# MonsieurETM/QPSK

Measured on AMD Instinct MI355X. Metric: complex Msamples/s demodulated + % HBM roofline, 2400-baud RRC+Costas path, higher is better.
Workload: dtype f32

## Files before the change

include/qpsk_hip.h:

```cpp
#ifndef QPSK_HIP_H
#define QPSK_HIP_H

#include <stddef.h>
#include <stdint.h>

#ifdef __cplusplus
extern "C" {
#endif

#define QPSK_NTAPS 127

typedef enum {
    QPSK_OK = 0,
    QPSK_ERR_NO_DEVICE = -1,
    QPSK_ERR_ARG = -2,
    QPSK_ERR_HIP = -3,
    QPSK_ERR_ALLOC = -4,
    QPSK_ERR_STATE = -5,
    QPSK_ERR_RANGE = -6
} qpsk_status;

typedef enum {
    QPSK_TIMING_HIST = 0,
    QPSK_TIMING_FIXED = 1,
// ... 134 lines not shown
int qpsk_outer_push(qpsk_ctx *ctx, const uint8_t *d_bits, long long bits_pitch, int nbits, int max_words, int32_t *d_count, uint8_t *d_words,
                    long long word_pitch, long long *d_pos, uint8_t *d_flags, int32_t *d_info);
int qpsk_outer_interleave_batch(qpsk_ctx *ctx, const uint8_t *d_words, int nrows, int nwords, int n, int branches, const uint8_t *d_hist_in,
                                uint8_t *d_hist_out, uint8_t *d_out);

enum { QPSK_DISPERSAL_MSB_FIRST = 1 };
int qpsk_dispersal_batch(qpsk_ctx *ctx, const uint8_t *d_in, long long in_pitch, int nrows, int len, int group, int flags, const uint8_t *d_flags,
                         int first, uint8_t *d_out, long long out_pitch);
int qpsk_dispersal_sequence(int len, int group, int flags, uint8_t *out);

int qpsk_nodesync_reset(qpsk_ctx *ctx, int nlinks, int nrot, int nshift, int span, int settle, int thr_num, int thr_den, int drop);
int qpsk_nodesync_shifts(int period, uint32_t keep0, uint32_t keep1);
int qpsk_nodesync_push(qpsk_ctx *ctx, const int8_t *d_soft_in, long long in_pitch, int ntx, const int32_t *d_vinfo, int8_t *d_soft_out,
                       long long out_pitch, int32_t *d_info);
int qpsk_nodesync_set(qpsk_ctx *ctx, const int32_t *d_cand);


int qpsk_rrc_fir_batch(qpsk_ctx *ctx, float *d_memory, const float *d_in, float *d_out, int nframes, int length);

int qpsk_rrc_fir_batch_fast(qpsk_ctx *ctx, float *d_memory, const float *d_in, float *d_out, int nframes, int length);

int qpsk_timing_hist_batch(qpsk_ctx *ctx, const float *d_filtered, int nframes, int32_t *d_index, int32_t *d_hist);

int qpsk_timing_scan_batch(qpsk_ctx *ctx, const float *d_in, int nframes, int32_t *d_index, int32_t *d_hist);

int qpsk_timing_fft_batch(qpsk_ctx *ctx, const float *d_in, int nframes, int32_t *d_index, float *d_filtered,
                          double *d_spectrum);

int qpsk_timing_fft_bin_batch(qpsk_ctx *ctx, const float *d_in, int nframes, int32_t *d_index, float *d_filtered,
                              double *d_bin);

int qpsk_costas_batch(qpsk_ctx *ctx, const float *d_symbols_in, int nframes, int nsym, float *d_state,
                      uint8_t *d_sym, float *d_costas);

int qpsk_fft_batch(qpsk_ctx *ctx, const double *d_in, double *d_out, int nbatch, int n, int inverse);

int qpsk_streams_reset(qpsk_ctx *ctx, int nstreams, double mixer_hz);
int qpsk_streams_set_loop_state(qpsk_ctx *ctx, const float *h_state);
int qpsk_streams_get_loop_state(qpsk_ctx *ctx, float *h_state);
int qpsk_streams_rx_cplx(qpsk_ctx *ctx, const float *d_in, uint8_t *d_sym, float *d_freq, float *d_phase,
                         float *d_costas, int32_t *d_index);
int qpsk_streams_rx_pcm(qpsk_ctx *ctx, const int16_t *d_pcm, uint8_t *d_sym, float *d_freq, float *d_phase,
                        float *d_costas, int32_t *d_index);
int qpsk_streams_rx_pcm_host(qpsk_ctx *ctx, const int16_t *h_pcm, float *h_loop_io, uint8_t *h_sym, float *h_costas,
                             int32_t *h_index);

int qpsk_tx_reset(qpsk_ctx *ctx, int nstreams, double tx_hz);
int qpsk_tx_symbols(qpsk_ctx *ctx, const uint8_t *d_symbols, int nsym, int16_t *d_pcm, float *d_baseband);


int qpsk_crc16_batch(qpsk_ctx *ctx, const uint8_t *d_data, int npackets, int nbytes, uint16_t *d_crc);

int qpsk_interleave_batch(qpsk_ctx *ctx, uint8_t *d_data, int npackets, int nbytes, int dir);

int qpsk_scramble_batch(qpsk_ctx *ctx, uint8_t *d_sym, int npackets, int nsym);

typedef struct qpsk_multi qpsk_multi;
int qpsk_multi_create(qpsk_multi **out, const int *devices, int ndev, const qpsk_params *p);
void qpsk_multi_destroy(qpsk_multi *mj);
int qpsk_multi_shards(const qpsk_multi *mj);
int qpsk_multi_load(qpsk_multi *mj, long long total_frames, const float *h_in);
int qpsk_multi_shard(qpsk_multi *mj, int r, int *device, long long *first, long long *count, qpsk_ctx **ctx, float **d_in);
int qpsk_multi_use_device_input(qpsk_multi *mj, int r, const float *d_in);
int qpsk_multi_set_direct_output(qpsk_multi *mj, int slot, uint8_t *h_sym, float *h_freq, float *h_phase);
int qpsk_multi_set_packed(qpsk_multi *mj, int on);
int qpsk_pack_symbols(qpsk_ctx *ctx, const uint8_t *d_sym, long long nrows, int nsym, uint8_t *d_packed);
int qpsk_unpack_symbols_host(const uint8_t *h_packed, long long nrows, int nsym, uint8_t *h_sym);
int qpsk_host_alloc(void **h_ptr, size_t bytes);
int qpsk_host_free(void *h_ptr);
int qpsk_multi_set_acquisition(qpsk_multi *mj, const int32_t *h_index, const float *h_seed);
int qpsk_multi_set_data(qpsk_multi *mj, int on);
int qpsk_multi_rx_begin(qpsk_multi *mj, int slot);
int qpsk_multi_rx_end(qpsk_multi *mj, int slot, uint8_t *h_sym, float *h_freq, float *h_phase);

int qpsk_dev_alloc(qpsk_ctx *ctx, void **d_ptr, size_t bytes);
int qpsk_dev_free(qpsk_ctx *ctx, void *d_ptr);
int qpsk_dev_upload(qpsk_ctx *ctx, void *d_dst, const void *h_src, size_t bytes);
int qpsk_dev_download(qpsk_ctx *ctx, void *h_dst, const void *d_src, size_t bytes);

int qpsk_selftest_sincos_hash(qpsk_ctx *ctx, uint32_t first, uint32_t count, unsigned long long *h_out);

int qpsk_test_inject_status(qpsk_ctx *ctx, int code);
int qpsk_test_hist_state(qpsk_ctx *ctx, int32_t *out);
int qpsk_test_fir_runs(qpsk_ctx *ctx, int nframes, int length, int32_t out[3]);
int qpsk_test_viterbi_launches(qpsk_ctx *ctx, int *out);
int qpsk_test_deframer_advance(qpsk_ctx *ctx, long long delta);
int qpsk_test_viterbi_stream_advance(qpsk_ctx *ctx, long long delta);
int qpsk_test_outer_advance(qpsk_ctx *ctx, long long delta);

#ifdef __cplusplus
}
#endif
#endif
```

qpsk_amd/csrc/api_ctx.cpp:

```cpp
#include "api_ctx.h"

using namespace qpsk;

static thread_local char g_err[512] = "";

int qpsk::fail(int code, const char *fmt, ...)
{
    va_list ap;
    va_start(ap, fmt);
    vsnprintf(g_err, sizeof g_err, fmt, ap);
    va_end(ap);
    return code;
}

static const struct { const char *name; int Tuning::*field; } TUNING_KEYS[] = {
    {"QPSK_FUSED_G", &Tuning::fused_g},       {"QPSK_FUSED_S", &Tuning::fused_s},     {"QPSK_FUSED_LDS", &Tuning::fused_lds},
    {"QPSK_FUSED_GENERIC", &Tuning::generic}, {"QPSK_PIPE_NF", &Tuning::pipe_nf},
    {"QPSK_PIPE_DBG", &Tuning::pipe_variant}, {"QPSK_HIST_GENERIC", &Tuning::hist_generic},
    {"QPSK_PIPE_V", &Tuning::pipe_v},         {"QPSK_PIPE_G", &Tuning::pipe_g},
    {"QPSK_PIPE_LAYOUT_LO", &Tuning::layout_lo}, {"QPSK_PIPE_LAYOUT_HI", &Tuning::layout_hi},
    {"QPSK_FIR_GENERIC", &Tuning::fir_generic}, {"QPSK_FFT_FUSED", &Tuning::fft_fused},
    {"QPSK_STREAM_BLOCK", &Tuning::stream_block}, {"QPSK_STREAM_POLL", &Tuning::stream_poll},
    {"QPSK_STREAM_SCAN", &Tuning::stream_scan}, {"QPSK_STREAM_CARRIER", &Tuning::stream_carrier},
    {"QPSK_LEAN_DMA", &Tuning::lean_dma},     {"QPSK_LEAN_PAIR", &Tuning::lean_pair},
    {"QPSK_EST_WAVES", &Tuning::est_waves},   {"QPSK_HIST_ONEPASS", &Tuning::hist_onepass},
    {"QPSK_VITERBI_LDS", &Tuning::viterbi_lds},   {"QPSK_VITERBI_CHUNK_ROWS", &Tuning::viterbi_chunk_rows},
};

int qpsk::ensure(qpsk_ctx *c, DevBuf &b, size_t bytes)
{
    if (b.cap >= bytes) return QPSK_OK;
    if (b.p) {
        HIP_TRY(hipStreamSynchronize(c->stream));
        HIP_TRY(hipFree(b.p));
        b.p = nullptr;
        b.cap = 0;
    }
    hipError_t e = hipMalloc(&b.p, bytes);
    if (e != hipSuccess) {
        b.p = nullptr;
        return fail(QPSK_ERR_ALLOC, "hipMalloc(%zu bytes): %s", bytes, hipGetErrorString(e));
    }
    b.cap = bytes;
    return QPSK_OK;
}

int qpsk::check_status(qpsk_ctx *c)
{
    const int st = __atomic_exchange_n(c->status.h_status, 0, __ATOMIC_ACQ_REL);
    if (st != STATUS_PIPE_TIMEOUT) c->streams.stream_work_unchecked = false;
    if (st == STATUS_PIPE_TIMEOUT) {
        if (c->streams.nstreams > 0 && c->streams.stream_work_unchecked) c->streams.poison();
        c->streams.stream_work_unchecked = false;
        return fail(QPSK_ERR_HIP, "pipeline kernel: producer/consumer wait timed out; results of the calls since the last synchronisation are invalid");
    }
    if (st == STATUS_PHASE_RANGE)
        return fail(QPSK_ERR_RANGE, "Costas loop phase beyond the bounded 2 pi wrap (input amplitude far outside the modem's range; "
                                    "the reference's phase_wrap() would spin or hang, costas_loop.c:61-67); results of the calls since the last synchronisation are invalid");
    if (st == STATUS_BAD_INDEX)
        return fail(QPSK_ERR_ARG, "an external timing offset (qpsk_rx_batch_ext d_index_in) lies outside 0..%d: the kernel demodulated that frame "
                                  "at offset 0; results of the calls since the last synchronisation are invalid", MAX_INDEX);
    if (st == STATUS_EST_NONFINITE)
        return fail(QPSK_ERR_RANGE, "qpsk_carrier_est_batch: a NaN / Inf sample inside the window the estimate reads; results of the calls since "
                                    "the last synchronisation are invalid");
    if (st == STATUS_SOFT_NONFINITE)
        return fail(QPSK_ERR_RANGE, "qpsk_soft_batch / qpsk_deframer_push_coded: a NaN / Inf sample among those a row's sums or soft output use, or a NaN / Inf gain; "
                                    "results of the calls since the last synchronisation are invalid");
    if (st == STATUS_SOFT_BAD_LAG)
        return fail(QPSK_ERR_ARG, "qpsk_soft_batch: a lag in d_lag is negative or puts the payload beyond the row (that row's soft output is zeros); "
                                  "results of the calls since the last synchronisation are invalid");
    if (st == STATUS_NONFINITE)
        return fail(QPSK_ERR_RANGE, "a Costas loop ended on a NaN / Inf state: the input held a non-finite sample (the reference hangs in phase_wrap() "
                                    "on an infinite phase, costas_loop.c:61-67); results of the calls since the last synchronisation are invalid");
    if (st != 0) return fail(QPSK_ERR_HIP, "kernel status %d", st);
    return QPSK_OK;
}

int qpsk_test_inject_status(qpsk_ctx *c, int code)
{
    if (!c || !c->status.h_status) return fail(QPSK_ERR_ARG, "null context");
    __atomic_store_n(c->status.h_status, code, __ATOMIC_RELEASE);
    return QPSK_OK;
}

int qpsk::bind(const qpsk_ctx *c)
{
    HIP_TRY(hipSetDevice(c->device));
    return QPSK_OK;
}

int qpsk::use_context_gains(qpsk_ctx *c)
{
    const float g[2] = {c->alpha, c->beta};
    if (c->h_gains.size() != 2 || c->h_gains[0] != g[0] || c->h_gains[1] != g[1]) {
        HIP_TRY(hipStreamSynchronize(c->stream));
        c->h_gains.assign(g, g + 2);
        HIP_TRY(hipMemcpyAsync(c->d_gains, c->h_gains.data(), sizeof g, hipMemcpyHostToDevice, c->stream));
    }
    return QPSK_OK;
}

const char *qpsk_last_error(void) { return g_err; }
const char *qpsk_version(void) { return "qpsk_hip 0.3 (gfx950)"; }

int qpsk_device_count(void)
{
    int n = 0;
    if (hipGetDeviceCount(&n) != hipSuccess) return 0;
// ... 40 lines not shown
        return fail(QPSK_ERR_NO_DEVICE, "no HIP device available (%s); this library has no CPU path",
                    e == hipSuccess ? "device count 0" : hipGetErrorString(e));
    if (device < 0) HIP_TRY(hipGetDevice(&device));
    if (device >= ndev) return fail(QPSK_ERR_NO_DEVICE, "device %d out of range (%d devices)", device, ndev);
    if (!(p->fs > 0.0) || !(p->rs > 0.0) || p->frame_size <= 0)
        return fail(QPSK_ERR_ARG, "fs, rs and frame_size must be positive");
    const int cycles = (int)(p->fs / p->rs);
    if (cycles < 1 || cycles > 64) return fail(QPSK_ERR_ARG, "CYCLES = (int)(fs/rs) = %d out of range 1..64", cycles);
    if (p->frame_size % cycles != 0)
        return fail(QPSK_ERR_ARG, "frame_size %d is not a multiple of CYCLES %d", p->frame_size, cycles);
    if (p->timing_mode < QPSK_TIMING_HIST || p->timing_mode > QPSK_TIMING_FFT)
        return fail(QPSK_ERR_ARG, "unknown timing_mode %d", p->timing_mode);
    if (p->fixed_index < 0 || p->fixed_index > MAX_INDEX)
        return fail(QPSK_ERR_ARG, "fixed_index %d outside 0..%d", p->fixed_index, MAX_INDEX);

    HIP_TRY(hipSetDevice(device));
    KERNEL_TRY(prepare_kernels());
    KERNEL_TRY(prepare_pipe_kernel());
    KERNEL_TRY(prepare_timing_scan());
    KERNEL_TRY(prepare_stream_block());
    KERNEL_TRY(prepare_stream_scan());
    KERNEL_TRY(prepare_carrier_est());
    qpsk_ctx *c = new qpsk_ctx();
    c->device = device;
    for (const auto &k : TUNING_KEYS) {
        const char *v = getenv(k.name);
        if (!v || !*v) continue;
        if (k.field == &Tuning::viterbi_chunk_rows) {
            char *end = nullptr;
            const long n = strtol(v, &end, 10);
            if (end == v || *end) continue;
            c->tune.*(k.field) = n < 0 ? -1 : n > INT_MAX ? INT_MAX : (int)n;
            continue;
        }
        c->tune.*(k.field) = atoi(v);
    }
    if (c->tune.viterbi_chunk_rows == 0) {
        delete c;
        return fail(QPSK_ERR_ARG, "qpsk_ctx_create: QPSK_VITERBI_CHUNK_ROWS = 0 in the environment (>= 1, or negative for the library's own choice)");
    }
    {
        int ncu = 0;
        if (hipDeviceGetAttribute(&ncu, hipDeviceAttributeMultiprocessorCount, device) == hipSuccess && ncu > 0)
            c->ncu = ncu;
    }
    c->prm = *p;
    c->cycles = cycles;
    c->nsym = p->frame_size / cycles;
    c->stream = (hipStream_t)stream;
    qpsk_host_rrc_taps((float)p->fs, (float)p->rs, p->rrc_alpha, c->taps);
    c->damping = sqrtf(2.0f) / 2.0f;
    qpsk_host_loop_gains(c->damping, p->loop_bw, &c->alpha, &c->beta);
    c->min_freq = p->min_freq;
    c->max_freq = p->max_freq;
    if (hipMalloc((void **)&c->d_taps, 128 * sizeof(float)) != hipSuccess ||
        hipMalloc((void **)&c->d_gains, MAX_BW * 2 * sizeof(float)) != hipSuccess ||
        hipHostMalloc((void **)&c->status.h_status, sizeof(int), hipHostMallocMapped) != hipSuccess ||
        hipHostGetDevicePointer((void **)&c->status.d_status, c->status.h_status, 0) != hipSuccess) {
        qpsk_ctx_destroy(c);
        return fail(QPSK_ERR_ALLOC, "hipMalloc of configuration buffers failed");
    }
    *c->status.h_status = 0;
    if (hipHostMalloc((void **)&c->streams.h_done, sizeof(unsigned), hipHostMallocMapped) != hipSuccess ||
        hipHostGetDevicePointer((void **)&c->streams.d_done, c->streams.h_done, 0) != hipSuccess) {
        qpsk_ctx_destroy(c);
        return fail(QPSK_ERR_ALLOC, "pinned counter");
    }
    *c->streams.h_done = 0;
    int rc = upload_config(c);
    if (rc != QPSK_OK) { qpsk_ctx_destroy(c); return rc; }
    *out = c;
    return QPSK_OK;
}

void qpsk_ctx_destroy(qpsk_ctx *c)
{
    if (!c) return;
    hipSetDevice(c->device);
    hipStreamSynchronize(c->stream);
    hipFree(c->d_taps);
    hipFree(c->d_gains);
    if (c->status.h_status) hipHostFree(c->status.h_status);
    if (c->streams.h_done) hipHostFree(c->streams.h_done);
    for (DevBuf *b : {&c->index, &c->filtered, &c->mixed, &c->keystream, &c->sympad, &c->mislist, &c->datacostas, &c->vitdec, &c->softgain, &c->dfstage})
        b->release();
    for (auto &kv : c->twiddles) hipFree(kv.second);
    hipFree(c->d_fast);
    c->hist.release();
    c->streams.release();
    c->tx.release();
    c->df.release();
    c->framer.release();
    c->vs.release();
    c->outer.release();
    c->nodesync.release();
    c->dispersal.release();
    delete c;
}

int qpsk_ctx_sync(qpsk_ctx *c)
{
    if (!c) return fail(QPSK_ERR_ARG, "null context");
    HIP_TRY(hipSetDevice(c->device));
    HIP_TRY(hipStreamSynchronize(c->stream));
    return check_status(c);
}

int qpsk_pack_symbols(qpsk_ctx *c, const uint8_t *d_sym, long long nrows, int nsym, uint8_t *d_packed)
{
    if (!c || !d_sym || !d_packed || nrows < 0 || nsym <= 0) return fail(QPSK_ERR_ARG, "qpsk_pack_symbols: bad argument");
    if (bind(c)) return QPSK_ERR_HIP;
    if ((nsym & 15) == 0 && (((uintptr_t)d_sym & 15) || ((uintptr_t)d_packed & 3)))
        return fail(QPSK_ERR_ARG, "qpsk_pack_symbols: d_sym must be 16-byte and d_packed 4-byte aligned");
    KERNEL_TRY(launch_pack_dibits(d_sym, d_packed, (size_t)nrows, nsym, c->stream));
    return QPSK_OK;
}

int qpsk_unpack_symbols_host(const uint8_t *h_packed, long long nrows, int nsym, uint8_t *h_sym)
{
    if (!h_packed || !h_sym || nrows < 0 || nsym <= 0) return fail(QPSK_ERR_ARG, "qpsk_unpack_symbols_host: bad argument");
    const size_t pb = (size_t)(nsym + 3) / 4;
    for (long long r = 0; r < nrows; r++) {
        const uint8_t *p = h_packed + (size_t)r * pb;
        uint8_t *o = h_sym + (size_t)r * (size_t)nsym;
        for (int i = 0; i < nsym; i++) o[i] = (uint8_t)((p[i >> 2] >> (2 * (i & 3))) & 3u);
    }
    return QPSK_OK;
}

int qpsk_ctx_check(qpsk_ctx *c)
{
    if (!c) return fail(QPSK_ERR_ARG, "null context");
    return check_status(c);
}

extern "C" int qpsk_set_error(int code, const char *msg)
{
    return fail(code, "%s", msg ? msg : "");
}

int qpsk_ctx_set_stream(qpsk_ctx *c, void *stream)
{
    if (!c) return fail(QPSK_ERR_ARG, "null context");
    HIP_TRY(hipSetDevice(c->device));
    HIP_TRY(hipStreamSynchronize(c->stream));
    c->stream = (hipStream_t)stream;
    return QPSK_OK;
}

int qpsk_ctx_set_tuning(qpsk_ctx *c, const char *name, int value)
{
    if (!c || !name) return fail(QPSK_ERR_ARG, "null argument");
    for (const auto &k : TUNING_KEYS)
        if (!strcmp(k.name, name)) {
            if (value == 0 && k.field == &Tuning::viterbi_chunk_rows)
                return fail(QPSK_ERR_ARG, "qpsk_ctx_set_tuning: QPSK_VITERBI_CHUNK_ROWS = 0 (>= 1, or negative for the library's own choice)");
            c->tune.*(k.field) = value < 0 ? -1 : value;
            return QPSK_OK;
        }
    return fail(QPSK_ERR_ARG, "qpsk_ctx_set_tuning: unknown name '%s'", name);
}

int qpsk_ctx_cycles(const qpsk_ctx *c) { return c ? c->cycles : 0; }
int qpsk_ctx_nsym(const qpsk_ctx *c) { return c ? c->nsym : 0; }
const char *qpsk_ctx_last_kernel(const qpsk_ctx *c) { return c ? c->last_kernel : ""; }

int qpsk_ctx_get_taps(const qpsk_ctx *c, float *h)
// ... 83 lines not shown
```

qpsk_amd/csrc/api_ctx.h:

```cpp
#ifndef QPSK_API_CTX_H
#define QPSK_API_CTX_H

#include "../../include/qpsk_hip.h"
#include "host_math.h"
#include "kernels.h"

#include <hip/hip_runtime.h>
#include <limits.h>
#include <math.h>
#include <stdarg.h>
#include <stdio.h>
#include <stdlib.h>
#include <string.h>
#include <time.h>
#include <algorithm>
#include <initializer_list>
#include <map>
#include <vector>

struct qpsk_ctx;

namespace qpsk {

QPSK_UNIT_LOCAL int fail(int code, const char *fmt, ...);

#define HIP_TRY(expr)                                                                         \
    do {                                                                                      \
        hipError_t e_ = (expr);                                                               \
        if (e_ != hipSuccess)                                                                 \
            return fail(QPSK_ERR_HIP, "%s: %s (%s:%d)", #expr, hipGetErrorString(e_), __FILE__, __LINE__); \
    } while (0)

#define KERNEL_TRY(expr)                                                                      \
    do {                                                                                      \
        (void)hipGetLastError();  \
        int e_ = (expr);                                                                      \
        if (e_ != 0)                                                                          \
            return fail(QPSK_ERR_HIP, "%s: %s (%s:%d)", #expr, hipGetErrorString((hipError_t)e_), __FILE__, __LINE__); \
    } while (0)

struct QPSK_UNIT_LOCAL DevBuf {
    void *p = nullptr;
    size_t cap = 0;
    void release() { hipFree(p); *this = DevBuf(); }
};

struct Tuning {
    int fused_g = -1, fused_s = -1, fused_lds = -1;
    int generic = -1;
    int pipe_nf = -1;
    int pipe_v = -1, pipe_g = -1;
    int layout_lo = -1, layout_hi = -1;
    int pipe_variant = -1;
    int hist_generic = -1;
    int fir_generic = -1;
    int stream_scan = -1;
    int stream_poll = -1;
    int stream_block = -1;
    int stream_carrier = -1;
    int lean_dma = -1;
    int hist_onepass = -1;
    int est_waves = -1;
    int lean_pair = -1;
    int viterbi_lds = -1;
    int fft_fused = -1;
    int viterbi_chunk_rows = -1;
};

static inline int tuned(int v, int dflt) { return v >= 0 ? v : dflt; }


struct StatusWord {
    int *h_status = nullptr;
    int *d_status = nullptr;
};

struct QPSK_UNIT_LOCAL HistGuess {
    int32_t *d_hint = nullptr;
    int32_t *h_hist_stats = nullptr, *d_hist_stats = nullptr;
    bool hint_valid = false;
    void release();
};

struct QPSK_UNIT_LOCAL Streams {
    int nstreams = 0;
    float *s_memory = nullptr, *s_dec = nullptr, *s_loop = nullptr, *s_mixer = nullptr;
    float *s_ctab = nullptr, *s_cstate = nullptr;
    bool carrier_shared = false;
    unsigned carrier_blocks = 0;
    unsigned carrier_scans = 0;
    float *carrier_pending = nullptr;
    bool stream_work_unchecked = false;
    bool streams_poisoned = false;
    unsigned char *h_stage = nullptr, *d_stage = nullptr;
    size_t stage_cap = 0;
    unsigned *h_done = nullptr, *d_done = nullptr;
    unsigned done_expect = 0;
    void poison()
    {
        streams_poisoned = true;
        carrier_shared = false;
        carrier_pending = nullptr;
    }
    void release();
};

struct QPSK_UNIT_LOCAL Transmitters {
    int ntx = 0;
    uint8_t *t_hist = nullptr;
    float *t_mixer = nullptr;
    DevBuf tx_b;
    void release();
};

struct QPSK_UNIT_LOCAL Deframer {
    uint8_t *state = nullptr, *tables = nullptr;
    size_t stride = 0;
    int nstreams = 0, nsync = 0, min_score = 0, nbytes = 0, max_packets = 0;
    unsigned long long sync_lo[2] = {0, 0}, sync_hi[2] = {0, 0};
    bool ready = false;
    bool coded = false;
    int mode = 0, nsteps = 0;
    int nbody = 0;
    CodedLayout layout;
    float scale = 0.f;
    unsigned crc_init = 0;
    void release();
};

struct QPSK_UNIT_LOCAL Framer {
    uint8_t *ks = nullptr;
    int ks_len = 0;
    void release();
};

struct QPSK_UNIT_LOCAL ViterbiStream {
    uint8_t *state = nullptr;
    size_t stride = 0;
    int nstreams = 0, depth = 0, window = 0;
    Puncture punct = {1, 1u, 1u, 2};
    bool punctured = false;
    long long total = 0;
    long long advanced = 0;
    void release();
};

struct QPSK_UNIT_LOCAL OuterLink {
    uint8_t *state = nullptr;
    size_t stride = 0;
    int nstreams = 0, n = 0, branches = 0, sync = 0, lock = 0, drop = 0, flags = 0;
    int group = 0;
    long long total = 0;
    void release();
};

struct QPSK_UNIT_LOCAL NodeSync {
    uint8_t *state = nullptr;
    int nlinks = 0, nrot = 0, nshift = 0, span = 0, settle = 0, thr_num = 0, thr_den = 0, drop = 0;
    int have = 0;
    void release();
};

struct QPSK_UNIT_LOCAL Dispersal {
    uint8_t *table = nullptr;
    int len = 0, group = 0, flags = 0;
    void release();
};

}

struct qpsk_ctx {
    int device = 0;
    qpsk::Tuning tune;
    int ncu = 256;
    const char *last_kernel = "";
    int viterbi_launches = 0;
    bool taps_symmetric = false;
    hipStream_t stream = nullptr;
    qpsk_params prm{};
    int cycles = 0, nsym = 0;
    float taps[QPSK_NTAPS];
    float damping = 0.f, alpha = 0.f, beta = 0.f;
    float min_freq = 0.f, max_freq = 0.f;
    float *d_taps = nullptr;
    float *d_gains = nullptr;
    std::vector<float> h_gains;
    qpsk::DevBuf index, filtered, mixed, keystream, sympad, mislist;
    qpsk::DevBuf datacostas;
    qpsk::DevBuf vitdec;
    qpsk::DevBuf softgain;
    qpsk::DevBuf dfstage;
    int keystream_len = 0;
    std::map<int, double *> twiddles;
    float *d_fast = nullptr;
    bool fast_valid = false;
    qpsk::StatusWord status;
    qpsk::HistGuess hist;
    qpsk::Streams streams;
    qpsk::Transmitters tx;
    qpsk::Deframer df;
    qpsk::Framer framer;
    qpsk::ViterbiStream vs;
    qpsk::OuterLink outer;
    qpsk::NodeSync nodesync;
    qpsk::Dispersal dispersal;
};

namespace qpsk {

static const int MAX_BW = 64;

QPSK_UNIT_LOCAL int ensure(qpsk_ctx *c, DevBuf &b, size_t bytes);
QPSK_UNIT_LOCAL int check_status(qpsk_ctx *c);
QPSK_UNIT_LOCAL int bind(const qpsk_ctx *c);
QPSK_UNIT_LOCAL int use_context_gains(qpsk_ctx *c);

QPSK_UNIT_LOCAL int fir_full_rate(qpsk_ctx *c, const float *x, const float *memory, float *y, int nframes, int length, size_t in_pitch = 0);
QPSK_UNIT_LOCAL int fft_timing_indices(qpsk_ctx *c, const float *d_in, int nframes, int32_t *d_index, float *d_y = nullptr,
                                       double *d_X = nullptr, size_t pitch = 0, double *d_bin = nullptr);
QPSK_UNIT_LOCAL int costas_over_symbols(qpsk_ctx *c, float *d_symbols, int nframes, int nsym, int dstride, float *d_state,
                                        uint8_t *d_sym, float *d_costas, const float *refill = nullptr,
                                        const int32_t *refill_index = nullptr, bool refill_planar = false);

struct Pattern {
    int period;
    uint32_t keep0, keep1;
};
QPSK_UNIT_LOCAL int layout_add_pattern(const char *who, const Pattern *pattern, CodedLayout *l);
QPSK_UNIT_LOCAL int layout_add_stride(const char *who, int nsteps, const int *stride, CodedLayout *l);
struct ViterbiRoute {
    size_t per_row;
    bool lds;
    size_t chunk_rows;
};
QPSK_UNIT_LOCAL ViterbiRoute viterbi_route(const qpsk_ctx *c, size_t rows, int nsteps);

}

#endif
```

qpsk_amd/csrc/api_rx.cpp:

```cpp
#include "api_ctx.h"

using namespace qpsk;

#ifdef QPSK_PIPE_PROFILE
static const int PIPE_VARIANT_MASK = ~0;
#else
static const int PIPE_VARIANT_MASK = 4 | 8 | 16 | 64 | 128 | 256 | 512 | 1024 | 8192;
#endif

int qpsk_test_hist_state(qpsk_ctx *c, int32_t *out)
{
    if (!c || !out) return fail(QPSK_ERR_ARG, "null argument");
    out[0] = out[1] = out[2] = out[3] = out[4] = -1;
    if (!c->hist.d_hint) return QPSK_OK;
    HIP_TRY(hipSetDevice(c->device));
    HIP_TRY(hipStreamSynchronize(c->stream));
    int32_t h[2];
    HIP_TRY(hipMemcpy(h, c->hist.d_hint, sizeof h, hipMemcpyDeviceToHost));
    out[0] = c->hist.hint_valid ? h[0] : -1;
    out[1] = h[1];
    out[2] = c->hist.h_hist_stats[0]; out[3] = c->hist.h_hist_stats[1]; out[4] = c->hist.h_hist_stats[2];
    return QPSK_OK;
}

int qpsk_test_fir_runs(qpsk_ctx *c, int nframes, int length, int32_t out[3])
{
    if (!c || !out) return fail(QPSK_ERR_ARG, "qpsk_test_fir_runs: null argument");
    if (nframes < 1 || length < 1) return fail(QPSK_ERR_ARG, "qpsk_test_fir_runs: nframes %d length %d", nframes, length);
    const FirRuns r = rrc_fir_stream_runs(nframes, length, c->ncu);
    out[0] = r.ntiles; out[1] = r.parts; out[2] = r.tpp;
    return QPSK_OK;
}

void HistGuess::release()
{
    if (d_hint) hipFree(d_hint);
    if (h_hist_stats) hipHostFree(h_hist_stats);
    *this = HistGuess();
}

static bool fir_takes_stream(const qpsk_ctx *c) { return c->taps_symmetric && tuned(c->tune.fir_generic, 0) == 0; }

int qpsk::fir_full_rate(qpsk_ctx *c, const float *x, const float *memory, float *y, int nframes, int length, size_t in_pitch)
{
    if (fir_takes_stream(c))
        return launch_rrc_fir_stream(x, memory, y, c->d_taps, nframes, length, c->stream, in_pitch, c->ncu);
    return launch_rrc_fir(x, memory, y, c->d_taps, nframes, length, c->stream, in_pitch);
}

static void pick_tiling(const qpsk_ctx *c, int nframes, int nbw, int *G, int *S)
{
    int g = nframes / 256;
    if (g < 1) g = 1;
    if (g > 64 / nbw) g = 64 / nbw;
    if (g < 1) g = 1;
    g = tuned(c->tune.fused_g, g);
    if (g < 1) g = 1;
    if (g * nbw > 64) g = 64 / nbw;
    int s = tuned(c->tune.fused_s, 64);
    s &= ~7;
    if (s < 8) s = 8;
    const size_t budget = (size_t)tuned(c->tune.fused_lds, 64 * 1024);
    while (s > 8 && fused_lds_bytes(g, s, c->cycles, nbw) > budget) s -= 8;
    while (g > 1 && fused_lds_bytes(g, s, c->cycles, nbw) > (size_t)MAX_LDS_BYTES) g--;
    *G = g;
    *S = s;
}

static int get_twiddles(qpsk_ctx *c, int n, double **out)
{
    auto it = c->twiddles.find(n);
    if (it != c->twiddles.end()) { *out = it->second; return QPSK_OK; }
    const size_t cnt = n >= 2 ? (size_t)n / 2 : 1;
    std::vector<double> h(2 * cnt, 0.0);
    qpsk_host_twiddles(n, h.data());
    double *tw = nullptr;
    HIP_TRY(hipMalloc((void **)&tw, sizeof(double) * 2 * cnt));
    HIP_TRY(hipMemcpy(tw, h.data(), sizeof(double) * 2 * cnt, hipMemcpyHostToDevice));
    c->twiddles[n] = tw;
    *out = tw;
    return QPSK_OK;
}

static int fft_timing_tables(qpsk_ctx *c, double **tw_out, double **cs_out)
{
    const int C = c->cycles, nfft = timing_fft_nfft();
    if (C < 2 || C > 8 || (C & (C - 1)))
        return fail(QPSK_ERR_ARG, "QPSK_TIMING_FFT needs CYCLES in {2,4,8} (the symbol-rate bin NFFT/CYCLES must be exact and the offset < 8); CYCLES = %d", C);
    if (c->prm.frame_size < timing_fft_first() + nfft)
        return fail(QPSK_ERR_ARG, "QPSK_TIMING_FFT needs frame_size >= %d", timing_fft_first() + nfft);
    double *tw = nullptr;
    int rc = get_twiddles(c, nfft, &tw);
    if (rc) return rc;
    double *cs = nullptr;
    auto it = c->twiddles.find(-C);
    if (it == c->twiddles.end()) {
        std::vector<double> full(2 * (size_t)C);
        qpsk_host_phases(C, full.data());
        HIP_TRY(hipMalloc((void **)&cs, sizeof(double) * 2 * C));
        HIP_TRY(hipMemcpy(cs, full.data(), sizeof(double) * 2 * C, hipMemcpyHostToDevice));
        c->twiddles[-C] = cs;
    } else {
        cs = it->second;
    }
    *tw_out = tw;
    *cs_out = cs;
    return QPSK_OK;
}

int qpsk::fft_timing_indices(qpsk_ctx *c, const float *d_in, int nframes, int32_t *d_index, float *d_y, double *d_X, size_t pitch, double *d_bin)
{
    double *tw = nullptr, *cs = nullptr;
    int rc = fft_timing_tables(c, &tw, &cs);
// ... 152 lines not shown
            if (hint) hipFree(hint);
            return fail(QPSK_ERR_ALLOC, "one-pass histogram route: %s", hipGetErrorString(e));
        }
        h_stats[0] = h_stats[1] = h_stats[2] = -1;
        c->hist.d_hint = hint;
        c->hist.h_hist_stats = h_stats;
        c->hist.d_hist_stats = d_stats;
        c->hist.hint_valid = false;
    }
    const int op = tuned(c->tune.hist_onepass, -1);
    const int seen = __atomic_load_n(&c->hist.h_hist_stats[1], __ATOMIC_ACQUIRE), off_majority = __atomic_load_n(&c->hist.h_hist_stats[2], __ATOMIC_ACQUIRE);
    const bool guess_is_good = seen > 0 && off_majority == 0;
    if (op == 0 || !c->hist.hint_valid || !(op == 1 || guess_is_good) || !rx_hist_shape_ok(a)) return QPSK_OK;
    if (int rc = ensure(c, c->index, sizeof(int32_t) * (size_t)a.nframes)) return rc;
    if (int rc = ensure(c, c->mislist, sizeof(int32_t) * (size_t)a.nframes)) return rc;
    int32_t *mis_count = c->hist.d_hint + 1;
    HIP_TRY(hipMemsetAsync(mis_count, 0, sizeof(int32_t), c->stream));
    KERNEL_TRY(launch_rx_hist(a, (int32_t *)c->index.p, c->hist.d_hint, (int32_t *)c->mislist.p, mis_count, c->status.d_status, c->stream));
    FusedArgs af = a;
    af.index = (const int32_t *)c->index.p;
    af.frame_list = (const int32_t *)c->mislist.p;
    af.frame_list_count = mis_count;
    af.G = 4;
    af.S = 64;
    KERNEL_TRY(launch_rx_fused(af, c->stream));
    KERNEL_TRY(launch_index_majority((const int32_t *)c->index.p, a.nframes, c->hist.d_hint, mis_count, c->hist.d_hist_stats, c->stream));
    c->last_kernel = "rx_hist_kernel (one pass on the guessed index) + rx_fused_kernel (fall-back list)";
    if (d_index)
        HIP_TRY(hipMemcpyAsync(d_index, c->index.p, sizeof(int32_t) * (size_t)a.nframes, hipMemcpyDeviceToDevice, c->stream));
    *taken = true;
    return QPSK_OK;
}

static int rx_launch(qpsk_ctx *c, const FusedArgs &a, const RxRoute &rt)
{
    if (a.est_tw && !(rt.kind == K_FUSED_PIPE && rt.nf == pipe_max_nf()) && rt.kind != K_LEAN)
        return fail(QPSK_ERR_STATE, "internal: in-launch FFT timing estimate planned for a kernel that has none");
    if (a.data_rule && rt.kind != K_LEAN)
        return fail(QPSK_ERR_STATE, "internal: data rule planned for a kernel that has none");
    switch (rt.kind) {
    case K_LEAN:
        KERNEL_TRY(launch_rx_lean(a, rt.G, rt.layout, c->status.d_status, c->stream));
        c->last_kernel = a.est_tw ? "rx_lean_kernel (FFT timing estimate inside the launch)" : "rx_lean_kernel";
        break;
    case K_PIPE2:
        KERNEL_TRY(launch_rx_pipe2(a, rt.G, rt.layout, c->status.d_status, c->stream));
        c->last_kernel = "rx_pipe2_kernel";
        break;
    case K_FUSED_PIPE:
        KERNEL_TRY(launch_rx_fused_pipe(a, rt.nf, c->status.d_status, c->stream));
        c->last_kernel = a.est_tw ? "rx_fused_pipe_kernel (FFT timing estimate inside the launch)" : "rx_fused_pipe_kernel";
        break;
    default:
        KERNEL_TRY(launch_rx_fused(a, c->stream));
        c->last_kernel = "rx_fused_kernel";
    }
    return QPSK_OK;
}

static int rx_batch_common(qpsk_ctx *c, const float *d_in, long long frame_pitch, int nframes, int nbw, uint8_t *d_sym,
                           float *d_freq, float *d_phase, float *d_costas, int32_t *d_index, float *d_hz,
                           const ExtAcq *ext = nullptr, uint8_t *d_data = nullptr)
{
    if (!c || !d_in || !(d_sym || d_data)) return fail(QPSK_ERR_ARG, "qpsk_rx_batch: null context, input or symbol buffer");
    if (nframes <= 0) return fail(QPSK_ERR_ARG, "qpsk_rx_batch: nframes = %d", nframes);
    if (frame_pitch == 0) frame_pitch = c->prm.frame_size;
    if (frame_pitch < c->prm.frame_size)
        return fail(QPSK_ERR_ARG, "qpsk_rx_batch_pitched: frame_pitch %lld below frame_size %d", frame_pitch, c->prm.frame_size);
    if (bind(c)) return QPSK_ERR_HIP;
    FusedArgs a{};
    a.x = reinterpret_cast<const float2 *>(d_in);
    a.frame_pitch = (size_t)frame_pitch;
    a.nframes = nframes;
    a.frame_size = c->prm.frame_size;
    a.cycles = c->cycles;
    a.nsym = c->nsym;
    pick_tiling(c, nframes, nbw, &a.G, &a.S);
    a.fixed_index = c->prm.fixed_index;
    a.dbg = tuned(c->tune.pipe_variant, 0) & PIPE_VARIANT_MASK;
    a.lean_dma = tuned(c->tune.lean_dma, 1) != 0;
    a.lean_twowin = tuned(c->tune.lean_dma, 1) != 2 ? 1 : 0;
    a.est_waves = tuned(c->tune.est_waves, 0);
    a.lean_pair = tuned(c->tune.lean_pair, 3);
    a.taps = c->d_taps;
    a.gains = c->d_gains;
    a.nbw = nbw;
    a.min_freq = c->min_freq;
    a.max_freq = c->max_freq;
    a.rs = c->prm.rs;
    a.sym = d_sym ? d_sym : d_data;
    a.data_rule = d_data && !d_sym;
    a.freq = d_freq;
    a.phase = d_phase;
    a.costas = reinterpret_cast<float2 *>(d_costas);
    a.hz = d_hz;
    a.status = c->status.d_status;
    if (ext) a.index = ext->index;
    if (ext && ext->seed) {
        a.state_in = ext->seed;
        a.seed_setters = 1;
    }

    RxRoute rt;
    if (int rc = rx_route(c, a, d_data != nullptr, &rt)) return rc;

    a.data_rule = rt.data_rule;
    if (rt.need_pad) {
        if (int rc = ensure(c, c->sympad, (size_t)rt.G * (size_t)c->nsym)) return rc;
        a.sym_pad = (uint8_t *)c->sympad.p;
    }
    if (rt.need_dump) {
        if (int rc = ensure(c, c->datacostas, sizeof(float2) * (size_t)nframes * (size_t)c->nsym)) return rc;
        a.costas = (float2 *)c->datacostas.p;
    }

    const bool hist_guess = c->prm.timing_mode == QPSK_TIMING_HIST && !ext;
    if (hist_guess) {
        bool taken = false;
        const int rc = rx_hist_onepass(c, a, rt, d_index, &taken);
        if (rc || taken) return rc;
    }

    const int32_t *idx = a.index;
    if (!idx) {
        if (int rc = timing_indices(c, d_in, (size_t)frame_pitch, nframes, &idx, rt.fused_fft)) return rc;
        a.index = idx;
    }
    if (rt.fused_fft) {
        double *est_tw = nullptr, *est_cs = nullptr;
        if (int rc = fft_timing_tables(c, &est_tw, &est_cs)) return rc;
        a.est_tw = reinterpret_cast<const double2 *>(est_tw);
        a.est_cs = reinterpret_cast<const double2 *>(est_cs);
        a.index_out = d_index ? (int32_t *)c->index.p : nullptr;
        if (d_index) idx = (const int32_t *)c->index.p;
    }

    if (int rc = rx_launch(c, a, rt)) return rc;

    if (hist_guess && c->hist.d_hint && idx && tuned(c->tune.hist_onepass, -1) != 0) {
        KERNEL_TRY(launch_index_majority(idx, nframes, c->hist.d_hint, c->hist.d_hint + 1, c->hist.d_hist_stats, c->stream));
        c->hist.hint_valid = true;
    }
    if (rt.kind == K_LEAN && (nframes & 1)) {
        const size_t last0 = (size_t)((nframes - 1) / rt.G) * (size_t)rt.G;
        HIP_TRY(hipMemcpyAsync(a.sym + (size_t)(nframes - 1) * (size_t)c->nsym, a.sym_pad + ((size_t)(nframes - 1) - last0) * (size_t)c->nsym,
                               (size_t)c->nsym, hipMemcpyDeviceToDevice, c->stream));
    }
    if (d_data && !a.data_rule)
        KERNEL_TRY(launch_data_from_costas(a.costas, d_data, (size_t)nframes * (size_t)c->nsym, c->stream));
    if (d_index) {
        if (idx == d_index) {
        } else if (idx)
            HIP_TRY(hipMemcpyAsync(d_index, idx, sizeof(int32_t) * (size_t)nframes, hipMemcpyDeviceToDevice, c->stream));
        else
            KERNEL_TRY(launch_fill_i32(d_index, nframes, c->prm.fixed_index, c->stream));
    }
    return QPSK_OK;
}

static int rx_prologue(qpsk_ctx *c)
{
    if (!c) return QPSK_OK;
    if (bind(c)) return QPSK_ERR_HIP;
    return use_context_gains(c);
}

// ... 46 lines not shown

int qpsk_rx_batch_data(qpsk_ctx *c, const float *d_in, long long frame_pitch, int nframes, const int32_t *d_index_in, const float *d_seed,
                       uint8_t *d_data, uint8_t *d_sym, float *d_freq, float *d_phase, int32_t *d_index, float *d_hz)
{
    if (int rp = rx_prologue(c)) return rp;
    if (frame_pitch < 0) return fail(QPSK_ERR_ARG, "qpsk_rx_batch_data: frame_pitch = %lld", frame_pitch);
    if (!d_data) return fail(QPSK_ERR_ARG, "qpsk_rx_batch_data: d_data is NULL");
    const ExtAcq ext = {d_index_in, d_seed};
    return rx_batch_common(c, d_in, frame_pitch, nframes, 1, d_sym, d_freq, d_phase, nullptr, d_index, d_hz, &ext, d_data);
}

int qpsk_sync_batch(qpsk_ctx *c, const uint8_t *d_data, int nframes, int nsym, const uint8_t *h_sync, int nsync, int lag_min, int lag_max,
                    int nout, uint8_t *d_out, int32_t *d_lag, int32_t *d_rot, int32_t *d_score)
{
    if (!c || !d_data || !h_sync) return fail(QPSK_ERR_ARG, "qpsk_sync_batch: null context, data or sync word");
    if (nframes <= 0 || nsym <= 0) return fail(QPSK_ERR_ARG, "qpsk_sync_batch: nframes = %d, nsym = %d", nframes, nsym);
    if (nsync < 1 || nsync > SYNC_MAX_WORD) return fail(QPSK_ERR_ARG, "qpsk_sync_batch: nsync = %d outside 1..%d", nsync, SYNC_MAX_WORD);
    if (nout < 0 || lag_min < 0 || lag_max < lag_min || (long long)lag_max + nsync + nout > nsym)
        return fail(QPSK_ERR_ARG, "qpsk_sync_batch: lags %d..%d, nsync %d, nout %d do not fit a row of %d", lag_min, lag_max, nsync, nout, nsym);
    if (!d_out && !d_lag && !d_rot && !d_score) return fail(QPSK_ERR_ARG, "qpsk_sync_batch: every output is NULL");
    for (int i = 0; i < nsync; i++)
        if (h_sync[i] > 3) return fail(QPSK_ERR_ARG, "qpsk_sync_batch: sync[%d] = %d is not a dibit", i, (int)h_sync[i]);
    if (d_out && nout > 0) {
        const uintptr_t o0 = (uintptr_t)d_out, o1 = o0 + (size_t)nframes * (size_t)nout;
        const uintptr_t d0 = (uintptr_t)d_data, d1 = d0 + (size_t)nframes * (size_t)nsym;
        if (o0 < d1 && d0 < o1) return fail(QPSK_ERR_ARG, "qpsk_sync_batch: d_out overlaps d_data");
    }
    if (bind(c)) return QPSK_ERR_HIP;
    KERNEL_TRY(launch_sync_search(d_data, nframes, nsym, h_sync, nsync, lag_min, lag_max, nout, nout > 0 ? d_out : nullptr, d_lag, d_rot,
                                  d_score, c->stream));
    c->last_kernel = "sync_search_kernel";
    return QPSK_OK;
}

int qpsk_rx_batch_bw_ext(qpsk_ctx *c, const float *d_in, int nframes, const float *h_loop_bw, int nbw, const int32_t *d_index_in,
                         const float *d_seed, uint8_t *d_sym, float *d_freq, float *d_phase, int32_t *d_index)
{
    const ExtAcq ext = {d_index_in, d_seed};
    return rx_batch_bw_impl(c, d_in, nframes, h_loop_bw, nbw, d_sym, d_freq, d_phase, d_index, &ext);
}

int qpsk::costas_over_symbols(qpsk_ctx *c, float *d_symbols, int nframes, int nsym, int dstride, float *d_state,
                              uint8_t *d_sym, float *d_costas, const float *refill, const int32_t *refill_index, bool refill_planar)
{
    float *carrier_tab = c->streams.carrier_pending;
    c->streams.carrier_pending = nullptr;
    if (tuned(c->tune.generic, 0)) {
        if (carrier_tab) KERNEL_TRY(launch_carrier_table(c->streams.s_cstate, carrier_tab, c->prm.frame_size, true, c->stream));
        KERNEL_TRY(launch_costas(d_symbols, nframes, nsym, dstride, 1, c->d_gains, c->min_freq, c->max_freq, d_state, d_state,
                                 d_sym, d_costas, c->status.d_status, c->stream));
        if (refill) {
            if (dstride != nsym) return fail(QPSK_ERR_ARG, "internal: refill needs packed rows");
            KERNEL_TRY(launch_decimate(refill, refill_index, d_symbols, nframes, nsym * c->cycles, c->cycles, nsym, c->stream));
        }
        return QPSK_OK;
    }
    FusedArgs a{};
    a.nframes = nframes;
    a.nsym = nsym;
    a.frame_size = nsym * c->cycles;
    a.cycles = c->cycles;
    a.refill = reinterpret_cast<const float2 *>(refill);
    a.refill_dst = reinterpret_cast<float2 *>(d_symbols);
    a.refill_planar = refill_planar ? 1 : 0;
    a.index = refill_index;
    a.gains = c->d_gains;
    a.nbw = 1;
    a.min_freq = c->min_freq;
    a.max_freq = c->max_freq;
    a.rs = c->prm.rs;
    a.state_in = d_state;
    a.state_out = d_state;
    a.sym = d_sym;
    a.costas = reinterpret_cast<float2 *>(d_costas);
    a.dsrc = reinterpret_cast<const float2 *>(d_symbols);
    a.dstride = dstride;
    a.status = c->status.d_status;
    if (carrier_tab) {
        a.carrier_state = c->streams.s_cstate;
        a.carrier_tab = reinterpret_cast<float2 *>(carrier_tab);
        a.carrier_frame = c->prm.frame_size;
    }
    a.dbg = tuned(c->tune.pipe_variant, 0) & PIPE_VARIANT_MASK;
    int nf = (nframes + c->ncu * pipe_frames(1) - 1) / (c->ncu * pipe_frames(1));
    if (nf < 1) nf = 1;
    if (nf > pipe_max_nf()) nf = pipe_max_nf();
    KERNEL_TRY(launch_costas_pipe(a, nf, c->status.d_status, c->stream));
    return QPSK_OK;
}

int qpsk_rrc_fir_batch(qpsk_ctx *c, float *d_memory, const float *d_in, float *d_out, int nframes, int length)
{
    if (!c || !d_in || !d_out) return fail(QPSK_ERR_ARG, "qpsk_rrc_fir_batch: null argument");
    if (nframes <= 0 || length <= 0) return fail(QPSK_ERR_ARG, "qpsk_rrc_fir_batch: nframes %d length %d", nframes, length);
    if (bind(c)) return QPSK_ERR_HIP;
    const float *src = d_in;
    if (d_in == d_out) {
        const size_t bytes = sizeof(float) * 2 * (size_t)nframes * length;
        int rc = ensure(c, c->mixed, bytes);
        if (rc) return rc;
        HIP_TRY(hipMemcpyAsync(c->mixed.p, d_in, bytes, hipMemcpyDeviceToDevice, c->stream));
        src = (const float *)c->mixed.p;
    }
    KERNEL_TRY(fir_full_rate(c, src, d_memory, d_out, nframes, length));
    c->last_kernel = fir_takes_stream(c) ? "rrc_fir_stream_kernel" : "rrc_fir_kernel";
    if (d_memory) KERNEL_TRY(launch_delay_line(src, d_memory, nframes, length, c->stream));
    return QPSK_OK;
}

int qpsk_rrc_fir_batch_fast(qpsk_ctx *c, float *d_memory, const float *d_in, float *d_out, int nframes, int length)
{
    if (!c || !d_in || !d_out) return fail(QPSK_ERR_ARG, "qpsk_rrc_fir_batch_fast: null argument");
    if (nframes <= 0 || length <= 0) return fail(QPSK_ERR_ARG, "qpsk_rrc_fir_batch_fast: nframes %d length %d", nframes, length);
    if (d_in == d_out) return fail(QPSK_ERR_ARG, "qpsk_rrc_fir_batch_fast: every block reads 126 samples in front of it: separate buffers");
    if (bind(c)) return QPSK_ERR_HIP;
    if (!c->fast_valid) {
        const int n = rrc_fir_fast_nfft();
        std::vector<float> t(4 * (size_t)n);
        qpsk_host_fir_fast_tables(c->taps, t.data(), t.data() + 2 * n);
        if (!c->d_fast) HIP_TRY(hipMalloc((void **)&c->d_fast, sizeof(float) * t.size()));
        HIP_TRY(hipStreamSynchronize(c->stream));
        HIP_TRY(hipMemcpy(c->d_fast, t.data(), sizeof(float) * t.size(), hipMemcpyHostToDevice));
        c->fast_valid = true;
    }
    KERNEL_TRY(launch_rrc_fir_fast(d_in, d_memory, d_out, c->d_fast, c->d_fast + 2 * rrc_fir_fast_nfft(), nframes, length, c->stream));
    if (d_memory) KERNEL_TRY(launch_delay_line(d_in, d_memory, nframes, length, c->stream));
    return QPSK_OK;
}

int qpsk_timing_hist_batch(qpsk_ctx *c, const float *d_filtered, int nframes, int32_t *d_index, int32_t *d_hist)
{
    if (!c || !d_filtered || !d_index) return fail(QPSK_ERR_ARG, "qpsk_timing_hist_batch: null argument");
    if (nframes <= 0) return fail(QPSK_ERR_ARG, "nframes = %d", nframes);
    if (bind(c)) return QPSK_ERR_HIP;
    KERNEL_TRY(launch_timing_hist(d_filtered, nframes, c->prm.frame_size, c->cycles, d_index, d_hist,
                                  tuned(c->tune.hist_generic, 0) == 2, c->stream));
    return QPSK_OK;
}

int qpsk_timing_scan_batch(qpsk_ctx *c, const float *d_in, int nframes, int32_t *d_index, int32_t *d_hist)
{
    if (!c || !d_in || !d_index) return fail(QPSK_ERR_ARG, "qpsk_timing_scan_batch: null argument");
    if (nframes <= 0) return fail(QPSK_ERR_ARG, "nframes = %d", nframes);
    if (bind(c)) return QPSK_ERR_HIP;
    if (!(c->cycles == 8 && c->prm.frame_size % timing_scan_tile() == 0 && ((uintptr_t)d_in % 16) == 0))
        return fail(QPSK_ERR_ARG, "qpsk_timing_scan_batch needs CYCLES = 8, frame_size %% %d == 0 and 16-byte aligned input "
                                  "(use qpsk_rrc_fir_batch + qpsk_timing_hist_batch otherwise)", timing_scan_tile());
    KERNEL_TRY(launch_timing_scan(d_in, nframes, c->prm.frame_size, c->d_taps, d_index, d_hist, c->status.d_status, c->stream, 0,
                                  c->taps_symmetric && tuned(c->tune.fir_generic, 0) == 0));
    return QPSK_OK;
}

int qpsk_timing_fft_batch(qpsk_ctx *c, const float *d_in, int nframes, int32_t *d_index, float *d_filtered, double *d_spectrum)
{
    if (!c || !d_in || !d_index) return fail(QPSK_ERR_ARG, "qpsk_timing_fft_batch: null argument");
    if (nframes <= 0) return fail(QPSK_ERR_ARG, "nframes = %d", nframes);
    if (bind(c)) return QPSK_ERR_HIP;
    return fft_timing_indices(c, d_in, nframes, d_index, d_filtered, d_spectrum);
}

int qpsk_timing_fft_bin_batch(qpsk_ctx *c, const float *d_in, int nframes, int32_t *d_index, float *d_filtered, double *d_bin)
{
    if (!c || !d_in || !d_index) return fail(QPSK_ERR_ARG, "qpsk_timing_fft_bin_batch: null argument");
    if (nframes <= 0) return fail(QPSK_ERR_ARG, "nframes = %d", nframes);
    if (bind(c)) return QPSK_ERR_HIP;
    return fft_timing_indices(c, d_in, nframes, d_index, d_filtered, nullptr, 0, d_bin);
// ... 83 lines not shown
```

qpsk_amd/csrc/costas_asm.h:

```cpp
#ifndef QPSK_COSTAS_ASM_H
#define QPSK_COSTAS_ASM_H

#include "qpsk_device.h"

namespace qpsk {

constexpr int COSTAS_ASM_GROUP = 16;
#ifndef COSTAS_RING_STEPS
#define COSTAS_RING_STEPS 64
#endif
constexpr int COSTAS_RING_GROUP = COSTAS_RING_STEPS;
static_assert(COSTAS_RING_GROUP == 16 || COSTAS_RING_GROUP == 32 || COSTAS_RING_GROUP == 64, "ring groups of 16, 32 or 64 steps");
#ifndef COSTAS_RING_STEPS_LO
#define COSTAS_RING_STEPS_LO 16
#endif
constexpr int COSTAS_RING_GROUP_LO = COSTAS_RING_STEPS_LO;
static_assert(COSTAS_RING_GROUP_LO == 16 || COSTAS_RING_GROUP_LO == 32 || COSTAS_RING_GROUP_LO == 64, "ring groups of 16, 32 or 64 steps");

__device__ __forceinline__ unsigned lds_addr(const void *p)
{
    return (unsigned)(__UINTPTR_TYPE__)(const __attribute__((address_space(3))) void *)p;
}

__device__ __forceinline__ unsigned long long uniform64(unsigned long long v)
// ... 30 lines not shown
    QPSK_STEP_1_PRE(QPSK_CMP_P(PIN), PIN)                                                                     \
    "s_cbranch_vccnz " LW "f\n"                                                                               \
    LR ":\n\t"

#define QPSK_STEP_P_PRE(CMP, PIN)                                                                             \
    CMP                                                                                                       \
    "v_cvt_f64_f32 v[106:107], " PIN "\n\t"                                                                   \
    "v_mul_f64 v[104:105], v[106:107], %[k2pi]\n\t"                                                           \
    "v_rndne_f64_e32 v[104:105], v[104:105]\n\t"                                                              \
    "v_fmac_f64_e32 v[106:107], %[nhpi], v[104:105]\n\t"                                                      \
    "v_mul_f64 v[108:109], v[106:107], v[106:107]\n\t"                                                        \
    "v_fma_f64 v[100:101], v[106:107], %[km], %[kj]\n\t"                                                      \
    "v_fma_f64 v[110:111], v[108:109], %[ka], %[kb]\n\t"                                                      \
    "v_mul_f64 v[104:105], v[108:109], v[100:101]\n\t"                                                        \
    "v_fma_f64 v[110:111], v[108:109], v[110:111], %[kc]\n\t"
#define QPSK_HEAD_CHAIN_P(PIN) QPSK_STEP_P_PRE("", PIN)
#define QPSK_HEAD_DEFERRED_P(PIN, LW, LR)                                                                    \
    QPSK_STEP_P_PRE(QPSK_CMP_P(PIN), PIN)                                                                     \
    "s_cbranch_vccnz " LW "f\n"                                                                               \
    LR ":\n\t"

#define QPSK_BODY_F32(PIN, POUT, DREG, WAIT, READ, QW)                                                        \
    WAIT                                                                                                      \
    "v_pk_mul_f32 v[100:101], " DREG ", v[110:111] op_sel_hi:[1,0]\n\t"                                       \
    "v_pk_mul_f32 v[104:105], " DREG ", v[112:113] op_sel:[1,0] op_sel_hi:[0,0]\n\t"                          \
    READ                                                                                                      \
    "v_pk_add_f32 v[114:115], v[100:101], v[104:105] neg_hi:[0,1]\n\t"                                        \
    QW                                                                                                        \
    "v_sub_f32_e64 v106, |v115|, |v114|\n\t"                                    \
    "v_xor_b32_e32 v108, v114, v115\n\t"                                  \
    "v_pk_mul_f32 v[102:103], %[beal], v[106:107] op_sel_hi:[1,0]\n\t"                   \
    "v_bfi_b32 v108, %[absm], 1.0, v108\n\t"                                                    \
    "v_fmac_f32_e32 v118, v108, v102\n\t"                           \
    "v_add_f32_e32 " POUT ", " PIN ", v118\n\t"                                                               \
    "v_fmac_f32_e32 " POUT ", v108, v103\n\t"

#define QPSK_BODY(PIN, POUT, DREG, WAIT, READ, QW)                                                            \
    "v_fma_f64 v[110:111], v[108:109], v[110:111], %[c2]\n\t"                                                 \
    "v_mul_f64 v[104:105], v[106:107], v[108:109]\n\t"                                                        \
    "v_fma_f64 v[110:111], v[108:109], v[110:111], %[c1]\n\t"                                                 \
    "v_fma_f64 v[112:113], v[108:109], v[112:113], %[s1]\n\t"                                                 \
    "v_fma_f64 v[110:111], v[108:109], v[110:111], 1.0\n\t"                                                   \
    "v_fmac_f64_e32 v[106:107], v[104:105], v[112:113]\n\t"                   \
    "v_cvt_f32_f64 v110, v[110:111]\n\t"                                                                      \
    "v_cvt_f32_f64 v112, v[106:107]\n\t"                                                                      \
    QPSK_BODY_F32(PIN, POUT, DREG, WAIT, READ, QW)

#define QPSK_BODY_P(PIN, POUT, DREG, WAIT, READ, QW)                                                          \
    "v_fma_f64 v[110:111], v[108:109], v[110:111], %[kd]\n\t"                                                 \
    "v_fmac_f64_e32 v[100:101], v[104:105], v[110:111]\n\t"                                                   \
    "v_cvt_f32_f64 v110, v[100:101]\n\t"                                                                      \
    "v_med3_f32 v118, v118, %[fmin], %[fmax]\n\t"                                                             \
    "v_min3_f32 v126, v126, |v114|, |v115|\n\t"                                                               \
    "v_mul_f32_dpp v112, v110, %[sg] quad_perm:[1,0,3,2] row_mask:0xf bank_mask:0xf\n\t"                      \
    QPSK_BODY_F32(PIN, POUT, DREG, WAIT, READ, QW)

#define QPSK_TAIL(POUT, FOUT, LW, LR)                                                                         \
    "v_cmp_ge_f32_e64 vcc, |" POUT "|, %[tau]\n\t"                                                            \
    "v_med3_f32 " FOUT ", v118, %[fmin], %[fmax]\n\t"                                                         \
    "v_min3_f32 v126, v126, |v114|, |v115|\n\t"                                                               \
    "s_cbranch_vccnz " LW "f\n"                                                                               \
    LR ":\n\t"

#define QPSK_WRAP_ONCE(P)                                                                                     \
    "v_cvt_f64_f32 v[100:101], " P "\n\t"                                                                     \
    "v_bfi_b32 v129, %[absm], v127, " P "\n\t"                                                                \
    "v_add_f64 v[100:101], v[100:101], -v[128:129]\n\t"                                                       \
    "v_cvt_f32_f64 v104, v[100:101]\n\t"                                                                      \
    "v_cndmask_b32_e32 " P ", " P ", v104, vcc\n\t"                                                           \
    "v_cmp_ge_f32_e64 vcc, |" P "|, %[tau]\n\t"                                                               \
    "s_or_b64 %[fl], %[fl], vcc\n\t"

#define QPSK_WRAP_HEAD(PIN, LW, LR)                                                                           \
    LW ":\n\t"                                                                                                \
    QPSK_WRAP_ONCE(PIN)                                                                                       \
    QPSK_STEP_1_PRE("", PIN)                                                                                  \
    "s_branch " LR "b\n"
#define QPSK_WRAP_HEAD_P(PIN, LW, LR)                                                                         \
    LW ":\n\t"                                                                                                \
    QPSK_WRAP_ONCE(PIN)                                                                                       \
    QPSK_STEP_P_PRE("", PIN)                                                                                  \
    "s_branch " LR "b\n"

#define QPSK_WRAP_TAIL(POUT, LW, LR)                                                                          \
    LW ":\n\t"                                                                                                \
    QPSK_WRAP_ONCE(POUT)                                                                                      \
    "s_branch " LR "b\n"

#define QPSK_WAIT0 "s_waitcnt lgkmcnt(0)\n\t"
#define QPSK_WAIT1 "s_waitcnt lgkmcnt(1)\n\t"
#define QPSK_RDA(OFF) "ds_read_b128 v[120:123], " QPSK_DA " offset:" QPSK_STR(OFF) "\n\t"
#define QPSK_RDB(OFF) "ds_read_b128 v[136:139], " QPSK_DA " offset:" QPSK_STR(OFF) "\n\t"
#define QPSK_QW(OFF) "ds_write_b128 " QPSK_ZA ", v[140:143] offset:" QPSK_STR(OFF) "\n\t"

#define QPSK_STEP_QUAD_(HD, BD, SA_LO, SA_HI, SB_LO, SB_HI, RD1, RD2, QOFF, P4, L1, L2, L3, L4)                \
    HD("v140", "1" L1, "2" L1)                                                                        \
    BD("v140", "v141", SA_LO, QPSK_WAIT1, RD1, "")                                                    \
    HD("v141", "1" L2, "2" L2)                                                                        \
    BD("v141", "v142", SA_HI, "", "", "")                                                             \
    HD("v142", "1" L3, "2" L3)                                                                        \
    BD("v142", "v143", SB_LO, QPSK_WAIT0, RD2, "")                                                    \
    HD("v143", "1" L4, "2" L4)                                                                        \
    BD("v143", P4, SB_HI, "", "", QPSK_QW(QOFF))
#define QPSK_STEP_QUAD(...) QPSK_STEP_QUAD_(QPSK_HEAD_DEFERRED, QPSK_BODY, __VA_ARGS__)

#define QPSK_DA "%[da]"
#define QPSK_ZA "%[za]"
__device__ __forceinline__ unsigned costas_asm_run(float &phase, float &freq, unsigned &d_addr, unsigned &z_addr,
                                                   unsigned groups, float alpha, float beta, float min_freq,
                                                   float max_freq, unsigned long long &flags_out, unsigned long long ign = 0ull)
{
    unsigned long long flags, tmp;
    ign = uniform64(ign);
    const double c3 = -0x1.6c087e89a359dp-10, s2 = 0x1.1107605230bc4p-7;
    double beal;
    {
        const float2 ba = make_float2(beta, alpha);
        __builtin_memcpy(&beal, &ba, 8);
    }
    asm volatile(
        "v_mov_b32 v128, 0x54442d18\n\t"
        "v_mov_b32 v127, 0x401921fb\n\t"
        "ds_read_b128 v[120:123], %[da]\n\t"
        "s_mov_b64 %[fl], 0\n\t"
        "s_waitcnt lgkmcnt(0)\n"
        "2:\n\t"
        "v_mov_b32 v130, %[p]\n\t"
        "v_mov_b32 v131, %[f]\n\t"
        "v_mov_b32 v118, %[f]\n\t"
        "v_mov_b32 v126, 0x7f800000\n\t"
        "v_mov_b32 v140, %[p]\n\t"
        QPSK_HEAD_CHAIN("v140")
        QPSK_BODY("v140", "v141", "v[120:121]", QPSK_WAIT1, QPSK_RDB(16), "")
        QPSK_HEAD_DEFERRED("v141", "101", "201")
        QPSK_BODY("v141", "v142", "v[122:123]", "", "", "")
        QPSK_HEAD_DEFERRED("v142", "102", "202")
        QPSK_BODY("v142", "v143", "v[136:137]", QPSK_WAIT0, QPSK_RDA(32), "")
        QPSK_HEAD_DEFERRED("v143", "103", "203")
        QPSK_BODY("v143", "v140", "v[138:139]", "", "", QPSK_QW(0))
        QPSK_STEP_QUAD("v[120:121]", "v[122:123]", "v[136:137]", "v[138:139]", QPSK_RDB(48), QPSK_RDA(64), 16, "v140", "04", "05", "06", "07")
        QPSK_STEP_QUAD("v[120:121]", "v[122:123]", "v[136:137]", "v[138:139]", QPSK_RDB(80), QPSK_RDA(96), 32, "v140", "08", "09", "10", "11")
        QPSK_STEP_QUAD("v[120:121]", "v[122:123]", "v[136:137]", "v[138:139]", QPSK_RDB(112), QPSK_RDA(128), 48, "%[p]", "12", "13", "14", "15")
        QPSK_TAIL("%[p]", "%[f]", "116", "216")
        "v_cmp_eq_f32_e64 %[tm], 0, v126\n\t"
        "s_andn2_b64 %[tm], %[tm], %[ign]\n\t"
        "s_or_b64 %[fl], %[fl], %[tm]\n\t"
        "s_cmp_lg_u64 %[fl], 0\n\t"
        "s_cbranch_scc1 3f\n\t"
        "v_add_u32_e32 %[da], 0x80, %[da]\n\t"
        "v_add_u32_e32 %[za], 0x40, %[za]\n\t"
        "s_sub_u32 %[ng], %[ng], 1\n\t"
        "s_cmp_lg_u32 %[ng], 0\n\t"
        "s_cbranch_scc1 2b\n\t"
        "s_branch 4f\n"
        "3:\n\t"
        "v_mov_b32 %[p], v130\n\t"
        "v_mov_b32 %[f], v131\n\t"
        "s_branch 4f\n"
        QPSK_WRAP_HEAD("v141", "101", "201")
        QPSK_WRAP_HEAD("v142", "102", "202")
        QPSK_WRAP_HEAD("v143", "103", "203")
        QPSK_WRAP_HEAD("v140", "104", "204")
        QPSK_WRAP_HEAD("v141", "105", "205")
        QPSK_WRAP_HEAD("v142", "106", "206")
        QPSK_WRAP_HEAD("v143", "107", "207")
        QPSK_WRAP_HEAD("v140", "108", "208")
        QPSK_WRAP_HEAD("v141", "109", "209")
        QPSK_WRAP_HEAD("v142", "110", "210")
        QPSK_WRAP_HEAD("v143", "111", "211")
        QPSK_WRAP_HEAD("v140", "112", "212")
        QPSK_WRAP_HEAD("v141", "113", "213")
        QPSK_WRAP_HEAD("v142", "114", "214")
        QPSK_WRAP_HEAD("v143", "115", "215")
        QPSK_WRAP_TAIL("%[p]", "116", "216")
        "4:\n\t"
        "s_waitcnt lgkmcnt(0)"
        : [p] "+v"(phase), [f] "+v"(freq), [da] "+v"(d_addr), [za] "+v"(z_addr), [ng] "+s"(groups),
          [fl] "=&s"(flags), [tm] "=&s"(tmp)
        : [c3] "v"(c3), [s2] "v"(s2), [fmax] "v"(max_freq), [beal] "v"(beal),
          [k2pi] "s"(0x1.45F306DC9C883p-1), [nhpi] "s"(-0x1.921FB54442D18p0), [c4] "s"(0x1.99343027bf8c3p-16),
          [s3] "s"(-0x1.994eb3774cf24p-13), [c2] "s"(0x1.55553e1068f19p-5), [s1] "s"(-0x1.555545995a603p-3),
          [c1] "s"(-0x1.ffffffd0c621cp-2), [fmin] "s"(min_freq), [tau] "s"(TAU_F), [absm] "s"(0x7fffffffu), [ign] "s"(ign)
        : "vcc", "scc", "memory", "v100", "v101", "v102", "v103", "v104", "v105", "v106", "v107", "v108", "v109",
          "v110", "v111", "v112", "v113", "v114", "v115", "v116", "v117", "v118", "v119", "v120", "v121", "v122",
          "v123", "v124", "v125", "v126", "v127", "v128", "v129", "v130", "v131", "v132", "v133", "v134", "v135",
          "v136", "v137", "v138", "v139", "v140", "v141", "v142", "v143");
    flags_out = flags;
    return groups;
}

#undef QPSK_DA
#undef QPSK_ZA

#define QPSK_DA "v132"
#define QPSK_ZA "v134"
#define QPSK_RDN "ds_read_b128 v[120:123], v124\n\t"
#define QPSK_RING_CR "ds_read_b32 v125, %[ra]\n\t"
#define QPSK_CAT_(a, b) a##b
#define QPSK_CAT(a, b) QPSK_CAT_(a, b)
#define QPSK_RING_ALIGN_1 ".p2align 6\n"
#define QPSK_RING_ALIGN_P ".p2align 6\n\ts_nop 0\n\ts_nop 0\n\ts_nop 0\n\ts_nop 0\n"
#define QPSK_RQ(HD, BD, ...) QPSK_STEP_QUAD_(HD, BD, "v[120:121]", "v[122:123]", "v[136:137]", "v[138:139]", __VA_ARGS__)
#define QPSK_RING_Q0(HC, HD, BD, CR)                                                                                          \
    HC("v140")                                                                                                         \
    BD("v140", "v141", "v[120:121]", QPSK_WAIT1, QPSK_RDB(16) CR, "")                                                  \
    HD("v141", "1001", "2001")                                                                                         \
    BD("v141", "v142", "v[122:123]", "", "", "")                                                                       \
    HD("v142", "1002", "2002")                                                                                         \
    BD("v142", "v143", "v[136:137]", QPSK_WAIT0, QPSK_RDA(32), "")                                                     \
    HD("v143", "1003", "2003")                                                                                         \
    BD("v143", "v140", "v[138:139]", "", "", QPSK_QW(0))
#define QPSK_RING_QN(HD, BD, B8, B4, B, CR)                                                                                   \
    QPSK_RQ(HD, BD, QPSK_RDB(B8+16) CR, QPSK_RDA(B8+32), B4+0, "v140", B "00", B "01", B "02", B "03")
#define QPSK_RING_Q4_15(HD, BD, B8, B4, B, RDLAST, PLAST)                                                                     \
    QPSK_RQ(HD, BD, QPSK_RDB(B8+48), QPSK_RDA(B8+64), B4+16, "v140", B "04", B "05", B "06", B "07")                \
    QPSK_RQ(HD, BD, QPSK_RDB(B8+80), QPSK_RDA(B8+96), B4+32, "v140", B "08", B "09", B "10", B "11")                \
    QPSK_RQ(HD, BD, QPSK_RDB(B8+112), RDLAST, B4+48, PLAST, B "12", B "13", B "14", B "15")
#define QPSK_RING_W1_15(WH, B)                                                                                                \
    WH("v141", "1" B "01", "2" B "01") WH("v142", "1" B "02", "2" B "02") WH("v143", "1" B "03", "2" B "03")            \
    WH("v140", "1" B "04", "2" B "04") WH("v141", "1" B "05", "2" B "05") WH("v142", "1" B "06", "2" B "06")            \
    WH("v143", "1" B "07", "2" B "07") WH("v140", "1" B "08", "2" B "08") WH("v141", "1" B "09", "2" B "09")            \
    WH("v142", "1" B "10", "2" B "10") WH("v143", "1" B "11", "2" B "11") WH("v140", "1" B "12", "2" B "12")            \
    WH("v141", "1" B "13", "2" B "13") WH("v142", "1" B "14", "2" B "14") WH("v143", "1" B "15", "2" B "15")
#define QPSK_RING_W0(WH, B) WH("v140", "1" B "00", "2" B "00")
#define QPSK_RING_POS_16 "7"
#define QPSK_RING_DSH_16 "7"
#define QPSK_RING_ZSH_16 "6"
#define QPSK_RING_CSH_16 "2"
#define QPSK_RING_INCHUNK_16 "s_and_b32 %[t0], %[k], 3\n\ts_cmp_lg_u32 %[t0], 0\n\ts_cbranch_scc1 2b\n\t"
#define QPSK_RING_STEPS_16(HC, HD, BD)                                                                                        \
    QPSK_RING_Q0(HC, HD, BD, QPSK_RING_CR) QPSK_RING_Q4_15(HD, BD, 0, 0, "0", QPSK_RDN, "%[p]")
#define QPSK_RING_WRAPS_16(WH) QPSK_RING_W1_15(WH, "0")
#define QPSK_RING_POS_32 "3"
#define QPSK_RING_DSH_32 "8"
#define QPSK_RING_ZSH_32 "7"
#define QPSK_RING_CSH_32 "1"
#define QPSK_RING_INCHUNK_32 "s_and_b32 %[t0], %[k], 1\n\ts_cmp_lg_u32 %[t0], 0\n\ts_cbranch_scc1 2b\n\t"
#define QPSK_RING_STEPS_32(HC, HD, BD)                                                                                        \
    QPSK_RING_Q0(HC, HD, BD, "") QPSK_RING_Q4_15(HD, BD, 0, 0, "0", QPSK_RDA(128), "v140")                                    \
    QPSK_RING_QN(HD, BD, 128, 64, "1", QPSK_RING_CR) QPSK_RING_Q4_15(HD, BD, 128, 64, "1", QPSK_RDN, "%[p]")
#define QPSK_RING_WRAPS_32(WH) QPSK_RING_W1_15(WH, "0") QPSK_RING_W0(WH, "1") QPSK_RING_W1_15(WH, "1")
#define QPSK_RING_POS_64 "1"
#define QPSK_RING_DSH_64 "9"
#define QPSK_RING_ZSH_64 "8"
#define QPSK_RING_CSH_64 "0"
#define QPSK_RING_INCHUNK_64 ""
#define QPSK_RING_STEPS_64(HC, HD, BD)                                                                                        \
    QPSK_RING_Q0(HC, HD, BD, "") QPSK_RING_Q4_15(HD, BD, 0, 0, "0", QPSK_RDA(128), "v140")                                    \
    QPSK_RING_QN(HD, BD, 128, 64, "1", "") QPSK_RING_Q4_15(HD, BD, 128, 64, "1", QPSK_RDA(256), "v140")                       \
    QPSK_RING_QN(HD, BD, 256, 128, "2", "") QPSK_RING_Q4_15(HD, BD, 256, 128, "2", QPSK_RDA(384), "v140")                     \
    QPSK_RING_QN(HD, BD, 384, 192, "3", QPSK_RING_CR) QPSK_RING_Q4_15(HD, BD, 384, 192, "3", QPSK_RDN, "%[p]")
#define QPSK_RING_WRAPS_64(WH)                                                                                                \
    QPSK_RING_W1_15(WH, "0") QPSK_RING_W0(WH, "1") QPSK_RING_W1_15(WH, "1") QPSK_RING_W0(WH, "2") QPSK_RING_W1_15(WH, "2")      \
    QPSK_RING_W0(WH, "3") QPSK_RING_W1_15(WH, "3")
#define QPSK_RING_TEXT(HC, HD, BD, WH, INIT, ALIGN, G)                                                                        \
    "v_mov_b32 v128, 0x54442d18\n\t"                                                    \
    "v_mov_b32 v127, 0x401921fb\n\t" INIT                                                                                   \
    "s_and_b32 %[t0], %[k], " QPSK_CAT(QPSK_RING_POS_, G) "\n\t"                                                       \
    "s_lshl_b32 %[t0], %[t0], " QPSK_CAT(QPSK_RING_DSH_, G) "\n\t"                                                     \
    "v_add_u32_e32 v132, %[t0], %[db]\n\t"                                                                             \
    "ds_read_b128 v[120:123], v132\n\t"                                                                                \
    "s_mov_b64 %[fl], 0\n\t"                                                                                           \
    "s_waitcnt lgkmcnt(0)\n"                                                                                           \
                                                                                              \
    ALIGN                                                                                                              \
    "2:\n\t"                                                                                                           \
                                                        \
    "s_and_b32 %[t0], %[k], " QPSK_CAT(QPSK_RING_POS_, G) "\n\t"                                                       \
    "s_lshl_b32 %[t1], %[t0], " QPSK_CAT(QPSK_RING_DSH_, G) "\n\t"                                                     \
    "v_add_u32_e32 v132, %[t1], %[db]\n\t"                                                                             \
    "s_lshl_b32 %[t1], %[t0], " QPSK_CAT(QPSK_RING_ZSH_, G) "\n\t"                                                     \
    "v_add_u32_e32 v134, %[t1], %[zb]\n\t"                                                                             \
    "s_add_u32 %[t0], %[k], 1\n\t"                                                                                     \
    "s_and_b32 %[t0], %[t0], " QPSK_CAT(QPSK_RING_POS_, G) "\n\t"                                                      \
    "s_lshl_b32 %[t0], %[t0], " QPSK_CAT(QPSK_RING_DSH_, G) "\n\t"                                                     \
    "v_add_u32_e32 v124, %[t0], %[db]\n\t"                                                                             \
    "v_mov_b32 v130, %[p]\n\t"                                                                                         \
    "v_mov_b32 v131, %[f]\n\t"                                                                                         \
    "v_mov_b32 v118, %[f]\n\t"                                        \
    "v_mov_b32 v126, 0x7f800000\n\t"                                                                                   \
    "v_mov_b32 v140, %[p]\n\t"                                                                                         \
                      \
    QPSK_CAT(QPSK_RING_STEPS_, G)(HC, HD, BD)                                                                          \
    QPSK_TAIL("%[p]", "%[f]", "1900", "2900")                                                                          \
    "v_cmp_eq_f32_e64 %[tm], 0, v126\n\t"                                                                              \
    "s_andn2_b64 %[tm], %[tm], %[ign]\n\t"    \
    "s_or_b64 %[fl], %[fl], %[tm]\n\t"                                                                                 \
    "s_cmp_lg_u64 %[fl], 0\n\t"                                                                                        \
    "s_cbranch_scc1 3f\n\t"                                                                                            \
    "s_add_u32 %[k], %[k], 1\n\t"                                                                                      \
    QPSK_CAT(QPSK_RING_INCHUNK_, G)                             \
                         \
    "s_lshr_b32 %[t0], %[k], " QPSK_CAT(QPSK_RING_CSH_, G) "\n\t"                                                      \
    "v_mov_b32 v104, %[t0]\n\t"                                                                                        \
    "s_mov_b64 %[ex], exec\n\t"                                                                                        \
    "s_mov_b64 exec, 1\n\t"                                                                                            \
    "ds_write_b32 %[ca], v104\n\t"                                                                                     \
    "s_mov_b64 exec, %[ex]\n\t"                                                                                        \
    "s_cmp_ge_u32 %[k], %[ke]\n\t"                                                                                     \
    "s_cbranch_scc1 4f\n\t"                                                                                            \
       \
    "v_cmp_le_i32_e64 %[tm], v125, %[t0]\n\t"                                                                          \
    "s_cmp_lg_u64 %[tm], 0\n\t"                                                                                        \
    "s_cbranch_scc0 2b\n\t"                                                                                            \
    "s_branch 4f\n"                                                                                                    \
    "3:\n\t"                                                                                                           \
    "v_mov_b32 %[p], v130\n\t"                                                                                         \
    "v_mov_b32 %[f], v131\n\t"                                                                                         \
    "s_branch 4f\n"                                                                                                    \
    QPSK_CAT(QPSK_RING_WRAPS_, G)(WH)                                                                                  \
    QPSK_WRAP_TAIL("%[p]", "1900", "2900")                                                                             \
    "4:\n\t"                                                                                                           \
    "s_waitcnt lgkmcnt(0)"

__device__ __forceinline__ void costas_asm_run_ring(float &phase, float &freq, unsigned d_base, unsigned z_base,
                                                    unsigned ready_addr, unsigned consumed_addr, unsigned &k, unsigned kend,
                                                    float alpha, float beta, float min_freq, float max_freq,
                                                    unsigned long long &flags_out, unsigned long long ign = 0ull)
{
    unsigned long long flags, tmp, ex;
    ign = uniform64(ign);
    kend = __builtin_amdgcn_readfirstlane(kend);
    unsigned t0, t1;
    const double c3 = -0x1.6c087e89a359dp-10, s2 = 0x1.1107605230bc4p-7;
    double beal;
    {
        const float2 ba = make_float2(beta, alpha);
        __builtin_memcpy(&beal, &ba, 8);
    }
    asm volatile(
        QPSK_RING_TEXT(QPSK_HEAD_CHAIN, QPSK_HEAD_DEFERRED, QPSK_BODY, QPSK_WRAP_HEAD, "", QPSK_RING_ALIGN_1, COSTAS_RING_STEPS)
        : [p] "+v"(phase), [f] "+v"(freq), [k] "+s"(k), [fl] "=&s"(flags), [tm] "=&s"(tmp), [ex] "=&s"(ex),
          [t0] "=&s"(t0), [t1] "=&s"(t1)
        : [db] "v"(d_base), [zb] "v"(z_base), [ra] "v"(ready_addr), [ca] "v"(consumed_addr), [ke] "s"(kend),
          [c3] "v"(c3), [s2] "v"(s2), [fmax] "v"(max_freq), [beal] "v"(beal),
          [k2pi] "s"(0x1.45F306DC9C883p-1), [nhpi] "s"(-0x1.921FB54442D18p0), [c4] "s"(0x1.99343027bf8c3p-16),
          [s3] "s"(-0x1.994eb3774cf24p-13), [c2] "s"(0x1.55553e1068f19p-5), [s1] "s"(-0x1.555545995a603p-3),
          [c1] "s"(-0x1.ffffffd0c621cp-2), [fmin] "s"(min_freq), [tau] "s"(TAU_F), [absm] "s"(0x7fffffffu), [ign] "s"(ign)
        : "vcc", "scc", "memory", "v100", "v101", "v102", "v103", "v104", "v105", "v106", "v107", "v108", "v109",
          "v110", "v111", "v112", "v113", "v114", "v115", "v116", "v117", "v118", "v119", "v120", "v121", "v122",
          "v123", "v124", "v125", "v126", "v127", "v128", "v129", "v130", "v131", "v132", "v133", "v134", "v135",
          "v136", "v137", "v138", "v139", "v140", "v141", "v142", "v143");
    flags_out = flags;
}

__device__ __forceinline__ void costas_asm_run_ring_pair(float &phase, float &freq, unsigned d_base, unsigned z_base,
                                                         unsigned ready_addr, unsigned consumed_addr, unsigned &k, unsigned kend,
                                                         float alpha, float beta, float min_freq, float max_freq, bool odd,
                                                         unsigned long long &flags_out, unsigned long long ign = 0ull)
{
    unsigned long long flags, tmp, ex;
    ign = uniform64(ign);
    kend = __builtin_amdgcn_readfirstlane(kend);
    unsigned t0, t1;
    const double ka = odd ? 0.0 : 0x1.99343027bf8c3p-16, kb = odd ? -0x1.994eb3774cf24p-13 : -0x1.6c087e89a359dp-10;
    const double kc = odd ? 0x1.1107605230bc4p-7 : 0x1.55553e1068f19p-5, kd = odd ? -0x1.555545995a603p-3 : -0x1.ffffffd0c621cp-2;
    const double km = odd ? 1.0 : 0.0, kj = odd ? -0.0 : 1.0;
    const float sg = odd ? -1.0f : 1.0f;
    double beal;
    {
        const float2 ba = make_float2(beta, alpha);
        __builtin_memcpy(&beal, &ba, 8);
    }
    asm volatile(
        QPSK_RING_TEXT(QPSK_HEAD_CHAIN_P, QPSK_HEAD_DEFERRED_P, QPSK_BODY_P, QPSK_WRAP_HEAD_P, "v_mov_b32 v114, 1.0\n\tv_mov_b32 v115, 1.0\n\t", QPSK_RING_ALIGN_P, COSTAS_RING_STEPS)
        : [p] "+v"(phase), [f] "+v"(freq), [k] "+s"(k), [fl] "=&s"(flags), [tm] "=&s"(tmp), [ex] "=&s"(ex),
          [t0] "=&s"(t0), [t1] "=&s"(t1)
        : [db] "v"(d_base), [zb] "v"(z_base), [ra] "v"(ready_addr), [ca] "v"(consumed_addr), [ke] "s"(kend),
          [ka] "v"(ka), [kb] "v"(kb), [kc] "v"(kc), [kd] "v"(kd), [km] "v"(km), [kj] "v"(kj), [sg] "v"(sg),
          [fmax] "v"(max_freq), [beal] "v"(beal),
          [k2pi] "s"(0x1.45F306DC9C883p-1), [nhpi] "s"(-0x1.921FB54442D18p0),
          [fmin] "s"(min_freq), [tau] "s"(TAU_F), [absm] "s"(0x7fffffffu), [ign] "s"(ign)
        : "vcc", "scc", "memory", "v100", "v101", "v102", "v103", "v104", "v105", "v106", "v107", "v108", "v109",
          "v110", "v111", "v112", "v113", "v114", "v115", "v116", "v117", "v118", "v119", "v120", "v121", "v122",
          "v123", "v124", "v125", "v126", "v127", "v128", "v129", "v130", "v131", "v132", "v133", "v134", "v135",
          "v136", "v137", "v138", "v139", "v140", "v141", "v142", "v143");
    flags_out = flags;
}
#undef QPSK_DA
#undef QPSK_ZA

}
#endif
```

qpsk_amd/csrc/costas_asm_lo.h:

```cpp
#ifndef QPSK_COSTAS_ASM_LO_H
#define QPSK_COSTAS_ASM_LO_H

#include "costas_asm.h"

namespace qpsk {

constexpr int COSTAS_ASM_LO_END_VGPR = 128;

#define QPSKLO_HEAD_CHAIN(PIN)                                                                                  \
    "v_cvt_f64_f32 v[90:91], " PIN "\n\t"                                                                   \
    "v_mul_f64 v[88:89], v[90:91], %[k2pi]\n\t"                                                           \
    "v_rndne_f64_e32 v[88:89], v[88:89]\n\t"                                                              \
    "v_fmac_f64_e32 v[90:91], %[nhpi], v[88:89]\n\t"                                                      \
    "v_mul_f64 v[92:93], v[90:91], v[90:91]\n\t"                                                        \
    "v_fma_f64 v[94:95], v[92:93], %[c4], %[c3]\n\t"                                                      \
    "v_fma_f64 v[96:97], v[92:93], %[s3], %[s2]\n\t"

#define QPSKLO_CMP_P(PIN) "v_cmp_ge_f32_e64 vcc, |" PIN "|, %[tau]\n\t"
#define QPSKLO_STEP_1_PRE(CMP, PIN)                                                                             \
    CMP                                                                                                       \
    "v_cvt_f64_f32 v[90:91], " PIN "\n\t"                                                                   \
    "v_mul_f64 v[88:89], v[90:91], %[k2pi]\n\t"                                                           \
    "v_med3_f32 v102, v102, %[fmin], %[fmax]\n\t"                                                             \
    "v_rndne_f64_e32 v[88:89], v[88:89]\n\t"                                                              \
// ... 5 lines not shown
#define QPSKLO_HEAD_DEFERRED(PIN, LW, LR)                                                                      \
    QPSKLO_STEP_1_PRE(QPSKLO_CMP_P(PIN), PIN)                                                                     \
    "s_cbranch_vccnz " LW "f\n"                                                                               \
    LR ":\n\t"

#define QPSKLO_STEP_P_PRE(CMP, PIN)                                                                             \
    CMP                                                                                                       \
    "v_cvt_f64_f32 v[90:91], " PIN "\n\t"                                                                   \
    "v_mul_f64 v[88:89], v[90:91], %[k2pi]\n\t"                                                           \
    "v_rndne_f64_e32 v[88:89], v[88:89]\n\t"                                                              \
    "v_fmac_f64_e32 v[90:91], %[nhpi], v[88:89]\n\t"                                                      \
    "v_mul_f64 v[92:93], v[90:91], v[90:91]\n\t"                                                        \
    "v_fma_f64 v[84:85], v[90:91], %[km], %[kj]\n\t"                                                      \
    "v_fma_f64 v[94:95], v[92:93], %[ka], %[kb]\n\t"                                                      \
    "v_mul_f64 v[88:89], v[92:93], v[84:85]\n\t"                                                        \
    "v_fma_f64 v[94:95], v[92:93], v[94:95], %[kc]\n\t"
#define QPSKLO_HEAD_CHAIN_P(PIN) QPSKLO_STEP_P_PRE("", PIN)
#define QPSKLO_HEAD_DEFERRED_P(PIN, LW, LR)                                                                    \
    QPSKLO_STEP_P_PRE(QPSKLO_CMP_P(PIN), PIN)                                                                     \
    "s_cbranch_vccnz " LW "f\n"                                                                               \
    LR ":\n\t"

#define QPSKLO_BODY_F32(PIN, POUT, DREG, WAIT, READ, QW)                                                        \
    WAIT                                                                                                      \
    "v_pk_mul_f32 v[84:85], " DREG ", v[94:95] op_sel_hi:[1,0]\n\t"                                       \
    "v_pk_mul_f32 v[88:89], " DREG ", v[96:97] op_sel:[1,0] op_sel_hi:[0,0]\n\t"                          \
    READ                                                                                                      \
    "v_pk_add_f32 v[98:99], v[84:85], v[88:89] neg_hi:[0,1]\n\t"                                        \
    QW                                                                                                        \
    "v_sub_f32_e64 v90, |v99|, |v98|\n\t"                                    \
    "v_xor_b32_e32 v92, v98, v99\n\t"                                  \
    "v_pk_mul_f32 v[86:87], %[beal], v[90:91] op_sel_hi:[1,0]\n\t"                   \
    "v_bfi_b32 v92, %[absm], 1.0, v92\n\t"                                                    \
    "v_fmac_f32_e32 v102, v92, v86\n\t"                           \
    "v_add_f32_e32 " POUT ", " PIN ", v102\n\t"                                                               \
    "v_fmac_f32_e32 " POUT ", v92, v87\n\t"                 
#define QPSKLO_BODY(PIN, POUT, DREG, WAIT, READ, QW)                                                            \
    "v_fma_f64 v[94:95], v[92:93], v[94:95], %[c2]\n\t"                                                 \
    "v_mul_f64 v[88:89], v[90:91], v[92:93]\n\t"                                                        \
    "v_fma_f64 v[94:95], v[92:93], v[94:95], %[c1]\n\t"                                                 \
    "v_fma_f64 v[96:97], v[92:93], v[96:97], %[s1]\n\t"                                                 \
    "v_fma_f64 v[94:95], v[92:93], v[94:95], 1.0\n\t"                                                   \
    "v_fmac_f64_e32 v[90:91], v[88:89], v[96:97]\n\t"                   \
    "v_cvt_f32_f64 v94, v[94:95]\n\t"                                                                      \
    "v_cvt_f32_f64 v96, v[90:91]\n\t"                                                                      \
    QPSKLO_BODY_F32(PIN, POUT, DREG, WAIT, READ, QW)

#define QPSKLO_BODY_P(PIN, POUT, DREG, WAIT, READ, QW)                                                          \
    "v_fma_f64 v[94:95], v[92:93], v[94:95], %[kd]\n\t"                                                 \
    "v_fmac_f64_e32 v[84:85], v[88:89], v[94:95]\n\t"                                                   \
    "v_cvt_f32_f64 v94, v[84:85]\n\t"                                                                      \
    "v_med3_f32 v102, v102, %[fmin], %[fmax]\n\t"                                                             \
    "v_min3_f32 v110, v110, |v98|, |v99|\n\t"                                                               \
    "v_mul_f32_dpp v96, v94, %[sg] quad_perm:[1,0,3,2] row_mask:0xf bank_mask:0xf\n\t"                      \
    QPSKLO_BODY_F32(PIN, POUT, DREG, WAIT, READ, QW)

#define QPSKLO_TAIL(POUT, FOUT, LW, LR)                                                                         \
    "v_cmp_ge_f32_e64 vcc, |" POUT "|, %[tau]\n\t"                                                            \
    "v_med3_f32 " FOUT ", v102, %[fmin], %[fmax]\n\t"                                                         \
    "v_min3_f32 v110, v110, |v98|, |v99|\n\t"                                                               \
    "s_cbranch_vccnz " LW "f\n"                                                                               \
    LR ":\n\t"

#define QPSKLO_WRAP_ONCE(P)                                                                                     \
    "v_cvt_f64_f32 v[84:85], " P "\n\t"                                                                     \
    "v_bfi_b32 v113, %[absm], v111, " P "\n\t"                                                                \
    "v_add_f64 v[84:85], v[84:85], -v[112:113]\n\t"                                                       \
    "v_cvt_f32_f64 v88, v[84:85]\n\t"                                                                      \
    "v_cndmask_b32_e32 " P ", " P ", v88, vcc\n\t"                                                           \
    "v_cmp_ge_f32_e64 vcc, |" P "|, %[tau]\n\t"                                                               \
    "s_or_b64 %[fl], %[fl], vcc\n\t"

#define QPSKLO_WRAP_HEAD(PIN, LW, LR)                                                                           \
    LW ":\n\t"                                                                                                \
    QPSKLO_WRAP_ONCE(PIN)                                                                                       \
    QPSKLO_STEP_1_PRE("", PIN)                                                                                  \
    "s_branch " LR "b\n"
#define QPSKLO_WRAP_HEAD_P(PIN, LW, LR)                                                                         \
    LW ":\n\t"                                                                                                \
    QPSKLO_WRAP_ONCE(PIN)                                                                                       \
    QPSKLO_STEP_P_PRE("", PIN)                                                                                  \
    "s_branch " LR "b\n"

#define QPSKLO_WRAP_TAIL(POUT, LW, LR)                                                                          \
    LW ":\n\t"                                                                                                \
    QPSKLO_WRAP_ONCE(POUT)                                                                                      \
    "s_branch " LR "b\n"

#define QPSKLO_WAIT0 "s_waitcnt lgkmcnt(0)\n\t"
#define QPSKLO_WAIT1 "s_waitcnt lgkmcnt(1)\n\t"
#define QPSKLO_RDA(OFF) "ds_read_b128 v[104:107], " QPSKLO_DA " offset:" QPSK_STR(OFF) "\n\t"
#define QPSKLO_RDB(OFF) "ds_read_b128 v[120:123], " QPSKLO_DA " offset:" QPSK_STR(OFF) "\n\t"
#define QPSKLO_QW(OFF) "ds_write_b128 " QPSKLO_ZA ", v[124:127] offset:" QPSK_STR(OFF) "\n\t"

#define QPSKLO_STEP_QUAD_(HD, BD, SA_LO, SA_HI, SB_LO, SB_HI, RD1, RD2, QOFF, P4, L1, L2, L3, L4)                \
    HD("v124", "1" L1, "2" L1)                                                                        \
    BD("v124", "v125", SA_LO, QPSKLO_WAIT1, RD1, "")                                                    \
    HD("v125", "1" L2, "2" L2)                                                                        \
    BD("v125", "v126", SA_HI, "", "", "")                                                             \
    HD("v126", "1" L3, "2" L3)                                                                        \
    BD("v126", "v127", SB_LO, QPSKLO_WAIT0, RD2, "")                                                    \
    HD("v127", "1" L4, "2" L4)                                                                        \
    BD("v127", P4, SB_HI, "", "", QPSKLO_QW(QOFF))
#define QPSKLO_STEP_QUAD(...) QPSKLO_STEP_QUAD_(QPSKLO_HEAD_DEFERRED, QPSKLO_BODY, __VA_ARGS__)

#define QPSKLO_DA "%[da]"
#define QPSKLO_ZA "%[za]"
__device__ __forceinline__ unsigned costas_asm_run_lo(float &phase, float &freq, unsigned &d_addr, unsigned &z_addr,
                                                   unsigned groups, float alpha, float beta, float min_freq,
                                                   float max_freq, unsigned long long &flags_out, unsigned long long ign = 0ull)
{
    unsigned long long flags, tmp;
    ign = uniform64(ign);
    const double c3 = -0x1.6c087e89a359dp-10, s2 = 0x1.1107605230bc4p-7;
    double beal;                     {
        const float2 ba = make_float2(beta, alpha);
        __builtin_memcpy(&beal, &ba, 8);
    }
    asm volatile(
        "v_mov_b32 v112, 0x54442d18\n\t"                "v_mov_b32 v111, 0x401921fb\n\t"
        "ds_read_b128 v[104:107], %[da]\n\t"
        "s_mov_b64 %[fl], 0\n\t"
        "s_waitcnt lgkmcnt(0)\n"
        "2:\n\t"
        "v_mov_b32 v114, %[p]\n\t"
        "v_mov_b32 v115, %[f]\n\t"
        "v_mov_b32 v102, %[f]\n\t"                    "v_mov_b32 v110, 0x7f800000\n\t"                "v_mov_b32 v124, %[p]\n\t"
                QPSKLO_HEAD_CHAIN("v124")
        QPSKLO_BODY("v124", "v125", "v[104:105]", QPSKLO_WAIT1, QPSKLO_RDB(16), "")
        QPSKLO_HEAD_DEFERRED("v125", "101", "201")
        QPSKLO_BODY("v125", "v126", "v[106:107]", "", "", "")
        QPSKLO_HEAD_DEFERRED("v126", "102", "202")
        QPSKLO_BODY("v126", "v127", "v[120:121]", QPSKLO_WAIT0, QPSKLO_RDA(32), "")
        QPSKLO_HEAD_DEFERRED("v127", "103", "203")
        QPSKLO_BODY("v127", "v124", "v[122:123]", "", "", QPSKLO_QW(0))
                QPSKLO_STEP_QUAD("v[104:105]", "v[106:107]", "v[120:121]", "v[122:123]", QPSKLO_RDB(48), QPSKLO_RDA(64), 16, "v124", "04", "05", "06", "07")
        QPSKLO_STEP_QUAD("v[104:105]", "v[106:107]", "v[120:121]", "v[122:123]", QPSKLO_RDB(80), QPSKLO_RDA(96), 32, "v124", "08", "09", "10", "11")
        QPSKLO_STEP_QUAD("v[104:105]", "v[106:107]", "v[120:121]", "v[122:123]", QPSKLO_RDB(112), QPSKLO_RDA(128), 48, "%[p]", "12", "13", "14", "15")
        QPSKLO_TAIL("%[p]", "%[f]", "116", "216")
        "v_cmp_eq_f32_e64 %[tm], 0, v110\n\t"
        "s_andn2_b64 %[tm], %[tm], %[ign]\n\t"           "s_or_b64 %[fl], %[fl], %[tm]\n\t"
        "s_cmp_lg_u64 %[fl], 0\n\t"
        "s_cbranch_scc1 3f\n\t"
        "v_add_u32_e32 %[da], 0x80, %[da]\n\t"
        "v_add_u32_e32 %[za], 0x40, %[za]\n\t"
        "s_sub_u32 %[ng], %[ng], 1\n\t"
        "s_cmp_lg_u32 %[ng], 0\n\t"
        "s_cbranch_scc1 2b\n\t"
        "s_branch 4f\n"
        "3:\n\t"
        "v_mov_b32 %[p], v114\n\t"
        "v_mov_b32 %[f], v115\n\t"
        "s_branch 4f\n"
        QPSKLO_WRAP_HEAD("v125", "101", "201")
        QPSKLO_WRAP_HEAD("v126", "102", "202")
        QPSKLO_WRAP_HEAD("v127", "103", "203")
        QPSKLO_WRAP_HEAD("v124", "104", "204")
        QPSKLO_WRAP_HEAD("v125", "105", "205")
        QPSKLO_WRAP_HEAD("v126", "106", "206")
        QPSKLO_WRAP_HEAD("v127", "107", "207")
        QPSKLO_WRAP_HEAD("v124", "108", "208")
        QPSKLO_WRAP_HEAD("v125", "109", "209")
        QPSKLO_WRAP_HEAD("v126", "110", "210")
        QPSKLO_WRAP_HEAD("v127", "111", "211")
        QPSKLO_WRAP_HEAD("v124", "112", "212")
        QPSKLO_WRAP_HEAD("v125", "113", "213")
        QPSKLO_WRAP_HEAD("v126", "114", "214")
        QPSKLO_WRAP_HEAD("v127", "115", "215")
        QPSKLO_WRAP_TAIL("%[p]", "116", "216")
        "4:\n\t"
        "s_waitcnt lgkmcnt(0)"
        : [p] "+v"(phase), [f] "+v"(freq), [da] "+v"(d_addr), [za] "+v"(z_addr), [ng] "+s"(groups),
          [fl] "=&s"(flags), [tm] "=&s"(tmp)
        : [c3] "v"(c3), [s2] "v"(s2), [fmax] "v"(max_freq), [beal] "v"(beal),
          [k2pi] "s"(0x1.45F306DC9C883p-1), [nhpi] "s"(-0x1.921FB54442D18p0), [c4] "s"(0x1.99343027bf8c3p-16),
          [s3] "s"(-0x1.994eb3774cf24p-13), [c2] "s"(0x1.55553e1068f19p-5), [s1] "s"(-0x1.555545995a603p-3),
          [c1] "s"(-0x1.ffffffd0c621cp-2), [fmin] "s"(min_freq), [tau] "s"(TAU_F), [absm] "s"(0x7fffffffu), [ign] "s"(ign)
        : "vcc", "scc", "memory", "v84", "v85", "v86", "v87", "v88", "v89", "v90", "v91", "v92", "v93",
          "v94", "v95", "v96", "v97", "v98", "v99", "v100", "v101", "v102", "v103", "v104", "v105", "v106",
          "v107", "v108", "v109", "v110", "v111", "v112", "v113", "v114", "v115", "v116", "v117", "v118", "v119",
          "v120", "v121", "v122", "v123", "v124", "v125", "v126", "v127");
    flags_out = flags;
    return groups;
}

#undef QPSKLO_DA
#undef QPSKLO_ZA

#define QPSKLO_DA "v116"
#define QPSKLO_ZA "v118"
#define QPSKLO_RDN "ds_read_b128 v[104:107], v108\n\t"
#define QPSKLO_RING_CR "ds_read_b32 v109, %[ra]\n\t"
#define QPSKLO_CAT_(a, b) a##b
#define QPSKLO_CAT(a, b) QPSKLO_CAT_(a, b)
#define QPSKLO_RING_ALIGN_1 ".p2align 6\n"
#define QPSKLO_RING_ALIGN_P ".p2align 6\n\ts_nop 0\n\ts_nop 0\n\ts_nop 0\n\ts_nop 0\n"
#define QPSKLO_RQ(HD, BD, ...) QPSKLO_STEP_QUAD_(HD, BD, "v[104:105]", "v[106:107]", "v[120:121]", "v[122:123]", __VA_ARGS__)
#define QPSKLO_RING_Q0(HC, HD, BD, CR)                                                                                          \
    HC("v124")                                                                                                         \
    BD("v124", "v125", "v[104:105]", QPSKLO_WAIT1, QPSKLO_RDB(16) CR, "")                                                  \
    HD("v125", "1001", "2001")                                                                                         \
    BD("v125", "v126", "v[106:107]", "", "", "")                                                                       \
    HD("v126", "1002", "2002")                                                                                         \
    BD("v126", "v127", "v[120:121]", QPSKLO_WAIT0, QPSKLO_RDA(32), "")                                                     \
    HD("v127", "1003", "2003")                                                                                         \
    BD("v127", "v124", "v[122:123]", "", "", QPSKLO_QW(0))
#define QPSKLO_RING_QN(HD, BD, B8, B4, B, CR)                                                                                   \
    QPSKLO_RQ(HD, BD, QPSKLO_RDB(B8+16) CR, QPSKLO_RDA(B8+32), B4+0, "v124", B "00", B "01", B "02", B "03")
#define QPSKLO_RING_Q4_15(HD, BD, B8, B4, B, RDLAST, PLAST)                                                                     \
    QPSKLO_RQ(HD, BD, QPSKLO_RDB(B8+48), QPSKLO_RDA(B8+64), B4+16, "v124", B "04", B "05", B "06", B "07")                \
    QPSKLO_RQ(HD, BD, QPSKLO_RDB(B8+80), QPSKLO_RDA(B8+96), B4+32, "v124", B "08", B "09", B "10", B "11")                \
    QPSKLO_RQ(HD, BD, QPSKLO_RDB(B8+112), RDLAST, B4+48, PLAST, B "12", B "13", B "14", B "15")
#define QPSKLO_RING_W1_15(WH, B)                                                                                                \
    WH("v125", "1" B "01", "2" B "01") WH("v126", "1" B "02", "2" B "02") WH("v127", "1" B "03", "2" B "03")            \
    WH("v124", "1" B "04", "2" B "04") WH("v125", "1" B "05", "2" B "05") WH("v126", "1" B "06", "2" B "06")            \
    WH("v127", "1" B "07", "2" B "07") WH("v124", "1" B "08", "2" B "08") WH("v125", "1" B "09", "2" B "09")            \
    WH("v126", "1" B "10", "2" B "10") WH("v127", "1" B "11", "2" B "11") WH("v124", "1" B "12", "2" B "12")            \
    WH("v125", "1" B "13", "2" B "13") WH("v126", "1" B "14", "2" B "14") WH("v127", "1" B "15", "2" B "15")
#define QPSKLO_RING_W0(WH, B) WH("v124", "1" B "00", "2" B "00")
#define QPSKLO_RING_POS_16 "7"
#define QPSKLO_RING_DSH_16 "7"
#define QPSKLO_RING_ZSH_16 "6"
#define QPSKLO_RING_CSH_16 "2"
#define QPSKLO_RING_INCHUNK_16 "s_and_b32 %[t0], %[k], 3\n\ts_cmp_lg_u32 %[t0], 0\n\ts_cbranch_scc1 2b\n\t"
#define QPSKLO_RING_STEPS_16(HC, HD, BD)                                                                                        \
    QPSKLO_RING_Q0(HC, HD, BD, QPSKLO_RING_CR) QPSKLO_RING_Q4_15(HD, BD, 0, 0, "0", QPSKLO_RDN, "%[p]")
#define QPSKLO_RING_WRAPS_16(WH) QPSKLO_RING_W1_15(WH, "0")
#define QPSKLO_RING_POS_32 "3"
#define QPSKLO_RING_DSH_32 "8"
#define QPSKLO_RING_ZSH_32 "7"
#define QPSKLO_RING_CSH_32 "1"
#define QPSKLO_RING_INCHUNK_32 "s_and_b32 %[t0], %[k], 1\n\ts_cmp_lg_u32 %[t0], 0\n\ts_cbranch_scc1 2b\n\t"
#define QPSKLO_RING_STEPS_32(HC, HD, BD)                                                                                        \
    QPSKLO_RING_Q0(HC, HD, BD, "") QPSKLO_RING_Q4_15(HD, BD, 0, 0, "0", QPSKLO_RDA(128), "v124")                                    \
    QPSKLO_RING_QN(HD, BD, 128, 64, "1", QPSKLO_RING_CR) QPSKLO_RING_Q4_15(HD, BD, 128, 64, "1", QPSKLO_RDN, "%[p]")
#define QPSKLO_RING_WRAPS_32(WH) QPSKLO_RING_W1_15(WH, "0") QPSKLO_RING_W0(WH, "1") QPSKLO_RING_W1_15(WH, "1")
#define QPSKLO_RING_POS_64 "1"
#define QPSKLO_RING_DSH_64 "9"
#define QPSKLO_RING_ZSH_64 "8"
#define QPSKLO_RING_CSH_64 "0"
#define QPSKLO_RING_INCHUNK_64 ""
#define QPSKLO_RING_STEPS_64(HC, HD, BD)                                                                                        \
    QPSKLO_RING_Q0(HC, HD, BD, "") QPSKLO_RING_Q4_15(HD, BD, 0, 0, "0", QPSKLO_RDA(128), "v124")                                    \
    QPSKLO_RING_QN(HD, BD, 128, 64, "1", "") QPSKLO_RING_Q4_15(HD, BD, 128, 64, "1", QPSKLO_RDA(256), "v124")                       \
    QPSKLO_RING_QN(HD, BD, 256, 128, "2", "") QPSKLO_RING_Q4_15(HD, BD, 256, 128, "2", QPSKLO_RDA(384), "v124")                     \
    QPSKLO_RING_QN(HD, BD, 384, 192, "3", QPSKLO_RING_CR) QPSKLO_RING_Q4_15(HD, BD, 384, 192, "3", QPSKLO_RDN, "%[p]")
#define QPSKLO_RING_WRAPS_64(WH)                                                                                                \
    QPSKLO_RING_W1_15(WH, "0") QPSKLO_RING_W0(WH, "1") QPSKLO_RING_W1_15(WH, "1") QPSKLO_RING_W0(WH, "2") QPSKLO_RING_W1_15(WH, "2")      \
    QPSKLO_RING_W0(WH, "3") QPSKLO_RING_W1_15(WH, "3")
#define QPSKLO_RING_TEXT(HC, HD, BD, WH, INIT, ALIGN, G)                                                                        \
    "v_mov_b32 v112, 0x54442d18\n\t"                                                    \
    "v_mov_b32 v111, 0x401921fb\n\t" INIT                                                                                   \
    "s_and_b32 %[t0], %[k], " QPSKLO_CAT(QPSKLO_RING_POS_, G) "\n\t"                                                       \
    "s_lshl_b32 %[t0], %[t0], " QPSKLO_CAT(QPSKLO_RING_DSH_, G) "\n\t"                                                     \
    "v_add_u32_e32 v116, %[t0], %[db]\n\t"                                                                             \
    "ds_read_b128 v[104:107], v116\n\t"                                                                                \
    "s_mov_b64 %[fl], 0\n\t"                                                                                           \
    "s_waitcnt lgkmcnt(0)\n"                                                                                           \
                                                                                              \
    ALIGN                                                                                                              \
    "2:\n\t"                                                                                                           \
                                                        \
    "s_and_b32 %[t0], %[k], " QPSKLO_CAT(QPSKLO_RING_POS_, G) "\n\t"                                                       \
    "s_lshl_b32 %[t1], %[t0], " QPSKLO_CAT(QPSKLO_RING_DSH_, G) "\n\t"                                                     \
    "v_add_u32_e32 v116, %[t1], %[db]\n\t"                                                                             \
    "s_lshl_b32 %[t1], %[t0], " QPSKLO_CAT(QPSKLO_RING_ZSH_, G) "\n\t"                                                     \
    "v_add_u32_e32 v118, %[t1], %[zb]\n\t"                                                                             \
    "s_add_u32 %[t0], %[k], 1\n\t"                                                                                     \
    "s_and_b32 %[t0], %[t0], " QPSKLO_CAT(QPSKLO_RING_POS_, G) "\n\t"                                                      \
    "s_lshl_b32 %[t0], %[t0], " QPSKLO_CAT(QPSKLO_RING_DSH_, G) "\n\t"                                                     \
    "v_add_u32_e32 v108, %[t0], %[db]\n\t"                                                                             \
    "v_mov_b32 v114, %[p]\n\t"                                                                                         \
    "v_mov_b32 v115, %[f]\n\t"                                                                                         \
    "v_mov_b32 v102, %[f]\n\t"                                        \
    "v_mov_b32 v110, 0x7f800000\n\t"                                                                                   \
    "v_mov_b32 v124, %[p]\n\t"                                                                                         \
                      \
    QPSKLO_CAT(QPSKLO_RING_STEPS_, G)(HC, HD, BD)                                                                          \
    QPSKLO_TAIL("%[p]", "%[f]", "1900", "2900")                                                                          \
    "v_cmp_eq_f32_e64 %[tm], 0, v110\n\t"                                                                              \
    "s_andn2_b64 %[tm], %[tm], %[ign]\n\t"    \
    "s_or_b64 %[fl], %[fl], %[tm]\n\t"                                                                                 \
    "s_cmp_lg_u64 %[fl], 0\n\t"                                                                                        \
    "s_cbranch_scc1 3f\n\t"                                                                                            \
    "s_add_u32 %[k], %[k], 1\n\t"                                                                                      \
    QPSKLO_CAT(QPSKLO_RING_INCHUNK_, G)                             \
                         \
    "s_lshr_b32 %[t0], %[k], " QPSKLO_CAT(QPSKLO_RING_CSH_, G) "\n\t"                                                      \
    "v_mov_b32 v88, %[t0]\n\t"                                                                                        \
    "s_mov_b64 %[ex], exec\n\t"                                                                                        \
    "s_mov_b64 exec, 1\n\t"                                                                                            \
    "ds_write_b32 %[ca], v88\n\t"                                                                                     \
    "s_mov_b64 exec, %[ex]\n\t"                                                                                        \
    "s_cmp_ge_u32 %[k], %[ke]\n\t"                                                                                     \
    "s_cbranch_scc1 4f\n\t"                                                                                            \
       \
    "v_cmp_le_i32_e64 %[tm], v109, %[t0]\n\t"                                                                          \
    "s_cmp_lg_u64 %[tm], 0\n\t"                                                                                        \
    "s_cbranch_scc0 2b\n\t"                                                                                            \
    "s_branch 4f\n"                                                                                                    \
    "3:\n\t"                                                                                                           \
    "v_mov_b32 %[p], v114\n\t"                                                                                         \
    "v_mov_b32 %[f], v115\n\t"                                                                                         \
    "s_branch 4f\n"                                                                                                    \
    QPSKLO_CAT(QPSKLO_RING_WRAPS_, G)(WH)                                                                                  \
    QPSKLO_WRAP_TAIL("%[p]", "1900", "2900")                                                                             \
    "4:\n\t"                                                                                                           \
    "s_waitcnt lgkmcnt(0)"

__device__ __forceinline__ void costas_asm_run_ring_lo(float &phase, float &freq, unsigned d_base, unsigned z_base,
                                                    unsigned ready_addr, unsigned consumed_addr, unsigned &k, unsigned kend,
                                                    float alpha, float beta, float min_freq, float max_freq,
                                                    unsigned long long &flags_out, unsigned long long ign = 0ull)
{
    unsigned long long flags, tmp, ex;
    ign = uniform64(ign);
    kend = __builtin_amdgcn_readfirstlane(kend);
    unsigned t0, t1;
    const double c3 = -0x1.6c087e89a359dp-10, s2 = 0x1.1107605230bc4p-7;
    double beal;
    {
        const float2 ba = make_float2(beta, alpha);
        __builtin_memcpy(&beal, &ba, 8);
    }
    asm volatile(
        QPSKLO_RING_TEXT(QPSKLO_HEAD_CHAIN, QPSKLO_HEAD_DEFERRED, QPSKLO_BODY, QPSKLO_WRAP_HEAD, "", QPSKLO_RING_ALIGN_1, COSTAS_RING_STEPS_LO)
        : [p] "+v"(phase), [f] "+v"(freq), [k] "+s"(k), [fl] "=&s"(flags), [tm] "=&s"(tmp), [ex] "=&s"(ex),
          [t0] "=&s"(t0), [t1] "=&s"(t1)
        : [db] "v"(d_base), [zb] "v"(z_base), [ra] "v"(ready_addr), [ca] "v"(consumed_addr), [ke] "s"(kend),
          [c3] "v"(c3), [s2] "v"(s2), [fmax] "v"(max_freq), [beal] "v"(beal),
          [k2pi] "s"(0x1.45F306DC9C883p-1), [nhpi] "s"(-0x1.921FB54442D18p0), [c4] "s"(0x1.99343027bf8c3p-16),
          [s3] "s"(-0x1.994eb3774cf24p-13), [c2] "s"(0x1.55553e1068f19p-5), [s1] "s"(-0x1.555545995a603p-3),
          [c1] "s"(-0x1.ffffffd0c621cp-2), [fmin] "s"(min_freq), [tau] "s"(TAU_F), [absm] "s"(0x7fffffffu), [ign] "s"(ign)
        : "vcc", "scc", "memory", "v84", "v85", "v86", "v87", "v88", "v89", "v90", "v91", "v92", "v93",
          "v94", "v95", "v96", "v97", "v98", "v99", "v100", "v101", "v102", "v103", "v104", "v105", "v106",
          "v107", "v108", "v109", "v110", "v111", "v112", "v113", "v114", "v115", "v116", "v117", "v118", "v119",
          "v120", "v121", "v122", "v123", "v124", "v125", "v126", "v127");
    flags_out = flags;
}

__device__ __forceinline__ void costas_asm_run_ring_pair_lo(float &phase, float &freq, unsigned d_base, unsigned z_base,
                                                         unsigned ready_addr, unsigned consumed_addr, unsigned &k, unsigned kend,
                                                         float alpha, float beta, float min_freq, float max_freq, bool odd,
                                                         unsigned long long &flags_out, unsigned long long ign = 0ull)
{
    unsigned long long flags, tmp, ex;
    ign = uniform64(ign);
    kend = __builtin_amdgcn_readfirstlane(kend);
    unsigned t0, t1;
        const double ka = odd ? 0.0 : 0x1.99343027bf8c3p-16, kb = odd ? -0x1.994eb3774cf24p-13 : -0x1.6c087e89a359dp-10;
    const double kc = odd ? 0x1.1107605230bc4p-7 : 0x1.55553e1068f19p-5, kd = odd ? -0x1.555545995a603p-3 : -0x1.ffffffd0c621cp-2;
    const double km = odd ? 1.0 : 0.0, kj = odd ? -0.0 : 1.0;
    const float sg = odd ? -1.0f : 1.0f;
    double beal;
    {
        const float2 ba = make_float2(beta, alpha);
        __builtin_memcpy(&beal, &ba, 8);
    }
    asm volatile(
                QPSKLO_RING_TEXT(QPSKLO_HEAD_CHAIN_P, QPSKLO_HEAD_DEFERRED_P, QPSKLO_BODY_P, QPSKLO_WRAP_HEAD_P, "v_mov_b32 v98, 1.0\n\tv_mov_b32 v99, 1.0\n\t", QPSKLO_RING_ALIGN_P, COSTAS_RING_STEPS_LO)
        : [p] "+v"(phase), [f] "+v"(freq), [k] "+s"(k), [fl] "=&s"(flags), [tm] "=&s"(tmp), [ex] "=&s"(ex),
          [t0] "=&s"(t0), [t1] "=&s"(t1)
        : [db] "v"(d_base), [zb] "v"(z_base), [ra] "v"(ready_addr), [ca] "v"(consumed_addr), [ke] "s"(kend),
          [ka] "v"(ka), [kb] "v"(kb), [kc] "v"(kc), [kd] "v"(kd), [km] "v"(km), [kj] "v"(kj), [sg] "v"(sg),
          [fmax] "v"(max_freq), [beal] "v"(beal),
          [k2pi] "s"(0x1.45F306DC9C883p-1), [nhpi] "s"(-0x1.921FB54442D18p0),
          [fmin] "s"(min_freq), [tau] "s"(TAU_F), [absm] "s"(0x7fffffffu), [ign] "s"(ign)
        : "vcc", "scc", "memory", "v84", "v85", "v86", "v87", "v88", "v89", "v90", "v91", "v92", "v93",
          "v94", "v95", "v96", "v97", "v98", "v99", "v100", "v101", "v102", "v103", "v104", "v105", "v106",
          "v107", "v108", "v109", "v110", "v111", "v112", "v113", "v114", "v115", "v116", "v117", "v118", "v119",
          "v120", "v121", "v122", "v123", "v124", "v125", "v126", "v127");
    flags_out = flags;
}
#undef QPSKLO_DA
#undef QPSKLO_ZA

}
#endif
```

qpsk_amd/csrc/kernels.h:

```cpp
#ifndef QPSK_KERNELS_H
#define QPSK_KERNELS_H

#include <hip/hip_runtime.h>
#include <stddef.h>
#include <stdint.h>

namespace qpsk {

constexpr int LOOKBACK = 128;
constexpr int LOOKAHEAD = 8;
constexpr int MAX_LDS_BYTES = 160 * 1024;
constexpr int MAX_INDEX = 7;
constexpr int STATUS_PIPE_TIMEOUT = 1;
constexpr int STATUS_PHASE_RANGE = 2;
constexpr int STATUS_NONFINITE = 3;
constexpr int STATUS_BAD_INDEX = 4;
constexpr int STATUS_EST_NONFINITE = 5;
constexpr int STATUS_SOFT_NONFINITE = 6;
constexpr int STATUS_SOFT_BAD_LAG = 7;

struct FusedArgs {
    const float2 *x;
    size_t frame_pitch;
    int nframes, frame_size, cycles, nsym;
    int G, S;
    int mixed;
    int share_simd0;
    const int32_t *index;
    int fixed_index;
    const double2 *est_tw, *est_cs;
    int32_t *index_out;
    int lean_twowin;
    int lean_dma;
    int est_waves;
    int lean_pair;
    int dbg;
    const float2 *dsrc;
    int dstride;
    const float2 *refill;
    float2 *refill_dst;
    int refill_planar;
    const int32_t *frame_list, *frame_list_count;
    const float *taps;
    const float *gains;
    int nbw;
    float min_freq, max_freq;
    double rs;
    const float *state_in;
    int seed_setters;
    float *state_out;
    uint8_t *sym;
    uint8_t *sym_pad;
    float *freq, *phase;
    float2 *costas;
    float *hz;
    int *status;
    float *carrier_state;
    float2 *carrier_tab;
    int carrier_frame;
    int data_rule;
};

size_t fused_lds_bytes(int G, int S, int cycles, int nbw);
int prepare_kernels(void);
int launch_rx_fused(const FusedArgs &a, hipStream_t s);
size_t pipe_lds_bytes(int NF, int nbw);
int pipe_frames(int NF);
int pipe_cycles(void);
int pipe_max_nf(void);
int prepare_pipe_kernel(void);
#define QPSK_UNIT_LOCAL __attribute__((visibility("hidden")))
QPSK_UNIT_LOCAL int prepare_costas_pipe(void);
QPSK_UNIT_LOCAL int prepare_rx_fused_pipe(void);
int launch_rx_fused_pipe(const FusedArgs &a, int NF, int *status, hipStream_t s);
int launch_costas_pipe(const FusedArgs &a, int NF, int *status, hipStream_t s);
size_t pipe2_lds_bytes(int G, int nwin, int nbw);
int pipe2_max_fir(void);
int pipe2_max_frames(void);
int pipe2_max_units_per_wave(void);
int pipe2_max_hw_waves(void);
unsigned long long pipe2_default_layout(int NU);
struct LayoutCount {
    int units, nwin, hw;
    bool share_simd0, valid;
};
inline LayoutCount layout_count(unsigned long long layout, int max_per_wave = pipe2_max_units_per_wave())
{
    LayoutCount n = {0, 0, 1, false, (layout & 15) == 0};
    for (int w = 1; w < 16; w++) {
        const int cw = (int)((layout >> (4 * w)) & 15);
        if (cw > max_per_wave || (cw && w >= pipe2_max_hw_waves())) n.valid = false;
        n.units += cw;
        n.nwin += cw != 0;
        if (cw) n.hw = w + 1;
        if (cw && (w == 4 || w == 8)) n.share_simd0 = true;
    }
    return n;
}
int launch_rx_pipe2(const FusedArgs &a, int G, unsigned long long layout, int *status, hipStream_t s);
QPSK_UNIT_LOCAL int prepare_rx_pipe2(void);
size_t lean_lds_bytes(int G, int nwin);
unsigned long long lean_default_layout(int NU);
bool lean_shape_ok(const FusedArgs &a, int G);
int launch_rx_lean(const FusedArgs &a, int G, unsigned long long layout, int *status, hipStream_t s);
QPSK_UNIT_LOCAL int prepare_rx_lean(void);
bool lean_est_ok(const FusedArgs &a, int G, unsigned long long layout);
bool rx_hist_shape_ok(const FusedArgs &a);
int launch_rx_hist(const FusedArgs &a, int32_t *index_true, const int32_t *hint, int32_t *mis_list, int32_t *mis_count, int *status, hipStream_t s);
int launch_index_majority(const int32_t *index, int nframes, int32_t *hint, int32_t *mis_count, int32_t *h_stats, hipStream_t s);
QPSK_UNIT_LOCAL int prepare_rx_hist(void);
int launch_rrc_fir(const float *x, const float *memory, float *y, const float *taps, int nframes, int length,
                   hipStream_t s, size_t in_pitch = 0);
int launch_rrc_fir_stream(const float *x, const float *memory, float *y, const float *taps, int nframes, int length,
                          hipStream_t s, size_t in_pitch = 0, int ncu = 0);
struct FirRuns { int ntiles, parts, tpp; };
FirRuns rrc_fir_stream_runs(int nframes, int length, int ncu);
int launch_delay_line(const float *x, float *memory, int nframes, int length, hipStream_t s);
int launch_rrc_fir_fast(const float *x, const float *memory, float *y, const float *H, const float *tw, int nframes, int length,
// ... 298 lines not shown
```

qpsk_amd/csrc/rx_hist.hip:

```cpp
#include "rx_pipe2_geom.h"
#include "costas_asm_lo.h"
#include "fir_full8s_asm.h"

namespace qpsk {

struct StreamLo {
    static constexpr int RING_GROUP = COSTAS_RING_GROUP_LO;
    template <class... A> static __device__ __forceinline__ void ring(A &&...a) { costas_asm_run_ring_lo(a...); }
    template <class... A> static __device__ __forceinline__ void ring_pair(A &&...a) { costas_asm_run_ring_pair_lo(a...); }
    template <class... A> static __device__ __forceinline__ unsigned run(A &&...a) { return costas_asm_run_lo(a...); }
};

namespace histk {
constexpr int G = 16, NSCAN = 4, NFIR = 8, UF = 2, QL = 32, R = 8;
constexpr int TILE = QL * R;
constexpr int DRO = 2, PADS = 2, WPOS = TILE + HIST, WSF = 480, PITCH = TILE + 4;
constexpr int HW_WAVES = 14;
constexpr int THREADS = 64 * HW_WAVES;
__device__ constexpr int role_of(int hw)
{
    return hw == 0 ? 12 : hw <= 3 ? hw - 1 : hw <= 11 ? hw : hw == 13 ? 3 : -1;
}
__device__ __host__ constexpr int slot_of(int p) { return p + PADS * (p / R); }
static_assert(slot_of(WPOS - 1) < WSF && WSF % 2 == 0, "window geometry (timing_scan.hip)");
static_assert(COSTAS_ASM_LO_END_VGPR <= 128, "rx_hist_kernel: four waves on SIMD 0");
struct Ctl {
    int ready[NFIR];
    int consumed[NSCAN];
    int flushed[NSCAN];
    lean::Ctl loop;
    DeferredVerdict spec;
};
static_assert(sizeof(Ctl) % 16 == 0, "the frame windows behind the control block take 16-byte stores");
}

__global__ void __launch_bounds__(histk::THREADS)
rx_hist_kernel(FusedArgs a, int32_t *index_true, const int32_t *hint, int32_t *mis_list, int32_t *mis_count, int *status)
{
    using namespace histk;
    using GM = lean::GeomLean;
    extern __shared__ __attribute__((aligned(16))) unsigned char smem_raw[];
    Ctl *sm = reinterpret_cast<Ctl *>(smem_raw);
    float2 *win = reinterpret_cast<float2 *>(smem_raw + sizeof(Ctl));
    float *ring = reinterpret_cast<float *>(win + (size_t)G * WSF);
    unsigned char *rows = reinterpret_cast<unsigned char *>(ring + (size_t)G * DRO * 2 * PITCH);
    float2 *dring = reinterpret_cast<float2 *>(rows);
    float *zring = reinterpret_cast<float *>(rows + lean::Z_OFFSET_BYTES);
    const int tid = threadIdx.x, lane = tid & 63;
    const int wave = role_of(__builtin_amdgcn_readfirstlane(tid >> 6));
    const int f0 = blockIdx.x * G;
    const int frame_size = a.frame_size, nframes = a.nframes;
    const int ntiles = frame_size / TILE, nchunks = a.nsym / pipe2::S;
    const int gi = __builtin_amdgcn_readfirstlane(hint[0]) & 7;
    int *abortf = &sm->loop.abort_flag;

    if (tid < NFIR) sm->ready[tid] = 0;
    if (tid < NSCAN) { sm->consumed[tid] = 0; sm->flushed[tid] = 0; }
    if (tid < MAX_WAVES) sm->loop.ready[tid] = 0;
    if (tid == 0) { sm->loop.consumed = 0; sm->loop.abort_flag = 0; sm->spec.done = 0; }
    __syncthreads();

    if (wave < 0) return;
    if (wave == NSCAN + NFIR) {
        costas_wave<GM, StreamLo>(a, &sm->loop, dring, zring, G, f0, lane, nchunks, status, &sm->spec);
        return;
    }
    if (wave < NSCAN) {
        __builtin_amdgcn_s_setprio(3);
        const int fl = lane >> 4, comp = (lane >> 3) & 1, q = lane & 7;
        const int g = 4 * wave + fl;
        const float qf = (float)q;
        float av = 0.0f, mx = 0.0f;
        int cum = 0, done = 0;
        bool ok = true;
        auto serve_flush = [&]() {
            const int cons = __builtin_amdgcn_readfirstlane(ld_acquire(&sm->loop.consumed));
            while (done < cons && done < nchunks) {
                if (f0 + g < nframes) flush_records<GM, 4>(a, zring, dring, g, f0 + g, lane & 15, done);
                done++;
                if (lane == 0) st_release(&sm->flushed[wave], done);
            }
        };
        for (int t = 0; t < ntiles && ok; t++) {
            int spins = 0;
            while (!__all(ld_acquire(&sm->ready[g >> 1]) >= t + 1)) {
                serve_flush();
                __builtin_amdgcn_s_sleep(2);
                if (++spins > SPIN_LIMIT || __hip_atomic_load(abortf, __ATOMIC_RELAXED, __HIP_MEMORY_SCOPE_WORKGROUP)) {
                    __hip_atomic_store(abortf, 1, __ATOMIC_RELAXED, __HIP_MEMORY_SCOPE_WORKGROUP);
                    ok = false;
// ... 208 lines not shown
```

qpsk_amd/csrc/rx_pipe.h:

```cpp
#ifndef QPSK_RX_PIPE_H
#define QPSK_RX_PIPE_H
#include <hip/hip_runtime.h>
#include <stdint.h>
#include "qpsk_device.h"
#include "costas_asm.h"
#include "kernels.h"
#include "rx_profile.h"

namespace qpsk {

namespace pipe {

constexpr int C = 8;
constexpr int DR = 2;
constexpr int MAX_WAVES = 16;
constexpr int SPIN_LIMIT = 1 << 24;

template <int QL_, int R_, int MAX_NF_, int SPARE_, bool PINNED_>
struct Geom {
    static constexpr bool PINNED = PINNED_;
    static constexpr int QL = QL_;
    static constexpr int R = R_;
    static constexpr int MAX_NF = MAX_NF_;
    static constexpr int SPARE = SPARE_;
    static constexpr int FWV = 64 / QL;
    static constexpr int S = R * QL;
    static constexpr int CH = S * C;
    static constexpr int TSTEPS = NTAPS + C * (R - 1);
    static constexpr int PAD = R * C;
    static constexpr int WL = CH + 128;
    static constexpr int WSLOTS = ((WL + 2 * (WL / (2 * C)) + 31) / 32) * 32;
    static constexpr int DSTRIDE = DR * S + 2;
    static constexpr int ZSTRIDE = DR * S + 4;
    static constexpr int MAX_THREADS = SPARE ? 512 : 64 * (MAX_NF + 1);
    static_assert(QL == 16 && 64 % QL == 0 && 128 % PAD == 0, "slot arithmetic assumes 16 lanes per frame");
};
template <int QL_, int R_>
struct WaveMap {
    static constexpr int QL = QL_, R = R_;
};
using GeomNarrow = Geom<16, 4, 4, 1, true>;

#define QPSK_GEOM_CONSTANTS(GM)                                                                          \
    constexpr int QL = GM::QL, R = GM::R, FWV = GM::FWV, S = GM::S, CH = GM::CH, WSLOTS = GM::WSLOTS,    \
                  DSTRIDE = GM::DSTRIDE, ZSTRIDE = GM::ZSTRIDE, TSTEPS = GM::TSTEPS, PAD = GM::PAD,      \
                  MAX_NF = GM::MAX_NF;                                                                   \
    (void)QL; (void)R; (void)FWV; (void)S; (void)CH; (void)WSLOTS; (void)DSTRIDE; (void)ZSTRIDE;         \
    (void)TSTEPS; (void)PAD; (void)MAX_NF

struct Smem {
    float taps[128];
    int ready[MAX_WAVES];
    int consumed;
    int abort_flag;
    int pad_[2];
    int est_index[16];
};

__device__ __forceinline__ int ld_acquire(const int *p)
{
    int v = __hip_atomic_load(p, __ATOMIC_RELAXED, __HIP_MEMORY_SCOPE_WORKGROUP);
    __builtin_amdgcn_fence(__ATOMIC_ACQUIRE, "workgroup");
    return v;
}

__device__ __forceinline__ void st_release(int *p, int v)
{
    __builtin_amdgcn_fence(__ATOMIC_RELEASE, "workgroup");
    __hip_atomic_store(p, v, __ATOMIC_RELAXED, __HIP_MEMORY_SCOPE_WORKGROUP);
}

__device__ __forceinline__ void report_status(int *status, int what)
{
    __hip_atomic_store(status, what, __ATOMIC_RELAXED, __HIP_MEMORY_SCOPE_SYSTEM);
}

__device__ __forceinline__ bool wait_ge(int *p, int target, int *abort_flag)
{
    int spins = 0;
    while (ld_acquire(p) < target) {
        __builtin_amdgcn_s_sleep(2);
        if (++spins > SPIN_LIMIT || __hip_atomic_load(abort_flag, __ATOMIC_RELAXED, __HIP_MEMORY_SCOPE_WORKGROUP)) {
            __hip_atomic_store(abort_flag, 1, __ATOMIC_RELAXED, __HIP_MEMORY_SCOPE_WORKGROUP);
            return false;
        }
    }
    return true;
}

}

using namespace pipe;

struct StreamHi {
    static constexpr int RING_GROUP = COSTAS_RING_GROUP;
    template <class... A> static __device__ __forceinline__ void ring(A &&...a) { costas_asm_run_ring(a...); }
    template <class... A> static __device__ __forceinline__ void ring_pair(A &&...a) { costas_asm_run_ring_pair(a...); }
    template <class... A> static __device__ __forceinline__ unsigned run(A &&...a) { return costas_asm_run(a...); }
};

struct DeferredVerdict {
    unsigned over[2];
    unsigned nonfinite[2];
    int done;
    int pad_[3];
};

template <class GM, class ST = StreamHi, class SM>
__device__ __forceinline__ void costas_wave(const FusedArgs &a, SM *sm, const float2 *dring, float *zring, int G,
                                            int f0, int lane, int nchunks, int *status, DeferredVerdict *defer = nullptr)
{
    QPSK_GEOM_CONSTANTS(GM);
    const int nbw = a.nbw, N = a.nsym;
    if (a.share_simd0 != ((a.dbg & 512) != 0)) __builtin_amdgcn_s_setprio(1);
    else __builtin_amdgcn_s_setprio(3);
    const bool pair = a.lean_pair != 0;
    const bool odd = pair && (lane & 1);
    const int g = pair ? lane >> 1 : lane / nbw, b = pair ? 0 : lane - g * nbw;
    const bool inwg = pair ? lane < 2 * G : lane < G * nbw;
    const bool active = inwg && f0 + g < a.nframes;
    Loop st = {0.0f, 0.0f};
    LoopGains lg = {0.0f, 0.0f, a.min_freq, a.max_freq};
    bool over = false;
    if (active) {
        lg.alpha = a.gains[2 * b];
        lg.beta = a.gains[2 * b + 1];
        if (a.state_in) {
            st.phase = a.state_in[2 * ((size_t)(f0 + g) * nbw + b)];
            st.freq = a.state_in[2 * ((size_t)(f0 + g) * nbw + b) + 1];
            if (a.seed_setters) seed_setters(st.phase, st.freq, a.min_freq, a.max_freq, over);
        }
    }
    const int gl = inwg ? g : 0;
    const int gw = a.mixed == 2 ? gl / 2 : a.mixed == 1 && gl >= 12 ? 3 + (gl - 12) / 2 : gl / FWV;
    const float2 *dl = dring + (size_t)gl * DSTRIDE;
    float *zl = zring + (size_t)(pair ? gl : lane) * ZSTRIDE;
    const bool fast_clamp = a.min_freq < 0.0f && a.max_freq > 0.0f;
    float ph = st.phase, fr = st.freq;
    auto zero_run = [&](int from, int to) {
        const uint4 *p = reinterpret_cast<const uint4 *>(dl + from);
        unsigned acc = 0;
        for (int i = 0; i < (to - from) / 2; i++) {
            const uint4 v = p[i];
            acc |= v.x | v.y | v.z | v.w;
        }
        return acc == 0u;
    };
    auto excusable = [&](unsigned long long lanes, int from, int to) {
        const bool z = ((lanes >> lane) & 1ull) != 0ull && __float_as_uint(ph) != 0x80000000u && __float_as_uint(fr) != 0x80000000u &&
                       zero_run(from, to);
        return (unsigned long long)__ballot(z);
    };
    const float al = lg.alpha, be = lg.beta, fmin_ = a.min_freq, fmax_ = a.max_freq;
    bool ok = true;
    prof::SerialProbe probe(a, lane);
    const bool ring_stream = fast_clamp && !(a.dbg & (8 | 16 | probe.chunkwise_bits())) && S == 4 * COSTAS_ASM_GROUP && DR == 2;
    const int first_ring_chunk = __any(active && __float_as_uint(ph) == 0x80000000u) ? 1 : 0;
    for (int c = 0; c < nchunks && ok; c++) {
        if (ring_stream && c >= first_ring_chunk && (c + 1) * S <= N) {
            const int cfull = N / S;
            if (active) {
                constexpr int AG = ST::RING_GROUP;
                constexpr unsigned GPC = S == 4 * COSTAS_ASM_GROUP ? (unsigned)(S / AG) : 1u, RPOS = 2u * GPC - 1u;
                unsigned k = GPC * (unsigned)c;
                const unsigned kend = GPC * (unsigned)cfull;
                const unsigned d_base = lds_addr(dl), z_base = lds_addr(zl);
                const unsigned ready_addr = lds_addr(&sm->ready[gw]), consumed_addr = lds_addr(&sm->consumed);
                unsigned long long ign = 0ull;
                while (k < kend) {
                    if ((k & (GPC - 1u)) == 0u) {
                        ok = wait_ge(&sm->ready[gw], (int)(k / GPC) + 1, &sm->abort_flag);
                        if (!__all(ok)) { ok = false; break; }
                        if (ign) {
                            const int at = (int)(k & RPOS) * AG;
                            ign = excusable(ign, at, at + S);
                        }
                    }
                    unsigned long long fl = 0ull;
                    bool ran = false;
                    if (!__any(__float_as_uint(fr) == 0x80000000u)) {
                        unsigned ks = __builtin_amdgcn_readfirstlane(k);
                        const unsigned kstop = ign ? min(kend, (ks | (GPC - 1u)) + 1u) : kend;
                        probe.enter_stream();
                        if (pair)
                            ST::ring_pair(ph, fr, d_base, z_base, ready_addr, consumed_addr, ks, kstop, al, be, fmin_, fmax_, odd, fl, ign);
                        else
                            ST::ring(ph, fr, d_base, z_base, ready_addr, consumed_addr, ks, kstop, al, be, fmin_, fmax_, fl, ign);
                        ran = true;
                        probe.leave_stream();
                        k = ks;
                    }
                    if ((!ran || fl != 0ull) && k < kend) {
                        const int at = (int)(k & RPOS) * AG;
                        const unsigned long long fresh = fl & ~ign;
                        if (ran && fresh) {
                            const unsigned long long zm = excusable(fresh, at, ((int)(k & RPOS) | (int)(GPC - 1u)) * AG + AG);
                            if ((fresh & ~zm) == 0ull) { ign |= zm; continue; }
                        }
                        for (int i = 0; i < AG; i++) {
                            float tx, ty; unsigned qq;
                            zl[at + i] = ph;
                            costas_step_t<true>(ph, fr, al, be, fmin_, fmax_, dl[at + i], tx, ty, qq, over);
                        }
                        k++;
                        if ((k & (GPC - 1u)) == 0u && lane == 0) st_release(&sm->consumed, (int)(k / GPC));
                    }
                }
            }
            ok = __all(ok);
            c = cfull - 1;
            continue;
        }
        ok = wait_ge(&sm->ready[gw], c + 1, &sm->abort_flag);
        if (!__all(ok)) { ok = false; break; }
        probe.chunk_waited(c);
        const int slot = (c % DR) * S;
        const int cnt = min(S, N - c * S);
        if (active && !QPSK_ABLATE(a, 2)) {
            int j = 0;
            if (c == 0) {
                Loop s0 = {ph, fr};
                zl[slot] = ph;
                costas_step<true>(s0, lg, dl[slot], over);
                ph = s0.phase; fr = s0.freq;
                j = 1;
                for (; j < min(4, cnt); j++) {
                    float tx, ty; unsigned qq;
                    zl[slot + j] = ph;
                    if (fast_clamp) costas_step_t<true>(ph, fr, al, be, fmin_, fmax_, dl[slot + j], tx, ty, qq, over);
                    else costas_step_t<false>(ph, fr, al, be, fmin_, fmax_, dl[slot + j], tx, ty, qq, over);
                }
            }
            if (fast_clamp && !(a.dbg & 8)) {
                constexpr int AG = COSTAS_ASM_GROUP;
                unsigned long long ign = 0ull;
                while (cnt - j >= AG) {
                    unsigned da = lds_addr(dl + slot + j), za = lds_addr(zl + slot + j);
                    unsigned long long fl = 0ull;
                    bool ran = false;
                    const unsigned want = __builtin_amdgcn_readfirstlane((unsigned)(cnt - j) / AG);
                    unsigned left = want;
                    if (!__any(__float_as_uint(fr) == 0x80000000u)) {
                        left = ST::run(ph, fr, da, za, want, al, be, fmin_, fmax_, fl, ign);
                        ran = true;
                    }
                    j += AG * (int)(want - left);
                    if (left != 0) {
                        const unsigned long long fresh = fl & ~ign;
                        if (ran && fresh) {
                            const unsigned long long zm = excusable(fresh, slot + j, slot + j + AG * (int)left);
                            if ((fresh & ~zm) == 0ull) { ign |= zm; continue; }
                        }
                        for (int i = 0; i < AG; i++, j++) {
                            float tx, ty; unsigned qq;
                            zl[slot + j] = ph;
                            costas_step_t<true>(ph, fr, al, be, fmin_, fmax_, dl[slot + j], tx, ty, qq, over);
                        }
                    }
                }
            }
            float2 dcur = dl[slot + j];
            if (fast_clamp) {
#pragma unroll 1
                for (; j < cnt; j++) {
                    const float2 dnext = dl[slot + j + 1];
                    float tx, ty; unsigned qq;
                    zl[slot + j] = ph;
                    costas_step_t<true>(ph, fr, al, be, fmin_, fmax_, dcur, tx, ty, qq, over);
                    dcur = dnext;
                }
            } else {
#pragma unroll 4
                for (; j < cnt; j++) {
                    const float2 dnext = dl[slot + j + 1];
                    float tx, ty; unsigned qq;
                    zl[slot + j] = ph;
                    costas_step_t<false>(ph, fr, al, be, fmin_, fmax_, dcur, tx, ty, qq, over);
                    dcur = dnext;
                }
            }
        }
        if (lane == 0) st_release(&sm->consumed, c + 1);
        probe.chunk_done();
    }
    probe.finish(nchunks, S);
    st.phase = ph; st.freq = fr;
    if (active && ok && !odd) {
        const size_t o = (size_t)(f0 + g) * nbw + b;
        if (a.freq) a.freq[o] = st.freq;
        if (a.phase) a.phase[o] = st.phase;
// ... 79 lines not shown
```

qpsk_amd/lib.py:

```python
import ctypes as C
import os
import subprocess

import numpy as np

HERE = os.path.dirname(os.path.abspath(__file__))
TAU = 2.0 * 3.14159265358979323846
TIMING_HIST, TIMING_FIXED, TIMING_FFT = 0, 1, 2
OUTER_POLARITY, OUTER_MSB_FIRST = 1, 2
DISPERSAL_MSB_FIRST = 1
NTAPS = 127


class QpskError(RuntimeError):
    pass


class Params(C.Structure):
    _fields_ = [("fs", C.c_double), ("rs", C.c_double), ("frame_size", C.c_int), ("rrc_alpha", C.c_float),
                ("loop_bw", C.c_float), ("min_freq", C.c_float), ("max_freq", C.c_float),
                ("timing_mode", C.c_int), ("fixed_index", C.c_int)]


def lib_path():
    return os.environ.get("QPSK_HIP_LIB") or os.path.join(HERE, "libqpsk_hip.so")


def build(verbose=False):
    cmd = ["make", "-C", os.path.join(HERE, "csrc")]
    if not verbose:
        cmd.insert(1, "-s")
    subprocess.check_call(cmd)
    return lib_path()


_LIB = None

API_SYMBOLS = [
    "qpsk_last_error", "qpsk_version", "qpsk_device_count", "qpsk_params_default", "qpsk_ctx_create",
    "qpsk_ctx_destroy", "qpsk_ctx_sync", "qpsk_ctx_set_stream", "qpsk_ctx_set_tuning", "qpsk_ctx_cycles", "qpsk_ctx_nsym",
    "qpsk_ctx_last_kernel",
    "qpsk_ctx_get_taps", "qpsk_ctx_get_gains", "qpsk_ctx_set_taps", "qpsk_ctx_set_loop", "qpsk_rx_batch", "qpsk_rx_batch_pitched",
    "qpsk_rx_batch_bw", "qpsk_rrc_fir_batch", "qpsk_rrc_fir_batch_fast", "qpsk_timing_hist_batch", "qpsk_timing_scan_batch", "qpsk_timing_fft_batch", "qpsk_timing_fft_bin_batch", "qpsk_costas_batch", "qpsk_fft_batch",
    "qpsk_streams_reset", "qpsk_streams_set_loop_state", "qpsk_streams_get_loop_state", "qpsk_streams_rx_cplx",
    "qpsk_streams_rx_pcm", "qpsk_streams_rx_pcm_host", "qpsk_dev_alloc", "qpsk_dev_free", "qpsk_dev_upload", "qpsk_dev_download",
    "qpsk_selftest_sincos_hash", "qpsk_crc16_batch", "qpsk_interleave_batch", "qpsk_scramble_batch",
    "qpsk_tx_reset", "qpsk_tx_symbols", "qpsk_test_inject_status", "qpsk_test_hist_state", "qpsk_ctx_check",
    "qpsk_multi_create", "qpsk_multi_destroy", "qpsk_multi_shards", "qpsk_multi_load", "qpsk_multi_shard", "qpsk_multi_use_device_input",
    "qpsk_multi_rx_begin", "qpsk_multi_rx_end", "qpsk_multi_set_direct_output", "qpsk_host_alloc", "qpsk_host_free",
    "qpsk_multi_set_packed", "qpsk_pack_symbols", "qpsk_unpack_symbols_host",
    "qpsk_rx_batch_ext", "qpsk_rx_batch_bw_ext", "qpsk_multi_set_acquisition", "qpsk_carrier_est_batch",
    "qpsk_rx_batch_data", "qpsk_sync_batch", "qpsk_multi_set_data", "qpsk_deframer_reset", "qpsk_deframer_push",
    "qpsk_deframer_reset_coded", "qpsk_deframer_push_coded",
    "qpsk_soft_batch", "qpsk_conv_encode_batch", "qpsk_viterbi_batch",
    "qpsk_punct_ntx", "qpsk_conv_encode_punct_batch", "qpsk_viterbi_punct_batch", "qpsk_deframer_reset_coded_punct",
    "qpsk_test_viterbi_launches", "qpsk_test_deframer_advance", "qpsk_test_fir_runs",
    "qpsk_frame_len", "qpsk_frame_batch",
    "qpsk_ilv_stride", "qpsk_conv_encode_ilv_batch", "qpsk_viterbi_ilv_batch", "qpsk_frame_batch_ilv", "qpsk_deframer_reset_coded_ilv",
    "qpsk_rs_generator", "qpsk_rs_encode_batch", "qpsk_rs_decode_batch",
    "qpsk_viterbi_stream_reset", "qpsk_viterbi_stream_emits", "qpsk_viterbi_stream_push", "qpsk_viterbi_stream_flush",
    "qpsk_conv_encode_stream_batch", "qpsk_test_viterbi_stream_advance",
    "qpsk_outer_reset", "qpsk_outer_max_words", "qpsk_outer_push", "qpsk_outer_interleave_batch", "qpsk_test_outer_advance",
    "qpsk_nodesync_reset", "qpsk_nodesync_shifts", "qpsk_nodesync_push", "qpsk_nodesync_set",
    "qpsk_outer_reset_group", "qpsk_dispersal_batch", "qpsk_dispersal_sequence",
]
PUNCTURE = {"1/2": (1, 0x1, 0x1), "2/3": (2, 0x1, 0x3), "3/4": (3, 0x5, 0x3), "5/6": (5, 0x15, 0x0B), "7/8": (7, 0x51, 0x2F)}


def _pattern(puncture):
    if isinstance(puncture, str):
        if puncture not in PUNCTURE:
            raise ValueError("puncture must be one of %s or a (period, keep0, keep1) tuple" % sorted(PUNCTURE))
        puncture = PUNCTURE[puncture]
    period, keep0, keep1 = puncture
    return int(period), int(keep0), int(keep1)
DROPIN_SYMBOLS = [
    "qpsk_dropin_configure", "qpsk_dropin_set_device", "qpsk_dropin_shutdown", "rrc_fir", "rrc_make",
    "create_control_loop", "phase_detector", "update_gains", "advance_loop", "phase_wrap", "frequency_limit",
    "set_loop_bandwidth", "set_damping_factor", "set_alpha", "set_beta", "set_frequency", "set_phase",
    "set_max_freq", "set_min_freq", "get_loop_bandwidth", "get_damping_factor", "get_alpha", "get_beta",
    "get_frequency", "get_phase", "get_max_freq", "get_min_freq", "fft", "fftn", "ifft", "ifftn", "qpsk_demod",
    "rx_frame", "qpsk_dropin_costas_frame", "qpsk_dropin_symbols", "qpsk_dropin_offset_freq",
    "qpsk_dropin_timing_index",
]


def load():
    global _LIB
    if _LIB is not None:
        return _LIB
    p = lib_path()
    if not os.path.exists(p):
        raise QpskError("%s is missing: run `python -c 'import __graft_entry__ as g; g.build()'` "
                        "(there is no CPU fallback)" % p)
    try:
        import torch
    except ImportError:
        pass
    L = C.CDLL(p)
    vp, i32, f32 = C.c_void_p, C.c_int, C.c_float
    L.qpsk_last_error.restype = C.c_char_p
    L.qpsk_version.restype = C.c_char_p
    L.qpsk_params_default.argtypes = [C.POINTER(Params)]
    L.qpsk_ctx_create.argtypes = [C.POINTER(vp), i32, C.POINTER(Params), vp]
    L.qpsk_ctx_destroy.argtypes = [vp]
    L.qpsk_ctx_destroy.restype = None
    L.qpsk_ctx_sync.argtypes = [vp]
    L.qpsk_ctx_set_stream.argtypes = [vp, vp]
    L.qpsk_ctx_set_tuning.argtypes = [vp, C.c_char_p, i32]
    L.qpsk_ctx_cycles.argtypes = [vp]
    L.qpsk_ctx_nsym.argtypes = [vp]
    L.qpsk_ctx_last_kernel.argtypes = [vp]
    L.qpsk_ctx_last_kernel.restype = C.c_char_p
    L.qpsk_ctx_get_taps.argtypes = [vp, C.POINTER(f32)]
    L.qpsk_ctx_get_gains.argtypes = [vp, C.POINTER(f32), C.POINTER(f32)]
    L.qpsk_ctx_set_taps.argtypes = [vp, C.POINTER(f32)]
    L.qpsk_ctx_set_loop.argtypes = [vp, f32, f32, f32, f32]
    L.qpsk_rx_batch.argtypes = [vp, vp, i32, vp, vp, vp, vp, vp, vp]
    L.qpsk_rx_batch_pitched.argtypes = [vp, vp, C.c_longlong, i32, vp, vp, vp, vp, vp, vp]
    L.qpsk_rx_batch_bw.argtypes = [vp, vp, i32, C.POINTER(f32), i32, vp, vp, vp, vp]
    L.qpsk_rx_batch_ext.argtypes = [vp, vp, C.c_longlong, i32, vp, vp, vp, vp, vp, vp, vp, vp]
    L.qpsk_rx_batch_bw_ext.argtypes = [vp, vp, i32, C.POINTER(f32), i32, vp, vp, vp, vp, vp, vp]
    L.qpsk_multi_set_acquisition.argtypes = [vp, vp, vp]
    L.qpsk_carrier_est_batch.argtypes = [vp, vp, C.c_longlong, i32, i32, i32, vp, vp, vp, vp]
    L.qpsk_rx_batch_data.argtypes = [vp, vp, C.c_longlong, i32, vp, vp, vp, vp, vp, vp, vp, vp]
    L.qpsk_sync_batch.argtypes = [vp, vp, i32, i32, vp, i32, i32, i32, i32, vp, vp, vp, vp]
    L.qpsk_multi_set_data.argtypes = [vp, i32]
    L.qpsk_deframer_reset.argtypes = [vp, i32, vp, i32, i32, i32, i32]
    L.qpsk_deframer_push.argtypes = [vp, vp, vp, i32, vp, vp, vp, vp, vp, vp]
    L.qpsk_deframer_reset_coded.argtypes = [vp, i32, vp, i32, i32, i32, i32, i32, f32]
    L.qpsk_deframer_push_coded.argtypes = [vp, vp, i32, vp, vp, vp, vp, vp, vp, vp, vp]
    L.qpsk_soft_batch.argtypes = [vp, vp, C.c_longlong, i32, i32, i32, i32, f32, vp, vp, vp, i32, i32, vp, vp, vp]
    L.qpsk_conv_encode_batch.argtypes = [vp, vp, i32, i32, i32, vp]
    L.qpsk_viterbi_batch.argtypes = [vp, vp, C.c_longlong, i32, i32, vp, i32, vp, vp]
    u32 = C.c_uint32
    L.qpsk_punct_ntx.argtypes = [i32, i32, u32, u32]
    L.qpsk_conv_encode_punct_batch.argtypes = [vp, vp, i32, i32, i32, i32, u32, u32, vp]
    L.qpsk_viterbi_punct_batch.argtypes = [vp, vp, C.c_longlong, i32, i32, i32, u32, u32, vp, i32, vp, vp]
    L.qpsk_deframer_reset_coded_punct.argtypes = [vp, i32, vp, i32, i32, i32, i32, i32, f32, i32, u32, u32]
    L.qpsk_frame_len.argtypes = [i32, i32, i32, i32, u32, u32]
    L.qpsk_frame_batch.argtypes = [vp, vp, C.c_longlong, i32, i32, i32, vp, i32, i32, i32, u32, u32, i32, i32, i32, vp, vp]
    L.qpsk_ilv_stride.argtypes = [i32, i32]
    L.qpsk_conv_encode_ilv_batch.argtypes = [vp, vp, i32, i32, i32, i32, u32, u32, i32, vp]
    L.qpsk_viterbi_ilv_batch.argtypes = [vp, vp, C.c_longlong, i32, i32, i32, u32, u32, i32, vp, i32, vp, vp]
    L.qpsk_frame_batch_ilv.argtypes = [vp, vp, C.c_longlong, i32, i32, i32, vp, i32, i32, i32, u32, u32, i32, i32, i32, i32, vp, vp]
    L.qpsk_deframer_reset_coded_ilv.argtypes = [vp, i32, vp, i32, i32, i32, i32, i32, f32, i32, u32, u32, i32]
    L.qpsk_rs_generator.argtypes = [i32, vp]
    L.qpsk_rs_encode_batch.argtypes = [vp, vp, C.c_longlong, i32, i32, i32, vp, C.c_longlong]
    L.qpsk_rs_decode_batch.argtypes = [vp, vp, C.c_longlong, i32, i32, i32, vp, vp, C.c_longlong, vp]
    L.qpsk_rrc_fir_batch.argtypes = [vp, vp, vp, vp, i32, i32]
    L.qpsk_rrc_fir_batch_fast.argtypes = [vp, vp, vp, vp, i32, i32]
    L.qpsk_timing_hist_batch.argtypes = [vp, vp, i32, vp, vp]
    L.qpsk_timing_fft_batch.argtypes = [vp, vp, i32, vp, vp, vp]
    L.qpsk_timing_fft_bin_batch.argtypes = [vp, vp, i32, vp, vp, vp]
    L.qpsk_timing_scan_batch.argtypes = [vp, vp, i32, vp, vp]
    L.qpsk_costas_batch.argtypes = [vp, vp, i32, i32, vp, vp, vp]
    L.qpsk_fft_batch.argtypes = [vp, vp, vp, i32, i32, i32]
    L.qpsk_streams_reset.argtypes = [vp, i32, C.c_double]
    L.qpsk_streams_set_loop_state.argtypes = [vp, C.POINTER(f32)]
    L.qpsk_streams_get_loop_state.argtypes = [vp, C.POINTER(f32)]
    L.qpsk_streams_rx_cplx.argtypes = [vp, vp, vp, vp, vp, vp, vp]
    L.qpsk_streams_rx_pcm.argtypes = [vp, vp, vp, vp, vp, vp, vp]
    L.qpsk_streams_rx_pcm_host.argtypes = [vp, vp, vp, vp, vp, vp]
    L.qpsk_selftest_sincos_hash.argtypes = [vp, C.c_uint32, C.c_uint32, C.POINTER(C.c_ulonglong)]
    L.qpsk_test_inject_status.argtypes = [vp, i32]
    L.qpsk_ctx_check.argtypes = [vp]
    L.qpsk_test_hist_state.argtypes = [vp, C.POINTER(i32)]
    L.qpsk_test_viterbi_launches.argtypes = [vp, C.POINTER(i32)]
    L.qpsk_test_deframer_advance.argtypes = [vp, C.c_longlong]
    L.qpsk_viterbi_stream_reset.argtypes = [vp, i32, i32, i32, i32, u32, u32]
    L.qpsk_viterbi_stream_emits.argtypes = [vp, i32]
    L.qpsk_viterbi_stream_push.argtypes = [vp, vp, C.c_longlong, i32, vp, C.c_longlong, vp, C.POINTER(i32)]
    L.qpsk_viterbi_stream_flush.argtypes = [vp, i32, vp, C.c_longlong, vp, C.POINTER(i32)]
    L.qpsk_conv_encode_stream_batch.argtypes = [vp, vp, i32, i32, i32, u32, u32, vp, vp, vp]
    L.qpsk_test_viterbi_stream_advance.argtypes = [vp, C.c_longlong]
    L.qpsk_outer_reset.argtypes = [vp, i32, i32, i32, i32, i32, i32, i32]
    L.qpsk_outer_reset_group.argtypes = [vp, i32, i32, i32, i32, i32, i32, i32, i32]
    L.qpsk_dispersal_batch.argtypes = [vp, vp, C.c_longlong, i32, i32, i32, i32, vp, i32, vp, C.c_longlong]
    L.qpsk_dispersal_sequence.argtypes = [i32, i32, i32, vp]
    L.qpsk_outer_max_words.argtypes = [vp, i32]
    L.qpsk_outer_push.argtypes = [vp, vp, C.c_longlong, i32, i32, vp, vp, C.c_longlong, vp, vp, vp]
    L.qpsk_outer_interleave_batch.argtypes = [vp, vp, i32, i32, i32, i32, vp, vp, vp]
    L.qpsk_test_outer_advance.argtypes = [vp, C.c_longlong]
    L.qpsk_nodesync_reset.argtypes = [vp, i32, i32, i32, i32, i32, i32, i32, i32]
    L.qpsk_nodesync_shifts.argtypes = [i32, u32, u32]
    L.qpsk_nodesync_push.argtypes = [vp, vp, C.c_longlong, i32, vp, vp, C.c_longlong, vp]
    L.qpsk_nodesync_set.argtypes = [vp, vp]
    L.qpsk_test_fir_runs.argtypes = [vp, i32, i32, C.POINTER(i32)]
    L.qpsk_multi_create.argtypes = [C.POINTER(vp), C.POINTER(i32), i32, C.POINTER(Params)]
    L.qpsk_multi_destroy.argtypes = [vp]
    L.qpsk_multi_destroy.restype = None
    L.qpsk_multi_shards.argtypes = [vp]
    L.qpsk_multi_load.argtypes = [vp, C.c_longlong, vp]
    L.qpsk_multi_shard.argtypes = [vp, i32, C.POINTER(i32), C.POINTER(C.c_longlong), C.POINTER(C.c_longlong), C.POINTER(vp), C.POINTER(vp)]
    L.qpsk_multi_use_device_input.argtypes = [vp, i32, vp]
    L.qpsk_multi_set_direct_output.argtypes = [vp, i32, vp, vp, vp]
    L.qpsk_multi_set_packed.argtypes = [vp, i32]
    L.qpsk_pack_symbols.argtypes = [vp, vp, C.c_longlong, i32, vp]
    L.qpsk_unpack_symbols_host.argtypes = [vp, C.c_longlong, i32, vp]
    L.qpsk_host_alloc.argtypes = [C.POINTER(vp), C.c_size_t]
    L.qpsk_host_free.argtypes = [vp]
    L.qpsk_multi_rx_begin.argtypes = [vp, i32]
    L.qpsk_multi_rx_end.argtypes = [vp, i32, vp, vp, vp]
    L.qpsk_crc16_batch.argtypes = [vp, vp, i32, i32, vp]
    L.qpsk_interleave_batch.argtypes = [vp, vp, i32, i32, i32]
    L.qpsk_scramble_batch.argtypes = [vp, vp, i32, i32]
    L.qpsk_tx_reset.argtypes = [vp, i32, C.c_double]
    L.qpsk_tx_symbols.argtypes = [vp, vp, i32, vp, vp]
    _LIB = L
    return L


def version():
    return load().qpsk_version().decode()


FRAME_UNCODED, FRAME_CODED = 0, 1


def _coding(coded, puncture):
    if not coded:
        return (FRAME_UNCODED, 1, 1, 1)
    return (FRAME_CODED,) + _pattern("1/2" if puncture is None else puncture)


def frame_len(nsync, nbytes, coded=True, puncture=None):
    L = load()
    rc = L.qpsk_frame_len(int(nsync), int(nbytes), *_coding(coded, puncture))
    if rc < 0:
        raise QpskError("libqpsk_hip error %d: %s" % (rc, L.qpsk_last_error().decode()))
    return rc


def ilv_stride(nbits, want):
    L = load()
    rc = L.qpsk_ilv_stride(int(nbits), int(want))
    if rc < 0:
        raise QpskError("libqpsk_hip error %d: %s" % (rc, L.qpsk_last_error().decode()))
    return rc


def rs_generator(nroots):
    L = load()
    g = np.zeros(max(int(nroots), 0) + 1, np.uint8)
    rc = L.qpsk_rs_generator(int(nroots), g.ctypes.data_as(C.c_void_p))
    if rc < 0:
        raise QpskError("libqpsk_hip error %d: %s" % (rc, L.qpsk_last_error().decode()))
    return g


def dispersal_sequence(len=188, group=8, msb_first=False):
    L = load()
    out = np.zeros(max(int(group) * int(len), 1), np.uint8)
    rc = L.qpsk_dispersal_sequence(int(len), int(group), DISPERSAL_MSB_FIRST if msb_first else 0, out.ctypes.data_as(C.c_void_p))
    if rc < 0:
        raise QpskError("libqpsk_hip error %d: %s" % (rc, L.qpsk_last_error().decode()))
    return out[:rc].tobytes()


def nodesync_shifts(puncture):
    L = load()
    rc = L.qpsk_nodesync_shifts(*_pattern(puncture))
    if rc < 0:
        raise QpskError("libqpsk_hip error %d: %s" % (rc, L.qpsk_last_error().decode()))
    return rc


def _interleaved(interleave):
    return interleave is not None and int(interleave) != 1


def _ptr(t):
    return None if t is None else C.c_void_p(t.data_ptr())


class Modem:

    def __init__(self, fs=9600.0, rs=2400.0, frame_size=512, rrc_alpha=0.35, loop_bw=np.float32(TAU / 100.0),
                 min_freq=-1.0, max_freq=1.0, timing_mode=TIMING_HIST, fixed_index=0, device=None, stream="torch"):
        import torch
        self.torch = torch
        self.L = load()
        if not torch.cuda.is_available():
            raise QpskError("no GPU visible to torch; libqpsk_hip has no CPU path")
        self.device = torch.cuda.current_device() if device is None else int(device)
        self.dev = torch.device("cuda", self.device)
        self.params = Params(fs, rs, frame_size, rrc_alpha, loop_bw, min_freq, max_freq, timing_mode, fixed_index)
        if stream == "torch":
            s = C.c_void_p(torch.cuda.current_stream(self.dev).cuda_stream)
        elif stream is None:
            s = None
        else:
            s = C.c_void_p(int(stream))
        h = C.c_void_p()
        self._check(self.L.qpsk_ctx_create(C.byref(h), self.device, C.byref(self.params), s))
        self.h = h
        self.cycles = self.L.qpsk_ctx_cycles(h)
        self.nsym = self.L.qpsk_ctx_nsym(h)
        self.frame_size = frame_size
        self.nstreams = 0
        self._vs_streams = 0
        self._outer = None
        self._ns_links = 0

    def _check(self, rc):
        if rc != 0:
            raise QpskError("libqpsk_hip error %d: %s" % (rc, self.L.qpsk_last_error().decode()))

    def close(self):
        if getattr(self, "h", None):
            self.L.qpsk_ctx_destroy(self.h)
            self.h = None

    def __del__(self):
        try:
            self.close()
        except Exception:
            pass

    def sync(self, data=None, sync=None, lag_min=0, lag_max=0, nout=0):
        if data is None:
            self._check(self.L.qpsk_ctx_sync(self.h))
            return None
        return self._sync_search(data, sync, lag_min, lag_max, nout)

    def last_kernel(self):
        return self.L.qpsk_ctx_last_kernel(self.h).decode()

    def tune(self, **kw):
        for k, v in kw.items():
            self._check(self.L.qpsk_ctx_set_tuning(self.h, ("QPSK_" + k.upper()).encode(), -1 if v is None else int(v)))

    def viterbi_launches(self):
        n = C.c_int(-1)
        self._check(self.L.qpsk_test_viterbi_launches(self.h, C.byref(n)))
        return n.value

    def deframer_advance(self, delta):
        self._check(self.L.qpsk_test_deframer_advance(self.h, int(delta)))

    def fir_runs(self, nframes, length):
        out = (C.c_int * 3)()
        self._check(self.L.qpsk_test_fir_runs(self.h, int(nframes), int(length), out))
        return tuple(out)

    def set_stream(self, stream):
        s = None if stream is None else C.c_void_p(getattr(stream, "cuda_stream", stream))
        self._check(self.L.qpsk_ctx_set_stream(self.h, s))

    @property
    def taps(self):
        t = (C.c_float * NTAPS)()
        self._check(self.L.qpsk_ctx_get_taps(self.h, t))
        return np.array(t, np.float32)

    @property
    def gains(self):
        a, b = C.c_float(), C.c_float()
        self._check(self.L.qpsk_ctx_get_gains(self.h, C.byref(a), C.byref(b)))
        return np.float32(a.value), np.float32(b.value)

    def set_taps(self, taps):
        t = (C.c_float * NTAPS)(*[float(x) for x in taps])
        self._check(self.L.qpsk_ctx_set_taps(self.h, t))

    def set_loop(self, alpha, beta, min_freq, max_freq):
        self._check(self.L.qpsk_ctx_set_loop(self.h, alpha, beta, min_freq, max_freq))

    def _dev(self, a, dtype):
        t = self.torch
        if isinstance(a, np.ndarray):
            a = t.from_numpy(np.ascontiguousarray(a))
        a = a.to(self.dev)
        assert a.dtype == dtype, (a.dtype, dtype)
        return a.contiguous()

    def empty(self, shape, dtype):
        return self.torch.empty(shape, dtype=dtype, device=self.dev)

    def rx_batch(self, frames, want_costas=False, out=None):
        t = self.torch
        x = self._dev(frames, t.float32)
        F = x.shape[0]
        assert x.shape[1] == self.frame_size and x.shape[2] == 2
        o = out or dict(sym=self.empty((F, self.nsym), t.uint8), freq=self.empty((F,), t.float32),
                        phase=self.empty((F,), t.float32), index=self.empty((F,), t.int32),
                        hz=self.empty((F,), t.float32),
                        costas=self.empty((F, self.nsym, 2), t.float32) if want_costas else None)
        self._check(self.L.qpsk_rx_batch(self.h, _ptr(x), F, _ptr(o["sym"]), _ptr(o["freq"]), _ptr(o["phase"]),
                                         _ptr(o.get("costas")), _ptr(o.get("index")), _ptr(o.get("hz"))))
        return o

    def rx_batch_raw(self, x, F, sym, freq, phase, pitch=0, index=None):
        if pitch:
            rc = self.L.qpsk_rx_batch_pitched(self.h, _ptr(x), pitch, F, _ptr(sym), _ptr(freq), _ptr(phase), None, _ptr(index), None)
        else:
            rc = self.L.qpsk_rx_batch(self.h, _ptr(x), F, _ptr(sym), _ptr(freq), _ptr(phase), None, _ptr(index), None)
        if rc:
            self._check(rc)

    def rx_batch_bw(self, frames, loop_bws):
        t = self.torch
        x = self._dev(frames, t.float32)
        F, B = x.shape[0], len(loop_bws)
        bws = (C.c_float * B)(*[float(b) for b in loop_bws])
        o = dict(sym=self.empty((F, B, self.nsym), t.uint8), freq=self.empty((F, B), t.float32),
                 phase=self.empty((F, B), t.float32), index=self.empty((F,), t.int32))
        self._check(self.L.qpsk_rx_batch_bw(self.h, _ptr(x), F, bws, B, _ptr(o["sym"]), _ptr(o["freq"]),
                                            _ptr(o["phase"]), _ptr(o["index"])))
        return o

    def rx_batch_ext(self, frames, index=None, seed=None, want_costas=False, pitch=0):
        t = self.torch
        x = self._dev(frames, t.float32)
        F = x.shape[0]
# ... 704 lines not shown
```

Measured before the change: 453,600.

## Add adaptive branch-free phase-wrap Costas ring mode with wrap statistics

```diff
diff --git a/include/qpsk_hip.h b/include/qpsk_hip.h
--- a/include/qpsk_hip.h
+++ b/include/qpsk_hip.h
@@ -240,6 +240,7 @@
 
 int qpsk_test_inject_status(qpsk_ctx *ctx, int code);
 int qpsk_test_hist_state(qpsk_ctx *ctx, int32_t *out);
+int qpsk_test_wrap_stats(qpsk_ctx *ctx, uint32_t out[4]);
 int qpsk_test_fir_runs(qpsk_ctx *ctx, int nframes, int length, int32_t out[3]);
 int qpsk_test_viterbi_launches(qpsk_ctx *ctx, int *out);
 int qpsk_test_deframer_advance(qpsk_ctx *ctx, long long delta);
diff --git a/qpsk_amd/csrc/api_ctx.cpp b/qpsk_amd/csrc/api_ctx.cpp
--- a/qpsk_amd/csrc/api_ctx.cpp
+++ b/qpsk_amd/csrc/api_ctx.cpp
@@ -24,6 +24,7 @@
     {"QPSK_STREAM_SCAN", &Tuning::stream_scan}, {"QPSK_STREAM_CARRIER", &Tuning::stream_carrier},
     {"QPSK_LEAN_DMA", &Tuning::lean_dma},     {"QPSK_LEAN_PAIR", &Tuning::lean_pair},
     {"QPSK_EST_WAVES", &Tuning::est_waves},   {"QPSK_HIST_ONEPASS", &Tuning::hist_onepass},
+    {"QPSK_WRAP_BF", &Tuning::wrap_bf},
     {"QPSK_VITERBI_LDS", &Tuning::viterbi_lds},   {"QPSK_VITERBI_CHUNK_ROWS", &Tuning::viterbi_chunk_rows},
 };
 
@@ -230,7 +231,7 @@
     hipFree(c->d_gains);
     if (c->status.h_status) hipHostFree(c->status.h_status);
     if (c->streams.h_done) hipHostFree(c->streams.h_done);
-    for (DevBuf *b : {&c->index, &c->filtered, &c->mixed, &c->keystream, &c->sympad, &c->mislist, &c->datacostas, &c->vitdec, &c->softgain, &c->dfstage})
+    for (DevBuf *b : {&c->index, &c->filtered, &c->mixed, &c->keystream, &c->sympad, &c->mislist, &c->datacostas, &c->vitdec, &c->softgain, &c->dfstage, &c->wrapstats})
         b->release();
     for (auto &kv : c->twiddles) hipFree(kv.second);
     hipFree(c->d_fast);
diff --git a/qpsk_amd/csrc/api_ctx.h b/qpsk_amd/csrc/api_ctx.h
--- a/qpsk_amd/csrc/api_ctx.h
+++ b/qpsk_amd/csrc/api_ctx.h
@@ -62,6 +62,7 @@
     int hist_onepass = -1;
     int est_waves = -1;
     int lean_pair = -1;
+    int wrap_bf = -1;
     int viterbi_lds = -1;
     int fft_fused = -1;
     int viterbi_chunk_rows = -1;
@@ -189,6 +190,7 @@
     qpsk::DevBuf datacostas;
     qpsk::DevBuf vitdec;
     qpsk::DevBuf softgain;
+    qpsk::DevBuf wrapstats;
     qpsk::DevBuf dfstage;
     int keystream_len = 0;
     std::map<int, double *> twiddles;
diff --git a/qpsk_amd/csrc/api_rx.cpp b/qpsk_amd/csrc/api_rx.cpp
--- a/qpsk_amd/csrc/api_rx.cpp
+++ b/qpsk_amd/csrc/api_rx.cpp
@@ -29,6 +29,18 @@
     if (nframes < 1 || length < 1) return fail(QPSK_ERR_ARG, "qpsk_test_fir_runs: nframes %d length %d", nframes, length);
     const FirRuns r = rrc_fir_stream_runs(nframes, length, c->ncu);
     out[0] = r.ntiles; out[1] = r.parts; out[2] = r.tpp;
+    return QPSK_OK;
+}
+
+int qpsk_test_wrap_stats(qpsk_ctx *c, uint32_t out[4])
+{
+    if (!c || !out) return fail(QPSK_ERR_ARG, "qpsk_test_wrap_stats: null argument");
+    out[0] = out[1] = out[2] = out[3] = 0u;
+    if (bind(c)) return QPSK_ERR_HIP;
+    HIP_TRY(hipStreamSynchronize(c->stream));
+    if (c->wrapstats.p) HIP_TRY(hipMemcpy(out, c->wrapstats.p, 4 * sizeof(uint32_t), hipMemcpyDeviceToHost));
+    else if (int rc = ensure(c, c->wrapstats, 4 * sizeof(uint32_t))) return rc;
+    HIP_TRY(hipMemset(c->wrapstats.p, 0, 4 * sizeof(uint32_t)));
     return QPSK_OK;
 }
 
@@ -347,6 +359,8 @@
     a.lean_twowin = tuned(c->tune.lean_dma, 1) != 2 ? 1 : 0;
     a.est_waves = tuned(c->tune.est_waves, 0);
     a.lean_pair = tuned(c->tune.lean_pair, 3);
+    a.wrap_mode = tuned(c->tune.wrap_bf, 2);
+    a.wrap_stats = static_cast<unsigned *>(c->wrapstats.p);
     a.taps = c->d_taps;
     a.gains = c->d_gains;
     a.nbw = nbw;
@@ -559,6 +573,8 @@
         a.carrier_frame = c->prm.frame_size;
     }
     a.dbg = tuned(c->tune.pipe_variant, 0) & PIPE_VARIANT_MASK;
+    a.wrap_mode = tuned(c->tune.wrap_bf, 2);
+    a.wrap_stats = static_cast<unsigned *>(c->wrapstats.p);
     int nf = (nframes + c->ncu * pipe_frames(1) - 1) / (c->ncu * pipe_frames(1));
     if (nf < 1) nf = 1;
     if (nf > pipe_max_nf()) nf = pipe_max_nf();
diff --git a/qpsk_amd/csrc/costas_asm.h b/qpsk_amd/csrc/costas_asm.h
--- a/qpsk_amd/csrc/costas_asm.h
+++ b/qpsk_amd/csrc/costas_asm.h
@@ -136,6 +136,23 @@
     QPSK_STEP_P_PRE("", PIN)                                                                                  \
     "s_branch " LR "b\n"
 
+#define QPSK_WRAP_COUNT                                                                                       \
+    "s_add_u32 %[wc], %[wc], 1\n\t"                                                                           \
+    "s_cmp_ge_u32 %[wc], %[wt]\n\t"                                                                           \
+    "s_cmov_b32 %[ke], 0\n\t"
+#define QPSK_WRAP_HEAD_CNT(PIN, LW, LR)                                                                       \
+    LW ":\n\t"                                                                                                \
+    QPSK_WRAP_COUNT                                                                                           \
+    QPSK_WRAP_ONCE(PIN)                                                                                       \
+    QPSK_STEP_1_PRE("", PIN)                                                                                  \
+    "s_branch " LR "b\n"
+#define QPSK_WRAP_HEAD_P_CNT(PIN, LW, LR)                                                                     \
+    LW ":\n\t"                                                                                                \
+    QPSK_WRAP_COUNT                                                                                           \
+    QPSK_WRAP_ONCE(PIN)                                                                                       \
+    QPSK_STEP_P_PRE("", PIN)                                                                                  \
+    "s_branch " LR "b\n"
+
 #define QPSK_WRAP_TAIL(POUT, LW, LR)                                                                          \
     LW ":\n\t"                                                                                                \
     QPSK_WRAP_ONCE(POUT)                                                                                      \
@@ -145,7 +162,9 @@
 #define QPSK_WAIT1 "s_waitcnt lgkmcnt(1)\n\t"
 #define QPSK_RDA(OFF) "ds_read_b128 v[120:123], " QPSK_DA " offset:" QPSK_STR(OFF) "\n\t"
 #define QPSK_RDB(OFF) "ds_read_b128 v[136:139], " QPSK_DA " offset:" QPSK_STR(OFF) "\n\t"
-#define QPSK_QW(OFF) "ds_write_b128 " QPSK_ZA ", v[140:143] offset:" QPSK_STR(OFF) "\n\t"
+#define QPSK_QW(OFF) "ds_write_b128 " QPSK_ZA ", v[140:143] offset:" QPSK_STR(OFF) "\n\t" QPSK_QUAD_SEEN
+#define QPSK_QUAD_SEEN ""
+#define QPSK_BLOCK_SEEN ""
 
 #define QPSK_STEP_QUAD_(HD, BD, SA_LO, SA_HI, SB_LO, SB_HI, RD1, RD2, QOFF, P4, L1, L2, L3, L4)                \
     HD("v140", "1" L1, "2" L1)                                                                        \
@@ -265,7 +284,7 @@
     HD("v143", "1003", "2003")                                                                                         \
     BD("v143", "v140", "v[138:139]", "", "", QPSK_QW(0))
 #define QPSK_RING_QN(HD, BD, B8, B4, B, CR)                                                                                   \
-    QPSK_RQ(HD, BD, QPSK_RDB(B8+16) CR, QPSK_RDA(B8+32), B4+0, "v140", B "00", B "01", B "02", B "03")
+    QPSK_RQ(HD, BD, QPSK_RDB(B8+16) CR QPSK_BLOCK_SEEN, QPSK_RDA(B8+32), B4+0, "v140", B "00", B "01", B "02", B "03")
 #define QPSK_RING_Q4_15(HD, BD, B8, B4, B, RDLAST, PLAST)                                                                     \
     QPSK_RQ(HD, BD, QPSK_RDB(B8+48), QPSK_RDA(B8+64), B4+16, "v140", B "04", B "05", B "06", B "07")                \
     QPSK_RQ(HD, BD, QPSK_RDB(B8+80), QPSK_RDA(B8+96), B4+32, "v140", B "08", B "09", B "10", B "11")                \
@@ -307,7 +326,7 @@
 #define QPSK_RING_WRAPS_64(WH)                                                                                                \
     QPSK_RING_W1_15(WH, "0") QPSK_RING_W0(WH, "1") QPSK_RING_W1_15(WH, "1") QPSK_RING_W0(WH, "2") QPSK_RING_W1_15(WH, "2")      \
     QPSK_RING_W0(WH, "3") QPSK_RING_W1_15(WH, "3")
-#define QPSK_RING_TEXT(HC, HD, BD, WH, INIT, ALIGN, G)                                                                        \
+#define QPSK_RING_TEXT(HC, HD, BD, WH, INIT, ALIGN, G, GEND)                                                                      \
     "v_mov_b32 v128, 0x54442d18\n\t"                                                    \
     "v_mov_b32 v127, 0x401921fb\n\t" INIT                                                                                   \
     "s_and_b32 %[t0], %[k], " QPSK_CAT(QPSK_RING_POS_, G) "\n\t"                                                       \
@@ -337,6 +356,7 @@
                       \
     QPSK_CAT(QPSK_RING_STEPS_, G)(HC, HD, BD)                                                                          \
     QPSK_TAIL("%[p]", "%[f]", "1900", "2900")                                                                          \
+    GEND                                                                                                               \
     "v_cmp_eq_f32_e64 %[tm], 0, v126\n\t"                                                                              \
     "s_andn2_b64 %[tm], %[tm], %[ign]\n\t"    \
     "s_or_b64 %[fl], %[fl], %[tm]\n\t"                                                                                 \
@@ -344,6 +364,7 @@
     "s_cbranch_scc1 3f\n\t"                                                                                            \
     "s_add_u32 %[k], %[k], 1\n\t"                                                                                      \
     QPSK_CAT(QPSK_RING_INCHUNK_, G)                             \
+    "s_mov_b32 %[wc], 0\n\t"                            \
                          \
     "s_lshr_b32 %[t0], %[k], " QPSK_CAT(QPSK_RING_CSH_, G) "\n\t"                                                      \
     "v_mov_b32 v104, %[t0]\n\t"                                                                                        \
@@ -370,12 +391,14 @@
 __device__ __forceinline__ void costas_asm_run_ring(float &phase, float &freq, unsigned d_base, unsigned z_base,
                                                     unsigned ready_addr, unsigned consumed_addr, unsigned &k, unsigned kend,
                                                     float alpha, float beta, float min_freq, float max_freq,
-                                                    unsigned long long &flags_out, unsigned long long ign = 0ull)
+                                                    unsigned long long &flags_out, unsigned long long ign, unsigned wrap_limit,
+                                                    bool &wrap_tripped)
 {
     unsigned long long flags, tmp, ex;
     ign = uniform64(ign);
     kend = __builtin_amdgcn_readfirstlane(kend);
-    unsigned t0, t1;
+    wrap_limit = __builtin_amdgcn_readfirstlane(wrap_limit);
+    unsigned t0, t1, wc = 0;
     const double c3 = -0x1.6c087e89a359dp-10, s2 = 0x1.1107605230bc4p-7;
     double beal;
     {
@@ -383,10 +406,10 @@
         __builtin_memcpy(&beal, &ba, 8);
     }
     asm volatile(
-        QPSK_RING_TEXT(QPSK_HEAD_CHAIN, QPSK_HEAD_DEFERRED, QPSK_BODY, QPSK_WRAP_HEAD, "", QPSK_RING_ALIGN_1, COSTAS_RING_STEPS)
+        QPSK_RING_TEXT(QPSK_HEAD_CHAIN, QPSK_HEAD_DEFERRED, QPSK_BODY, QPSK_WRAP_HEAD_CNT, "", QPSK_RING_ALIGN_1, COSTAS_RING_STEPS, "")
         : [p] "+v"(phase), [f] "+v"(freq), [k] "+s"(k), [fl] "=&s"(flags), [tm] "=&s"(tmp), [ex] "=&s"(ex),
-          [t0] "=&s"(t0), [t1] "=&s"(t1)
-        : [db] "v"(d_base), [zb] "v"(z_base), [ra] "v"(ready_addr), [ca] "v"(consumed_addr), [ke] "s"(kend),
+          [t0] "=&s"(t0), [t1] "=&s"(t1), [wc] "+s"(wc), [ke] "+s"(kend)
+        : [db] "v"(d_base), [zb] "v"(z_base), [ra] "v"(ready_addr), [ca] "v"(consumed_addr), [wt] "s"(wrap_limit),
           [c3] "v"(c3), [s2] "v"(s2), [fmax] "v"(max_freq), [beal] "v"(beal),
           [k2pi] "s"(0x1.45F306DC9C883p-1), [nhpi] "s"(-0x1.921FB54442D18p0), [c4] "s"(0x1.99343027bf8c3p-16),
           [s3] "s"(-0x1.994eb3774cf24p-13), [c2] "s"(0x1.55553e1068f19p-5), [s1] "s"(-0x1.555545995a603p-3),
@@ -396,17 +419,20 @@
           "v123", "v124", "v125", "v126", "v127", "v128", "v129", "v130", "v131", "v132", "v133", "v134", "v135",
           "v136", "v137", "v138", "v139", "v140", "v141", "v142", "v143");
     flags_out = flags;
+    wrap_tripped = kend == 0u;
 }
 
 __device__ __forceinline__ void costas_asm_run_ring_pair(float &phase, float &freq, unsigned d_base, unsigned z_base,
                                                          unsigned ready_addr, unsigned consumed_addr, unsigned &k, unsigned kend,
                                                          float alpha, float beta, float min_freq, float max_freq, bool odd,
-                                                         unsigned long long &flags_out, unsigned long long ign = 0ull)
+                                                         unsigned long long &flags_out, unsigned long long ign, unsigned wrap_limit,
+                                                         bool &wrap_tripped)
 {
     unsigned long long flags, tmp, ex;
     ign = uniform64(ign);
     kend = __builtin_amdgcn_readfirstlane(kend);
-    unsigned t0, t1;
+    wrap_limit = __builtin_amdgcn_readfirstlane(wrap_limit);
+    unsigned t0, t1, wc = 0;
     const double ka = odd ? 0.0 : 0x1.99343027bf8c3p-16, kb = odd ? -0x1.994eb3774cf24p-13 : -0x1.6c087e89a359dp-10;
     const double kc = odd ? 0x1.1107605230bc4p-7 : 0x1.55553e1068f19p-5, kd = odd ? -0x1.555545995a603p-3 : -0x1.ffffffd0c621cp-2;
     const double km = odd ? 1.0 : 0.0, kj = odd ? -0.0 : 1.0;
@@ -417,10 +443,10 @@
         __builtin_memcpy(&beal, &ba, 8);
     }
     asm volatile(
-        QPSK_RING_TEXT(QPSK_HEAD_CHAIN_P, QPSK_HEAD_DEFERRED_P, QPSK_BODY_P, QPSK_WRAP_HEAD_P, "v_mov_b32 v114, 1.0\n\tv_mov_b32 v115, 1.0\n\t", QPSK_RING_ALIGN_P, COSTAS_RING_STEPS)
+        QPSK_RING_TEXT(QPSK_HEAD_CHAIN_P, QPSK_HEAD_DEFERRED_P, QPSK_BODY_P, QPSK_WRAP_HEAD_P_CNT, "v_mov_b32 v114, 1.0\n\tv_mov_b32 v115, 1.0\n\t", QPSK_RING_ALIGN_P, COSTAS_RING_STEPS, "")
         : [p] "+v"(phase), [f] "+v"(freq), [k] "+s"(k), [fl] "=&s"(flags), [tm] "=&s"(tmp), [ex] "=&s"(ex),
-          [t0] "=&s"(t0), [t1] "=&s"(t1)
-        : [db] "v"(d_base), [zb] "v"(z_base), [ra] "v"(ready_addr), [ca] "v"(consumed_addr), [ke] "s"(kend),
+          [t0] "=&s"(t0), [t1] "=&s"(t1), [wc] "+s"(wc), [ke] "+s"(kend)
+        : [db] "v"(d_base), [zb] "v"(z_base), [ra] "v"(ready_addr), [ca] "v"(consumed_addr), [wt] "s"(wrap_limit),
           [ka] "v"(ka), [kb] "v"(kb), [kc] "v"(kc), [kd] "v"(kd), [km] "v"(km), [kj] "v"(kj), [sg] "v"(sg),
           [fmax] "v"(max_freq), [beal] "v"(beal),
           [k2pi] "s"(0x1.45F306DC9C883p-1), [nhpi] "s"(-0x1.921FB54442D18p0),
@@ -430,6 +456,7 @@
           "v123", "v124", "v125", "v126", "v127", "v128", "v129", "v130", "v131", "v132", "v133", "v134", "v135",
           "v136", "v137", "v138", "v139", "v140", "v141", "v142", "v143");
     flags_out = flags;
+    wrap_tripped = kend == 0u;
 }
 #undef QPSK_DA
 #undef QPSK_ZA
diff --git a/qpsk_amd/csrc/costas_asm_bf.h b/qpsk_amd/csrc/costas_asm_bf.h
--- /dev/null
+++ b/qpsk_amd/csrc/costas_asm_bf.h
@@ -0,0 +1,105 @@
+#ifndef QPSK_COSTAS_ASM_BF_H
+#define QPSK_COSTAS_ASM_BF_H
+
+#include "costas_asm.h"
+
+namespace qpsk {
+
+#define QPSK_WRAP_INLINE(PIN)                                                                                 \
+    QPSK_CMP_P(PIN)                                                                                           \
+    "v_cvt_f64_f32 v[106:107], " PIN "\n\t"                                                                   \
+    "v_bfi_b32 v129, %[absm], v127, " PIN "\n\t"                                                              \
+    "v_add_f64 v[100:101], v[106:107], -v[128:129]\n\t"                                                       \
+    "v_cvt_f32_f64 v104, v[100:101]\n\t"                                                                      \
+    "v_cndmask_b32_e32 " PIN ", " PIN ", v104, vcc\n\t"
+#define QPSK_HEAD_INLINE(PIN, LW, LR) QPSK_WRAP_INLINE(PIN) QPSK_STEP_1_PRE("", PIN)
+#define QPSK_HEAD_INLINE_P(PIN, LW, LR) QPSK_WRAP_INLINE(PIN) QPSK_STEP_P_PRE("", PIN)
+#define QPSK_WRAP_NONE(PIN, LW, LR)
+#define QPSK_GROUP_END_BF                                                                                     \
+    "v_cmp_ge_f32_e64 vcc, v117, %[tau]\n\t"                                                                  \
+    "s_or_b64 %[fl], %[fl], vcc\n\t"
+#define QPSK_INIT_BF "v_mov_b32 v117, 0\n\t"
+
+#define QPSK_DA "v132"
+#define QPSK_ZA "v134"
+#undef QPSK_QUAD_SEEN
+#define QPSK_QUAD_SEEN "v_max3_f32 v117, |v140|, |v141|, v117\n\tv_max3_f32 v117, |v142|, |v143|, v117\n\t"
+#undef QPSK_BLOCK_SEEN
+#define QPSK_BLOCK_SEEN "s_cmp_lg_u64 vcc, 0\n\ts_addc_u32 %[ws], %[ws], 0\n\t"
+
+__device__ __forceinline__ void costas_asm_run_ring_bf(float &phase, float &freq, unsigned d_base, unsigned z_base,
+                                                       unsigned ready_addr, unsigned consumed_addr, unsigned &k, unsigned kend,
+                                                       float alpha, float beta, float min_freq, float max_freq,
+                                                       unsigned long long &flags_out, unsigned long long ign, unsigned &seen)
+{
+    unsigned long long flags, tmp, ex;
+    ign = uniform64(ign);
+    kend = __builtin_amdgcn_readfirstlane(kend);
+    unsigned t0, t1, wc = 0, ws = __builtin_amdgcn_readfirstlane(seen);
+    const double c3 = -0x1.6c087e89a359dp-10, s2 = 0x1.1107605230bc4p-7;
+    double beal;
+    {
+        const float2 ba = make_float2(beta, alpha);
+        __builtin_memcpy(&beal, &ba, 8);
+    }
+    asm volatile(
+        QPSK_RING_TEXT(QPSK_HEAD_CHAIN, QPSK_HEAD_INLINE, QPSK_BODY, QPSK_WRAP_NONE, QPSK_INIT_BF, QPSK_RING_ALIGN_1, COSTAS_RING_STEPS, QPSK_GROUP_END_BF)
+        : [p] "+v"(phase), [f] "+v"(freq), [k] "+s"(k), [fl] "=&s"(flags), [tm] "=&s"(tmp), [ex] "=&s"(ex),
+          [t0] "=&s"(t0), [t1] "=&s"(t1), [wc] "+s"(wc), [ws] "+s"(ws)
+        : [db] "v"(d_base), [zb] "v"(z_base), [ra] "v"(ready_addr), [ca] "v"(consumed_addr), [ke] "s"(kend),
+          [c3] "v"(c3), [s2] "v"(s2), [fmax] "v"(max_freq), [beal] "v"(beal),
+          [k2pi] "s"(0x1.45F306DC9C883p-1), [nhpi] "s"(-0x1.921FB54442D18p0), [c4] "s"(0x1.99343027bf8c3p-16),
+          [s3] "s"(-0x1.994eb3774cf24p-13), [c2] "s"(0x1.55553e1068f19p-5), [s1] "s"(-0x1.555545995a603p-3),
+          [c1] "s"(-0x1.ffffffd0c621cp-2), [fmin] "s"(min_freq), [tau] "s"(TAU_F), [absm] "s"(0x7fffffffu), [ign] "s"(ign)
+        : "vcc", "scc", "memory", "v100", "v101", "v102", "v103", "v104", "v105", "v106", "v107", "v108", "v109",
+          "v110", "v111", "v112", "v113", "v114", "v115", "v116", "v117", "v118", "v119", "v120", "v121", "v122",
+          "v123", "v124", "v125", "v126", "v127", "v128", "v129", "v130", "v131", "v132", "v133", "v134", "v135",
+          "v136", "v137", "v138", "v139", "v140", "v141", "v142", "v143");
+    flags_out = flags;
+    seen = ws;
+}
+
+__device__ __forceinline__ void costas_asm_run_ring_pair_bf(float &phase, float &freq, unsigned d_base, unsigned z_base,
+                                                            unsigned ready_addr, unsigned consumed_addr, unsigned &k, unsigned kend,
+                                                            float alpha, float beta, float min_freq, float max_freq, bool odd,
+                                                            unsigned long long &flags_out, unsigned long long ign, unsigned &seen)
+{
+    unsigned long long flags, tmp, ex;
+    ign = uniform64(ign);
+    kend = __builtin_amdgcn_readfirstlane(kend);
+    unsigned t0, t1, wc = 0, ws = __builtin_amdgcn_readfirstlane(seen);
+    const double ka = odd ? 0.0 : 0x1.99343027bf8c3p-16, kb = odd ? -0x1.994eb3774cf24p-13 : -0x1.6c087e89a359dp-10;
+    const double kc = odd ? 0x1.1107605230bc4p-7 : 0x1.55553e1068f19p-5, kd = odd ? -0x1.555545995a603p-3 : -0x1.ffffffd0c621cp-2;
+    const double km = odd ? 1.0 : 0.0, kj = odd ? -0.0 : 1.0;
+    const float sg = odd ? -1.0f : 1.0f;
+    double beal;
+    {
+        const float2 ba = make_float2(beta, alpha);
+        __builtin_memcpy(&beal, &ba, 8);
+    }
+    asm volatile(
+        QPSK_RING_TEXT(QPSK_HEAD_CHAIN_P, QPSK_HEAD_INLINE_P, QPSK_BODY_P, QPSK_WRAP_NONE, "v_mov_b32 v114, 1.0\n\tv_mov_b32 v115, 1.0\n\t" QPSK_INIT_BF, QPSK_RING_ALIGN_P, COSTAS_RING_STEPS, QPSK_GROUP_END_BF)
+        : [p] "+v"(phase), [f] "+v"(freq), [k] "+s"(k), [fl] "=&s"(flags), [tm] "=&s"(tmp), [ex] "=&s"(ex),
+          [t0] "=&s"(t0), [t1] "=&s"(t1), [wc] "+s"(wc), [ws] "+s"(ws)
+        : [db] "v"(d_base), [zb] "v"(z_base), [ra] "v"(ready_addr), [ca] "v"(consumed_addr), [ke] "s"(kend),
+          [ka] "v"(ka), [kb] "v"(kb), [kc] "v"(kc), [kd] "v"(kd), [km] "v"(km), [kj] "v"(kj), [sg] "v"(sg),
+          [fmax] "v"(max_freq), [beal] "v"(beal),
+          [k2pi] "s"(0x1.45F306DC9C883p-1), [nhpi] "s"(-0x1.921FB54442D18p0),
+          [fmin] "s"(min_freq), [tau] "s"(TAU_F), [absm] "s"(0x7fffffffu), [ign] "s"(ign)
+        : "vcc", "scc", "memory", "v100", "v101", "v102", "v103", "v104", "v105", "v106", "v107", "v108", "v109",
+          "v110", "v111", "v112", "v113", "v114", "v115", "v116", "v117", "v118", "v119", "v120", "v121", "v122",
+          "v123", "v124", "v125", "v126", "v127", "v128", "v129", "v130", "v131", "v132", "v133", "v134", "v135",
+          "v136", "v137", "v138", "v139", "v140", "v141", "v142", "v143");
+    flags_out = flags;
+    seen = ws;
+}
+
+#undef QPSK_QUAD_SEEN
+#define QPSK_QUAD_SEEN ""
+#undef QPSK_BLOCK_SEEN
+#define QPSK_BLOCK_SEEN ""
+#undef QPSK_DA
+#undef QPSK_ZA
+
+}
+#endif
diff --git a/qpsk_amd/csrc/costas_asm_lo.h b/qpsk_amd/csrc/costas_asm_lo.h
--- a/qpsk_amd/csrc/costas_asm_lo.h
+++ b/qpsk_amd/csrc/costas_asm_lo.h
@@ -111,6 +111,23 @@
     QPSKLO_STEP_P_PRE("", PIN)                                                                                  \
     "s_branch " LR "b\n"
 
+#define QPSKLO_WRAP_COUNT                                                                                       \
+    "s_add_u32 %[wc], %[wc], 1\n\t"                                                                           \
+    "s_cmp_ge_u32 %[wc], %[wt]\n\t"                                                                           \
+    "s_cmov_b32 %[ke], 0\n\t"
+#define QPSKLO_WRAP_HEAD_CNT(PIN, LW, LR)                                                                       \
+    LW ":\n\t"                                                                                                \
+    QPSKLO_WRAP_COUNT                                                                                           \
+    QPSKLO_WRAP_ONCE(PIN)                                                                                       \
+    QPSKLO_STEP_1_PRE("", PIN)                                                                                  \
+    "s_branch " LR "b\n"
+#define QPSKLO_WRAP_HEAD_P_CNT(PIN, LW, LR)                                                                     \
+    LW ":\n\t"                                                                                                \
+    QPSKLO_WRAP_COUNT                                                                                           \
+    QPSKLO_WRAP_ONCE(PIN)                                                                                       \
+    QPSKLO_STEP_P_PRE("", PIN)                                                                                  \
+    "s_branch " LR "b\n"
+
 #define QPSKLO_WRAP_TAIL(POUT, LW, LR)                                                                          \
     LW ":\n\t"                                                                                                \
     QPSKLO_WRAP_ONCE(POUT)                                                                                      \
@@ -120,7 +137,9 @@
 #define QPSKLO_WAIT1 "s_waitcnt lgkmcnt(1)\n\t"
 #define QPSKLO_RDA(OFF) "ds_read_b128 v[104:107], " QPSKLO_DA " offset:" QPSK_STR(OFF) "\n\t"
 #define QPSKLO_RDB(OFF) "ds_read_b128 v[120:123], " QPSKLO_DA " offset:" QPSK_STR(OFF) "\n\t"
-#define QPSKLO_QW(OFF) "ds_write_b128 " QPSKLO_ZA ", v[124:127] offset:" QPSK_STR(OFF) "\n\t"
+#define QPSKLO_QW(OFF) "ds_write_b128 " QPSKLO_ZA ", v[124:127] offset:" QPSK_STR(OFF) "\n\t" QPSKLO_QUAD_SEEN
+#define QPSKLO_QUAD_SEEN ""
+#define QPSKLO_BLOCK_SEEN ""
 
 #define QPSKLO_STEP_QUAD_(HD, BD, SA_LO, SA_HI, SB_LO, SB_HI, RD1, RD2, QOFF, P4, L1, L2, L3, L4)                \
     HD("v124", "1" L1, "2" L1)                                                                        \
@@ -235,7 +254,7 @@
     HD("v127", "1003", "2003")                                                                                         \
     BD("v127", "v124", "v[122:123]", "", "", QPSKLO_QW(0))
 #define QPSKLO_RING_QN(HD, BD, B8, B4, B, CR)                                                                                   \
-    QPSKLO_RQ(HD, BD, QPSKLO_RDB(B8+16) CR, QPSKLO_RDA(B8+32), B4+0, "v124", B "00", B "01", B "02", B "03")
+    QPSKLO_RQ(HD, BD, QPSKLO_RDB(B8+16) CR QPSKLO_BLOCK_SEEN, QPSKLO_RDA(B8+32), B4+0, "v124", B "00", B "01", B "02", B "03")
 #define QPSKLO_RING_Q4_15(HD, BD, B8, B4, B, RDLAST, PLAST)                                                                     \
     QPSKLO_RQ(HD, BD, QPSKLO_RDB(B8+48), QPSKLO_RDA(B8+64), B4+16, "v124", B "04", B "05", B "06", B "07")                \
     QPSKLO_RQ(HD, BD, QPSKLO_RDB(B8+80), QPSKLO_RDA(B8+96), B4+32, "v124", B "08", B "09", B "10", B "11")                \
@@ -277,7 +296,7 @@
 #define QPSKLO_RING_WRAPS_64(WH)                                                                                                \
     QPSKLO_RING_W1_15(WH, "0") QPSKLO_RING_W0(WH, "1") QPSKLO_RING_W1_15(WH, "1") QPSKLO_RING_W0(WH, "2") QPSKLO_RING_W1_15(WH, "2")      \
     QPSKLO_RING_W0(WH, "3") QPSKLO_RING_W1_15(WH, "3")
-#define QPSKLO_RING_TEXT(HC, HD, BD, WH, INIT, ALIGN, G)                                                                        \
+#define QPSKLO_RING_TEXT(HC, HD, BD, WH, INIT, ALIGN, G, GEND)                                                                      \
     "v_mov_b32 v112, 0x54442d18\n\t"                                                    \
     "v_mov_b32 v111, 0x401921fb\n\t" INIT                                                                                   \
     "s_and_b32 %[t0], %[k], " QPSKLO_CAT(QPSKLO_RING_POS_, G) "\n\t"                                                       \
@@ -307,6 +326,7 @@
                       \
     QPSKLO_CAT(QPSKLO_RING_STEPS_, G)(HC, HD, BD)                                                                          \
     QPSKLO_TAIL("%[p]", "%[f]", "1900", "2900")                                                                          \
+    GEND                                                                                                               \
     "v_cmp_eq_f32_e64 %[tm], 0, v110\n\t"                                                                              \
     "s_andn2_b64 %[tm], %[tm], %[ign]\n\t"    \
     "s_or_b64 %[fl], %[fl], %[tm]\n\t"                                                                                 \
@@ -314,6 +334,7 @@
     "s_cbranch_scc1 3f\n\t"                                                                                            \
     "s_add_u32 %[k], %[k], 1\n\t"                                                                                      \
     QPSKLO_CAT(QPSKLO_RING_INCHUNK_, G)                             \
+    "s_mov_b32 %[wc], 0\n\t"                            \
                          \
     "s_lshr_b32 %[t0], %[k], " QPSKLO_CAT(QPSKLO_RING_CSH_, G) "\n\t"                                                      \
     "v_mov_b32 v88, %[t0]\n\t"                                                                                        \
@@ -340,12 +361,14 @@
 __device__ __forceinline__ void costas_asm_run_ring_lo(float &phase, float &freq, unsigned d_base, unsigned z_base,
                                                     unsigned ready_addr, unsigned consumed_addr, unsigned &k, unsigned kend,
                                                     float alpha, float beta, float min_freq, float max_freq,
-                                                    unsigned long long &flags_out, unsigned long long ign = 0ull)
+                                                    unsigned long long &flags_out, unsigned long long ign, unsigned wrap_limit,
+                                                    bool &wrap_tripped)
 {
     unsigned long long flags, tmp, ex;
     ign = uniform64(ign);
     kend = __builtin_amdgcn_readfirstlane(kend);
-    unsigned t0, t1;
+    wrap_limit = __builtin_amdgcn_readfirstlane(wrap_limit);
+    unsigned t0, t1, wc = 0;
     const double c3 = -0x1.6c087e89a359dp-10, s2 = 0x1.1107605230bc4p-7;
     double beal;
     {
@@ -353,10 +376,10 @@
         __builtin_memcpy(&beal, &ba, 8);
     }
     asm volatile(
-        QPSKLO_RING_TEXT(QPSKLO_HEAD_CHAIN, QPSKLO_HEAD_DEFERRED, QPSKLO_BODY, QPSKLO_WRAP_HEAD, "", QPSKLO_RING_ALIGN_1, COSTAS_RING_STEPS_LO)
+        QPSKLO_RING_TEXT(QPSKLO_HEAD_CHAIN, QPSKLO_HEAD_DEFERRED, QPSKLO_BODY, QPSKLO_WRAP_HEAD_CNT, "", QPSKLO_RING_ALIGN_1, COSTAS_RING_STEPS_LO, "")
         : [p] "+v"(phase), [f] "+v"(freq), [k] "+s"(k), [fl] "=&s"(flags), [tm] "=&s"(tmp), [ex] "=&s"(ex),
-          [t0] "=&s"(t0), [t1] "=&s"(t1)
-        : [db] "v"(d_base), [zb] "v"(z_base), [ra] "v"(ready_addr), [ca] "v"(consumed_addr), [ke] "s"(kend),
+          [t0] "=&s"(t0), [t1] "=&s"(t1), [wc] "+s"(wc), [ke] "+s"(kend)
+        : [db] "v"(d_base), [zb] "v"(z_base), [ra] "v"(ready_addr), [ca] "v"(consumed_addr), [wt] "s"(wrap_limit),
           [c3] "v"(c3), [s2] "v"(s2), [fmax] "v"(max_freq), [beal] "v"(beal),
           [k2pi] "s"(0x1.45F306DC9C883p-1), [nhpi] "s"(-0x1.921FB54442D18p0), [c4] "s"(0x1.99343027bf8c3p-16),
           [s3] "s"(-0x1.994eb3774cf24p-13), [c2] "s"(0x1.55553e1068f19p-5), [s1] "s"(-0x1.555545995a603p-3),
@@ -366,17 +389,20 @@
           "v107", "v108", "v109", "v110", "v111", "v112", "v113", "v114", "v115", "v116", "v117", "v118", "v119",
           "v120", "v121", "v122", "v123", "v124", "v125", "v126", "v127");
     flags_out = flags;
+    wrap_tripped = kend == 0u;
 }
 
 __device__ __forceinline__ void costas_asm_run_ring_pair_lo(float &phase, float &freq, unsigned d_base, unsigned z_base,
                                                          unsigned ready_addr, unsigned consumed_addr, unsigned &k, unsigned kend,
                                                          float alpha, float beta, float min_freq, float max_freq, bool odd,
-                                                         unsigned long long &flags_out, unsigned long long ign = 0ull)
+                                                         unsigned long long &flags_out, unsigned long long ign, unsigned wrap_limit,
+                                                         bool &wrap_tripped)
 {
     unsigned long long flags, tmp, ex;
     ign = uniform64(ign);
     kend = __builtin_amdgcn_readfirstlane(kend);
-    unsigned t0, t1;
+    wrap_limit = __builtin_amdgcn_readfirstlane(wrap_limit);
+    unsigned t0, t1, wc = 0;
         const double ka = odd ? 0.0 : 0x1.99343027bf8c3p-16, kb = odd ? -0x1.994eb3774cf24p-13 : -0x1.6c087e89a359dp-10;
     const double kc = odd ? 0x1.1107605230bc4p-7 : 0x1.55553e1068f19p-5, kd = odd ? -0x1.555545995a603p-3 : -0x1.ffffffd0c621cp-2;
     const double km = odd ? 1.0 : 0.0, kj = odd ? -0.0 : 1.0;
@@ -387,10 +413,10 @@
         __builtin_memcpy(&beal, &ba, 8);
     }
     asm volatile(
-                QPSKLO_RING_TEXT(QPSKLO_HEAD_CHAIN_P, QPSKLO_HEAD_DEFERRED_P, QPSKLO_BODY_P, QPSKLO_WRAP_HEAD_P, "v_mov_b32 v98, 1.0\n\tv_mov_b32 v99, 1.0\n\t", QPSKLO_RING_ALIGN_P, COSTAS_RING_STEPS_LO)
+                QPSKLO_RING_TEXT(QPSKLO_HEAD_CHAIN_P, QPSKLO_HEAD_DEFERRED_P, QPSKLO_BODY_P, QPSKLO_WRAP_HEAD_P_CNT, "v_mov_b32 v98, 1.0\n\tv_mov_b32 v99, 1.0\n\t", QPSKLO_RING_ALIGN_P, COSTAS_RING_STEPS_LO, "")
         : [p] "+v"(phase), [f] "+v"(freq), [k] "+s"(k), [fl] "=&s"(flags), [tm] "=&s"(tmp), [ex] "=&s"(ex),
-          [t0] "=&s"(t0), [t1] "=&s"(t1)
-        : [db] "v"(d_base), [zb] "v"(z_base), [ra] "v"(ready_addr), [ca] "v"(consumed_addr), [ke] "s"(kend),
+          [t0] "=&s"(t0), [t1] "=&s"(t1), [wc] "+s"(wc), [ke] "+s"(kend)
+        : [db] "v"(d_base), [zb] "v"(z_base), [ra] "v"(ready_addr), [ca] "v"(consumed_addr), [wt] "s"(wrap_limit),
           [ka] "v"(ka), [kb] "v"(kb), [kc] "v"(kc), [kd] "v"(kd), [km] "v"(km), [kj] "v"(kj), [sg] "v"(sg),
           [fmax] "v"(max_freq), [beal] "v"(beal),
           [k2pi] "s"(0x1.45F306DC9C883p-1), [nhpi] "s"(-0x1.921FB54442D18p0),
@@ -400,6 +426,7 @@
           "v107", "v108", "v109", "v110", "v111", "v112", "v113", "v114", "v115", "v116", "v117", "v118", "v119",
           "v120", "v121", "v122", "v123", "v124", "v125", "v126", "v127");
     flags_out = flags;
+    wrap_tripped = kend == 0u;
 }
 #undef QPSKLO_DA
 #undef QPSKLO_ZA
diff --git a/qpsk_amd/csrc/kernels.h b/qpsk_amd/csrc/kernels.h
--- a/qpsk_amd/csrc/kernels.h
+++ b/qpsk_amd/csrc/kernels.h
@@ -34,6 +34,8 @@
     int lean_dma;
     int est_waves;
     int lean_pair;
+    int wrap_mode;
+    unsigned *wrap_stats;
     int dbg;
     const float2 *dsrc;
     int dstride;
diff --git a/qpsk_amd/csrc/rx_hist.hip b/qpsk_amd/csrc/rx_hist.hip
--- a/qpsk_amd/csrc/rx_hist.hip
+++ b/qpsk_amd/csrc/rx_hist.hip
@@ -6,6 +6,7 @@
 
 struct StreamLo {
     static constexpr int RING_GROUP = COSTAS_RING_GROUP_LO;
+    static constexpr bool HAS_BF = false;
     template <class... A> static __device__ __forceinline__ void ring(A &&...a) { costas_asm_run_ring_lo(a...); }
     template <class... A> static __device__ __forceinline__ void ring_pair(A &&...a) { costas_asm_run_ring_pair_lo(a...); }
     template <class... A> static __device__ __forceinline__ unsigned run(A &&...a) { return costas_asm_run_lo(a...); }
diff --git a/qpsk_amd/csrc/rx_pipe.h b/qpsk_amd/csrc/rx_pipe.h
--- a/qpsk_amd/csrc/rx_pipe.h
+++ b/qpsk_amd/csrc/rx_pipe.h
@@ -4,6 +4,7 @@
 #include <stdint.h>
 #include "qpsk_device.h"
 #include "costas_asm.h"
+#include "costas_asm_bf.h"
 #include "kernels.h"
 #include "rx_profile.h"
 
@@ -94,6 +95,9 @@
 
 struct StreamHi {
     static constexpr int RING_GROUP = COSTAS_RING_GROUP;
+    static constexpr bool HAS_BF = COSTAS_RING_GROUP == 64;
+    template <class... A> static __device__ __forceinline__ void ring_bf(A &&...a) { costas_asm_run_ring_bf(a...); }
+    template <class... A> static __device__ __forceinline__ void ring_pair_bf(A &&...a) { costas_asm_run_ring_pair_bf(a...); }
     template <class... A> static __device__ __forceinline__ void ring(A &&...a) { costas_asm_run_ring(a...); }
     template <class... A> static __device__ __forceinline__ void ring_pair(A &&...a) { costas_asm_run_ring_pair(a...); }
     template <class... A> static __device__ __forceinline__ unsigned run(A &&...a) { return costas_asm_run(a...); }
@@ -105,6 +109,11 @@
     int done;
     int pad_[3];
 };
+
+enum { WRAP_NEVER = 0, WRAP_ALWAYS = 1, WRAP_AUTO = 2 };
+constexpr unsigned WRAP_BF_LIMIT_PAIR = 8, WRAP_BF_LIMIT_ONE = 6;
+constexpr unsigned WRAP_BF_RUN = 16;
+constexpr unsigned WRAP_BF_STAY = 4;
 
 template <class GM, class ST = StreamHi, class SM>
 __device__ __forceinline__ void costas_wave(const FusedArgs &a, SM *sm, const float2 *dring, float *zring, int G,
@@ -167,7 +176,24 @@
                 const unsigned d_base = lds_addr(dl), z_base = lds_addr(zl);
                 const unsigned ready_addr = lds_addr(&sm->ready[gw]), consumed_addr = lds_addr(&sm->consumed);
                 unsigned long long ign = 0ull;
+                static_assert(!ST::HAS_BF || GPC == 1u, "the form is chosen per chunk: one group per chunk");
+                const int wmode = ST::HAS_BF ? a.wrap_mode : (int)WRAP_NEVER;
+                const unsigned wrap_limit = wmode != WRAP_AUTO ? ~0u : pair ? WRAP_BF_LIMIT_PAIR : WRAP_BF_LIMIT_ONE;
+                unsigned bf_left = wmode == WRAP_ALWAYS ? ~0u : 0u;
+                unsigned bf_seen = 0u;
+                unsigned wst[4] = {0u, 0u, 0u, 0u};
                 while (k < kend) {
+                    const bool bf = __builtin_amdgcn_readfirstlane(bf_left) != 0u;
+                    auto spent = [&](unsigned n) {
+                        if (bf && wmode == WRAP_AUTO && bf_left != 0u) {
+                            bf_left -= min(bf_left, n);
+                            if (bf_left == 0u) {
+                                if (bf_seen >= WRAP_BF_STAY) bf_left = WRAP_BF_RUN * GPC;
+                                else wst[3]++;
+                                bf_seen = 0u;
+                            }
+                        }
+                    };
                     if ((k & (GPC - 1u)) == 0u) {
                         ok = wait_ge(&sm->ready[gw], (int)(k / GPC) + 1, &sm->abort_flag);
                         if (!__all(ok)) { ok = false; break; }
@@ -182,13 +208,31 @@
                         unsigned ks = __builtin_amdgcn_readfirstlane(k);
                         const unsigned kstop = ign ? min(kend, (ks | (GPC - 1u)) + 1u) : kend;
                         probe.enter_stream();
-                        if (pair)
-                            ST::ring_pair(ph, fr, d_base, z_base, ready_addr, consumed_addr, ks, kstop, al, be, fmin_, fmax_, odd, fl, ign);
-                        else
-                            ST::ring(ph, fr, d_base, z_base, ready_addr, consumed_addr, ks, kstop, al, be, fmin_, fmax_, fl, ign);
+                        bool tripped = false;
+                        if constexpr (ST::HAS_BF) {
+                            if (bf) {
+                                const unsigned kbf = min(kstop, ks + min(bf_left, kend - ks));
+                                if (pair)
+                                    ST::ring_pair_bf(ph, fr, d_base, z_base, ready_addr, consumed_addr, ks, kbf, al, be, fmin_, fmax_, odd, fl, ign, bf_seen);
+                                else
+                                    ST::ring_bf(ph, fr, d_base, z_base, ready_addr, consumed_addr, ks, kbf, al, be, fmin_, fmax_, fl, ign, bf_seen);
+                            }
+                        }
+                        if (!bf) {
+                            if (pair)
+                                ST::ring_pair(ph, fr, d_base, z_base, ready_addr, consumed_addr, ks, kstop, al, be, fmin_, fmax_, odd, fl, ign, wrap_limit, tripped);
+                            else
+                                ST::ring(ph, fr, d_base, z_base, ready_addr, consumed_addr, ks, kstop, al, be, fmin_, fmax_, fl, ign, wrap_limit, tripped);
+                        }
                         ran = true;
                         probe.leave_stream();
+                        wst[bf ? 1 : 0] += ks - k;
+                        spent(ks - k);
                         k = ks;
+                        if (tripped) {
+                            bf_left = WRAP_BF_RUN * GPC;
+                            wst[2]++;
+                        }
                     }
                     if ((!ran || fl != 0ull) && k < kend) {
                         const int at = (int)(k & RPOS) * AG;
@@ -203,9 +247,12 @@
                             costas_step_t<true>(ph, fr, al, be, fmin_, fmax_, dl[at + i], tx, ty, qq, over);
                         }
                         k++;
+                        spent(1u);
                         if ((k & (GPC - 1u)) == 0u && lane == 0) st_release(&sm->consumed, (int)(k / GPC));
                     }
                 }
+                if (a.wrap_stats && lane == 0)
+                    for (int i = 0; i < 4; i++) atomicAdd(a.wrap_stats + i, wst[i]);
             }
             ok = __all(ok);
             c = cfull - 1;
diff --git a/qpsk_amd/lib.py b/qpsk_amd/lib.py
--- a/qpsk_amd/lib.py
+++ b/qpsk_amd/lib.py
@@ -45,7 +45,7 @@
     "qpsk_streams_reset", "qpsk_streams_set_loop_state", "qpsk_streams_get_loop_state", "qpsk_streams_rx_cplx",
     "qpsk_streams_rx_pcm", "qpsk_streams_rx_pcm_host", "qpsk_dev_alloc", "qpsk_dev_free", "qpsk_dev_upload", "qpsk_dev_download",
     "qpsk_selftest_sincos_hash", "qpsk_crc16_batch", "qpsk_interleave_batch", "qpsk_scramble_batch",
-    "qpsk_tx_reset", "qpsk_tx_symbols", "qpsk_test_inject_status", "qpsk_test_hist_state", "qpsk_ctx_check",
+    "qpsk_tx_reset", "qpsk_tx_symbols", "qpsk_test_inject_status", "qpsk_test_hist_state", "qpsk_test_wrap_stats", "qpsk_ctx_check",
     "qpsk_multi_create", "qpsk_multi_destroy", "qpsk_multi_shards", "qpsk_multi_load", "qpsk_multi_shard", "qpsk_multi_use_device_input",
     "qpsk_multi_rx_begin", "qpsk_multi_rx_end", "qpsk_multi_set_direct_output", "qpsk_host_alloc", "qpsk_host_free",
     "qpsk_multi_set_packed", "qpsk_pack_symbols", "qpsk_unpack_symbols_host",
@@ -166,6 +166,7 @@
     L.qpsk_test_inject_status.argtypes = [vp, i32]
     L.qpsk_ctx_check.argtypes = [vp]
     L.qpsk_test_hist_state.argtypes = [vp, C.POINTER(i32)]
+    L.qpsk_test_wrap_stats.argtypes = [vp, C.POINTER(C.c_uint32)]
     L.qpsk_test_viterbi_launches.argtypes = [vp, C.POINTER(i32)]
     L.qpsk_test_deframer_advance.argtypes = [vp, C.c_longlong]
     L.qpsk_viterbi_stream_reset.argtypes = [vp, i32, i32, i32, i32, u32, u32]
@@ -331,6 +332,11 @@
         for k, v in kw.items():
             self._check(self.L.qpsk_ctx_set_tuning(self.h, ("QPSK_" + k.upper()).encode(), -1 if v is None else int(v)))
 
+    def wrap_stats(self):
+        out = (C.c_uint32 * 4)()
+        self._check(self.L.qpsk_test_wrap_stats(self.h, out))
+        return tuple(out)
+
     def viterbi_launches(self):
         n = C.c_int(-1)
         self._check(self.L.qpsk_test_viterbi_launches(self.h, C.byref(n)))
```

Measured after the change: 454,700 (median of 3 runs). Within noise of the previous version (+0.2%).
